# cherise215/advchain

Hardware: AMD Instinct MI355X
Metric: augmented images/sec (N adv steps, chain=noise+bias+morph+affine) (higher is better)
Workload: dtype f32

## Files before the change

### advchain_amd/_lib.py

```python
import ctypes
import os
from ctypes import c_char_p, c_double, c_float, c_int, c_int64, c_void_p

_HERE = os.path.dirname(os.path.abspath(__file__))
LIB_PATH = os.path.join(_HERE, "csrc", "libadvchain_hip.so")

_P, _I, _L, _F, _D = c_void_p, c_int, c_int64, c_float, c_double

PROTOTYPES = {
    "advchain_version": (_I, []),
    "advchain_last_error": (c_char_p, []),
    "advchain_set_deterministic": (None, [_I]),
    "advchain_get_deterministic": (_I, []),
    "advchain_grid_sample_fwd": (_I, [_P, _P, _P, _L, _L, _I, _P, _P, _I, _I, _I, _P]),
    "advchain_grid_sample_fwd_ride": (_I, [_P, _P, _P, _P, _P, _L, _L, _I, _P, _P, _I, _I, _I, _I, _P]),
    "advchain_scatter_workspace": (_L, [_L, _I, _P]),
    "advchain_grid_sample_bwd": (_I, [_P, _P, _P, _P, _P, _P, _L, _L, _I, _P, _P, _I, _I, _I, _I, _P]),
    "advchain_window_stage_workspace": (_L, [_L, _L, _I, _P]),
    "advchain_grid_sample_bwd_staged": (_I, [_P, _P, _P, _P, _P, _P, _L, _L, _I, _P, _P, _I, _I, _I, _I, _P, _P]),
    "advchain_last_bwd_route": (_I, []),
    "advchain_det_warp_workspace": (_L, [_L, _L, _I, _P]),
    "advchain_grid_sample_bwd_det": (_I, [_P, _P, _P, _P, _P, _P, _L, _L, _I, _P, _P, _I, _I, _I, _P]),
    "advchain_compose_self_fwd": (_I, [_P, _P, _P, _L, _I, _P, _I, _P, _P]),
    "advchain_compose_self_bwd": (_I, [_P, _P, _P, _P, _I, _I, _L, _I, _P, _P]),
    "advchain_affine_warp_fwd": (_I, [_P, _P, _P, _L, _L, _I, _P, _I, _I, _P]),
    "advchain_affine_warp_fwd_ride": (_I, [_P, _P, _P, _P, _P, _L, _L, _I, _P, _I, _I, _I, _P]),
    "advchain_affine_warp_bwd_workspace": (_L, [_L, _I, _P]),
    "advchain_affine_warp_bwd": (_I, [_P, _P, _P, _P, _P, _P, _L, _L, _I, _P, _I, _I, _P]),
    "advchain_affine_warp_bwd_det": (_I, [_P, _P, _P, _P, _P, _P, _P, _L, _L, _I, _P, _I, _I, _P]),
    "advchain_affine_theta_fwd": (_I, [_P, _P, _F, _P, _P, _L, _I, _P]),
    "advchain_affine_theta_bwd": (_I, [_P, _P, _F, _P, _P, _P, _L, _I, _P]),
    "advchain_tp_interp_fwd": (_I, [_P, _P, _P, _P, _P, _P, _P, _L, _L, _I, _I, _F, _P, _P, _P]),
    "advchain_tp_interp_fwd_smoothed_pair": (_I, [_P, _P, _P, _P, _P, _P, _P, _P, _L, _L, _I, _F, _P, _P, _F, _P]),
    "advchain_band_reduce_axis": (_I, [_P, _P, _P, _P, _P, _P, _P, _P, _I, _L, _L, _F, _P]),
    "advchain_band_reduce_rows_dense": (_I, [_P, _P, _P, _P, _P, _L, _L, _L, _L, _F, _P]),
    "advchain_bias_field_fwd": (_I, [_P, _P, _P, _P, _P, _P, _P, _P, _P, _L, _L, _F, _I, _F, _P]),
    "advchain_bias_field_bwd": (_I, [_P, _P, _P, _P, _P, _P, _P, _P, _P, _P, _L, _L, _F, _I, _F, _P]),
    "advchain_bias_rows_per_wg": (_I, [_P, _L]),
    "advchain_bias_field_fwd_rows": (_I, [_P, _P, _P, _P, _P, _P, _P, _P, _P, _L, _L, _F, _I, _F, _I, _P]),
    "advchain_bias_field_bwd_rows": (_I, [_P, _P, _P, _P, _P, _P, _P, _P, _P, _P, _L, _L, _F, _I, _F, _I, _P]),
    "advchain_bias_field_bwd_reduced": (_I, [_P, _P, _P, _P, _P, _P, _P, _P, _P, _P, _L, _L, _F, _I, _F, _P, _P, _L, _I, _P]),
    "advchain_gauss_axis": (_I, [_P, _P, _P, _L, _L, _I, _P, _I, _P, _I, _I, _F, _P]),
    "advchain_gauss_axis_generic": (_I, [_P, _P, _L, _I, _P, _I, _P, _I, _F, _P]),
    "advchain_max_displacement": (_I, [_P, _P, _L, _I, _P, _P]),
    "advchain_grid_sample_bicubic2d_fwd": (_I, [_P, _P, _P, _L, _L, _P, _P, _I, _P]),
    "advchain_grid_sample_bicubic2d_bwd": (_I, [_P, _P, _P, _P, _P, _L, _L, _P, _P, _I, _P]),
    "advchain_affine_grid2d_fwd": (_I, [_P, _P, _L, _P, _P]),
    "advchain_affine_grid2d_bwd_workspace": (_L, [_L, _P]),
    "advchain_affine_grid2d_bwd": (_I, [_P, _P, _P, _L, _P, _P]),
    "advchain_slot_rows_max": (_I, [_P, _P, _L, _L, _I, _P]),
    "advchain_demons_compose_pair_fwd": (_I, [_P, _P, _P, _P, _P, _P, _P, _P, _P, _P, _P, _P, _P, _L, _I, _I, _P, _P, _F, _F, _I, _P]),
    "advchain_demons_compose_pair_bwd": (_I, [_P, _P, _P, _P, _P, _P, _P, _P, _P, _P, _P, _P, _P, _P, _P, _P, _P, _L, _P, _P, _P, _L,
                                              _I, _I, _P, _F, _F, _P]),
    "advchain_bounds_check": (_I, [_P, _P, _P, _L, _P, _P]),
    "advchain_expo_chain_fused_levels": (_I, [_L, _I, _P, _I, _P]),
    "advchain_expo_chain_fwd": (_I, [_P, _P, _P, _L, _I, _P, _I, _P, _P, _P, _P]),
    "advchain_expo_chain_bwd": (_I, [_P, _P, _P, _P, _P, _P, _P, _L, _I, _P, _I, _P]),
    "advchain_gauss_xy": (_I, [_P, _P, _P, _L, _L, _I, _P, _P, _I, _I, _F, _P, _P, _L]),
    "advchain_gauss_xy_staged": (_I, [_P, _P, _P, _L, _L, _I, _P, _P, _I, _I, _F, _P, _P, _L]),
    "advchain_gauss_xy_lanes": (_I, [_P, _P, _P, _L, _L, _I, _P, _P, _I, _I, _F, _P, _P, _L, _I, _I]),
    "advchain_gauss_xy_plan": (_I, [_I, _P, _L, _P, _P, _P]),
    "advchain_gauss_small": (_I, [_P, _P, _L, _I, _P, _P, _I, _F, _P]),
    "advchain_gauss_small_pair": (_I, [_P, _P, _L, _I, _P, _P, _F, _I, _P]),
    "advchain_axpy": (_I, [_P, _P, _P, _F, _L, _P]),
    "advchain_sign_axpy": (_I, [_P, _P, _P, _F, _L, _P, _P, _P]),
    "advchain_nonzero_mask": (_I, [_P, _P, _L, _P]),
    "advchain_consistency_finish": (_I, [_P, _P, _P, _P, _I, _P]),
    "advchain_norm_workspace": (_L, [_L, _L]),
    "advchain_norm_axpy": (_I, [_P, _P, _P, _P, _F, _L, _L, _P]),
    "advchain_norm_axpy_gated": (_I, [_P, _P, _P, _P, _F, _L, _L, _P, _P, _P]),
    "advchain_update_multi": (_I, [_P, _I, _P, _P]),
    "advchain_consistency_fwd": (_I, [_P, _P, _P, _P, _P, _P, _P, _L, _L, _I, _P, _I, _I, _I, _I, _P]),
    "advchain_consistency_bwd": (_I, [_P, _P, _P, _P, _P, _P, _F, _F, _F, _F, _I, _L, _L, _I, _P, _I, _P]),
    "advchain_consistency_fused_fwd": (_I, [_P, _P, _P, _P, _P, _L, _L, _I, _P, _I, _I, _I, _I, _P]),
    "advchain_consistency_fused_bwd": (_I, [_P, _P, _P, _P, _P, _P, _F, _F, _F, _F, _I, _L, _L, _I, _P, _I, _P]),
    "advchain_consistency_wide_fwd": (_I, [_P, _P, _P, _P, _P, _P, _L, _L, _I, _P, _I, _I, _I, _I, _P]),
    "advchain_consistency_wide_bwd": (_I, [_P, _P, _P, _P, _P, _P, _P, _F, _F, _F, _F, _I, _L, _L, _I, _P, _I, _P]),
    "advchain_consistency_ref_bwd": (_I, [_P, _P, _P, _P, _P, _P, _P, _F, _F, _F, _F, _I, _L, _L, _I, _P, _I, _P]),
    "advchain_set_ref_grad_reg_max_k": (None, [_I]),
    "advchain_get_ref_grad_reg_max_k": (_I, []),
    "advchain_consistency_lp_fwd": (_I, [_P, _I, _P, _I, _P, _P, _P, _P, _L, _L, _I, _P, _I, _I, _I, _I, _P]),
    "advchain_consistency_lp_bwd": (_I, [_P, _I, _P, _I, _P, _P, _P, _P, _P, _F, _F, _F, _F, _I, _L, _L, _I, _P, _I, _P]),
    "advchain_consistency_lp_ref_bwd": (_I, [_P, _I, _P, _I, _P, _P, _P, _P, _P, _F, _F, _F, _F, _I, _L, _L, _I, _P, _I, _P]),
    "advchain_consistency_cw_fwd": (_I, [_P, _I, _P, _I, _P, _P, _P, _P, _L, _L, _I, _P, _I, _I, _I, _I, _P, _P]),
    "advchain_consistency_cw_bwd": (_I, [_P, _I, _P, _I, _P, _P, _P, _P, _P, _F, _F, _F, _F, _I, _L, _L, _I, _P, _I, _P, _P]),
    "advchain_consistency_cw_ref_bwd": (_I, [_P, _I, _P, _I, _P, _P, _P, _P, _P, _F, _F, _F, _F, _I, _L, _L, _I, _P, _I, _P, _P]),
    "advchain_consistency_fused_fwd_bf16": (_I, [_P, _P, _P, _P, _P, _L, _L, _I, _P, _P]),
    "advchain_consistency_fused_bwd_bf16": (_I, [_P, _P, _P, _P, _P, _P, _F, _F, _F, _L, _L, _I, _P, _P]),
    "advchain_seg_loss_workspace": (_L, [_L, _I, _P]),
    "advchain_ce2d_fwd": (_I, [_P, _I, _P, _P, _P, _P, _P, _P, _L, _L, _P, _F, _P]),
    "advchain_ce2d_bwd": (_I, [_P, _I, _P, _P, _P, _P, _P, _P, _P, _L, _L, _P, _F, _P]),
    "advchain_contour_fwd": (_I, [_P, _P, _P, _P, _P, _P, _P, _L, _L, _I, _P, _I, _I, _P]),
    "advchain_contour_bwd": (_I, [_P, _P, _P, _P, _L, _L, _I, _P, _I, _P]),
    "advchain_one_hot": (_I, [_P, _P, _L, _L, _L, _P]),
    "advchain_dice_workspace": (_L, [_L, _L, _I, _P]),
    "advchain_dice_fwd": (_I, [_P, _I, _P, _P, _P, _P, _P, _P, _P, _L, _L, _I, _P, _I, _F, _F, _F, _P]),
    "advchain_dice_bwd": (_I, [_P, _I, _P, _P, _P, _P, _P, _P, _P, _P, _L, _L, _I, _P, _F, _F, _P]),
    "advchain_edt": (_I, [_P, _I, _P, _I, _P, _L, _I, _P, _P]),
    "advchain_signed_maps_workspace": (_L, [_L, _L, _I, _P]),
    "advchain_signed_maps": (_I, [_P, _P, _P, _P, _L, _L, _I, _P, _P]),
    "advchain_surface_metrics_workspace": (_L, [_L, _L, _I, _P]),
    "advchain_surface_metrics": (_I, [_P, _P, _P, _D, _P, _P, _P, _P, _P, _P, _P, _P, _P, _L, _L, _I, _P, _P]),
    "advchain_boundary_workspace": (_L, [_L, _L, _I, _P]),
    "advchain_boundary_fwd": (_I, [_P, _I, _P, _P, _P, _P, _P, _P, _L, _L, _I, _P, _I, _P]),
    "advchain_boundary_bwd": (_I, [_P, _I, _P, _P, _P, _P, _P, _P, _L, _L, _I, _P, _I, _P]),
    "advchain_image_diff2d_fwd": (_I, [_P, _P, _P, _L, _L, _P, _P]),
    "advchain_image_diff2d_bwd": (_I, [_P, _P, _P, _L, _L, _P, _P]),
    "advchain_jacobian_det2d_fwd": (_I, [_P, _P, _L, _P, _P]),
    "advchain_jacobian_det2d_bwd": (_I, [_P, _P, _P, _L, _P, _P]),
    "advchain_expo_start": (_I, [_P, _P, _F, _L, _I, _P, _P]),
    "advchain_image_diff3d_fwd": (_I, [_P, _P, _P, _P, _L, _L, _P, _P]),
    "advchain_image_diff3d_bwd": (_I, [_P, _P, _P, _P, _L, _L, _P, _P]),
    "advchain_jacobian_det_fwd": (_I, [_P, _P, _L, _I, _P, _I, _P]),
    "advchain_jacobian_det_bwd": (_I, [_P, _P, _P, _P, _L, _I, _P, _I, _P]),
    "advchain_jacobian_det_workspace": (_L, [_L, _I, _P]),
    "advchain_jacobian_stats_workspace": (_L, [_L, _I, _P]),
    "advchain_jacobian_stats": (_I, [_P, _P, _P, _P, _P, _P, _L, _I, _P, _I, _P]),
    "advchain_sumsq_ordered": (_I, [_P, _L, _P, _P, _P]),
    "advchain_bicubic2d_det_workspace": (_L, [_L, _L, _P]),
    "advchain_grid_sample_bicubic2d_bwd_det": (_I, [_P, _P, _P, _P, _P, _P, _L, _L, _P, _P, _I, _P]),
    "advchain_tp_interp_sumsq_partials": (_L, [_P, _L]),
    "advchain_tp_interp_sumsq_ordered": (_I, [_P, _P, _P, _P, _P, _P, _L, _L, _P, _P, _P]),
    "advchain_consistency_fwd_partials": (_L, [_L, _L, _I, _P, _I, _I, _I]),
    "advchain_consistency_fwd_ord": (_I, [_P, _P, _P, _P, _P, _P, _P, _L, _P, _L, _L, _I, _P, _I, _I, _I, _I, _P]),
    "advchain_consistency_fused_fwd_partials": (_L, [_L, _L, _I, _P, _I, _I, _I, _I]),
    "advchain_consistency_fused_fwd_ord": (_I, [_P, _P, _P, _P, _P, _L, _P, _L, _L, _I, _P, _I, _I, _I, _I, _P]),
    "advchain_consistency_wide_fwd_partials": (_L, [_L, _L, _I, _P, _I, _I]),
    "advchain_consistency_wide_fwd_ord": (_I, [_P, _P, _P, _P, _P, _P, _L, _P, _L, _L, _I, _P, _I, _I, _I, _I, _P]),
    "advchain_consistency_lp_fwd_partials": (_L, [_L, _L, _I, _P, _I]),
    "advchain_consistency_lp_fwd_ord": (_I, [_P, _I, _P, _I, _P, _P, _P, _P, _L, _P, _L, _L, _I, _P, _I, _I, _I, _I, _P, _P]),
    "advchain_consistency_finish_ord": (_I, [_P, _L, _P, _P, _P, _P, _P]),
}

class UpdateDesc(ctypes.Structure):
    _fields_ = [("base", c_void_p), ("x", c_void_p), ("out", c_void_p), ("old", c_void_p), ("N", c_int64), ("M", c_int64),
                ("kind", ctypes.c_int32), ("step", c_float)]


_lib = None


class AdvchainHipError(RuntimeError):
    pass


class _Lib(object):

    def __init__(self, cdll):
        self._cdll = cdll
        self._raw = {}
        self.records = []

    def _bind(self, name, res, args):
        fn = getattr(self._cdll, name)
        fn.restype = res
        fn.argtypes = args
        self._raw[name] = fn
        setattr(self, name, fn)

    def timed(self, names=None, every=1):
        import contextlib
        import torch

        @contextlib.contextmanager
        def ctx():
            chosen = [n for n in self._raw if (names is None or n in names) and self._raw[n].restype is c_int
                      and len(self._raw[n].argtypes) > 0]
            for n in chosen:
                raw = self._raw[n]

                count = [0]

                def wrapped(*a, _raw=raw, _n=n, _count=count):
                    _count[0] += 1
                    if _count[0] % every:
                        return _raw(*a)
                    e0 = torch.cuda.Event(enable_timing=True)
                    e1 = torch.cuda.Event(enable_timing=True)
                    e0.record()
                    rc = _raw(*a)
                    e1.record()
                    self.records.append((_n, a, e0, e1))
                    return rc
                setattr(self, n, wrapped)
# ... 47 lines not shown
```

### advchain_amd/csrc/adjoint_gather.hip

```cpp
#include "sampler_common.h"

namespace advchain {

constexpr int kXPad = 4;

__global__ void k_gather_prepare(int32_t* ws, int chain) {
  ws[2] = chain ? ws[3] : 0;
  ws[0] = 0;
  ws[1] = 0;
  ws[3] = 0;
}

template <int E>
__device__ __forceinline__ float tent(float f) { return fmaxf(0.f, 1.f - fabsf(f - (float)E)); }

template <int H, int K = -H>
struct XSpread {
  template <int C>
  static __device__ __forceinline__ void run(float (&acc)[C][2 * H + 1], const float (&a)[C], float fx) {
    const float w = tent<K>(fx);
#pragma unroll
    for (int c = 0; c < C; ++c) acc[c][K + H] = fmaf(a[c], w, acc[c][K + H]);
    if constexpr (K < H) XSpread<H, K + 1>::template run<C>(acc, a, fx);
  }
// ... 394 lines not shown
#pragma unroll
    for (int cz = 0; cz < (DIM == 3 ? 2 : 1); ++cz)
#pragma unroll
      for (int cy = 0; cy < 2; ++cy)
#pragma unroll
        for (int cx = 0; cx < 2; ++cx) {
          if (!t.ok(cz, cy, cx)) continue;
          const int o = t.off(cz, cy, cx, d);
          const float wgt = t.w(cz, cy, cx);
          for (int c = 0; c < C; ++c) {
            const float v = wgt * gout[((int64_t)n * C + c) * V + s];
            const float old = atomicAdd(gin + ((int64_t)n * C + c) * V + o, v);
            const float nv = fabsf(old + v);
            if (absmax_out && nv > __builtin_nontemporal_load(absmax_out))
              atomicMax(reinterpret_cast<unsigned int*>(absmax_out), __float_as_uint(nv));
          }
        }
  }
}

template <int VEC>
__global__ void __launch_bounds__(kBlock) k_max_displacement(const float* __restrict__ phi, float* __restrict__ out, Dims d, int ndim) {
  const int V = (int)d.voxels();
  const int plane = blockIdx.y;
  const int a = plane % ndim;
  const int Sa = a == 0 ? d.s2 : (a == 1 ? d.s1 : d.s0);
  const float* p = phi + (int64_t)plane * V;
  float m = 0.f;
  for (int i = (blockIdx.x * kBlock + threadIdx.x) * VEC; i < V; i += gridDim.x * kBlock * VEC) {
    float v[VEC];
    load_vec<VEC>(p + i, v);
    const int x = i % d.s2, q = i / d.s2;
    const int y = q % d.s1, z = q / d.s1;
#pragma unroll
    for (int k = 0; k < VEC; ++k) {
      const int sa = a == 0 ? x + k : (a == 1 ? y : z);
      const float dv = fabsf(unnormalize(v[k], Sa) - (float)sa);
      m = fmaxf(m, dv < 1.0e9f ? dv : 1.0e9f);
    }
  }
#pragma unroll
  for (int o = 32; o > 0; o >>= 1) m = fmaxf(m, __shfl_xor(m, o, 64));
  __shared__ float smem[kBlock / 64];
  if ((threadIdx.x & 63) == 0) smem[threadIdx.x >> 6] = m;
  __syncthreads();
  if (threadIdx.x == 0) {
    for (int w = 1; w < kBlock / 64; ++w) m = fmaxf(m, smem[w]);
    if (m > __builtin_nontemporal_load(out)) atomicMax(reinterpret_cast<unsigned int*>(out), __float_as_uint(m));
  }
}

template <int NT, int VEC>
__global__ void __launch_bounds__(NT) k_slot_rows_max(float* __restrict__ slots, float* __restrict__ out, int cols, int reset) {
  float* p = slots + (int64_t)blockIdx.x * cols;
  float m = -3.4e38f;
  bool nan = false;
  if (VEC == 4) {
    for (int j = threadIdx.x * 4; j < cols; j += NT * 4) {
      const float4 v = *reinterpret_cast<const float4*>(p + j);
      nan = nan || !(v.x == v.x) || !(v.y == v.y) || !(v.z == v.z) || !(v.w == v.w);
      m = fmaxf(fmaxf(m, fmaxf(v.x, v.y)), fmaxf(v.z, v.w));
      if (reset) *reinterpret_cast<float4*>(p + j) = make_float4(0.f, 0.f, 0.f, 0.f);
    }
  } else {
    for (int j = threadIdx.x; j < cols; j += NT) {
      const float v = p[j];
      nan = nan || !(v == v);
      m = fmaxf(m, v);
      if (reset) p[j] = 0.f;
    }
  }
#pragma unroll
  for (int o = 32; o > 0; o >>= 1) {
    m = fmaxf(m, __shfl_xor(m, o, 64));
    const int other = __shfl_xor((int)nan, o, 64);
    nan = nan || other != 0;
  }
  __shared__ float sm[NT / 64];
  __shared__ int sn[NT / 64];
  if ((threadIdx.x & 63) == 0) { sm[threadIdx.x >> 6] = m; sn[threadIdx.x >> 6] = nan; }
  __syncthreads();
  if (threadIdx.x == 0) {
    for (int w = 1; w < NT / 64; ++w) { m = fmaxf(m, sm[w]); nan = nan || sn[w]; }
    out[blockIdx.x] = nan ? __int_as_float(0x7fc00000) : m;
  }
}

__global__ void __launch_bounds__(64) k_bounds_check(const float* __restrict__ v, const float* __restrict__ lo,
                                                     const float* __restrict__ hi, int n, int* __restrict__ flag) {
  bool bad = false;
  for (int i = threadIdx.x; i < n; i += 64) {
    const float x = v[i];
    bad = bad || !(x >= lo[i] && x < hi[i]);
  }
  if (__any(bad) && threadIdx.x == 0) atomicOr(flag, 1);
}

}

using namespace advchain;

template <int DIM, int C, int H, bool SELF, bool GG, int TZ, int TY, int NT>
static void launch_gather(const float* gout, const float* in, const float* grid, float* gin, float* ggrid, int64_t N,
                          Dims d, int padding, int clamp_grid, int32_t* ws, int chain, bool strict, hipStream_t st) {
  using G = GatherCfg<DIM, C, H, SELF, GG, TZ, TY, NT>;
  const int wide = d.s2 > 64;
  const int n2 = wide ? (d.s2 + (64 - 2 * kXPad) - 1) / (64 - 2 * kXPad) : 1;
  const int n1 = (d.s1 + TY - 1) / TY;
  const int n0 = DIM == 3 ? (d.s0 + TZ - 1) / TZ : 1;
  int* cnt = ws;
  float* amax_out = SELF ? reinterpret_cast<float*>(ws + 3) : nullptr;
  int2* list = reinterpret_cast<int2*>(ws + 4);
  const int64_t cap64 = N * d.voxels();
  const int cap = cap64 > 0x7fffffff ? 0x7fffffff : (int)cap64;
  const bool border = padding == PAD_BORDER;
  const uintptr_t al = reinterpret_cast<uintptr_t>(gout) | reinterpret_cast<uintptr_t>(grid) |
                       (GatherCfg<DIM, C, H, SELF, GG, TZ, TY, NT>::STAGE_IN ? reinterpret_cast<uintptr_t>(in) : 0);
  const bool unaligned = (d.s2 & 3) != 0 || (al & 15) != 0;
  const int flags = ((border || clamp_grid) ? kClip : 0) | (border ? kBorder : 0) | (clamp_grid ? kClampGrid : 0) |
                    (unaligned ? kUnaligned : 0);
  auto kern = k_adjoint_gather<DIM, C, H, SELF, GG, TZ, TY, NT>;
  static bool attr_set = false;
  if (G::LDS > 65536 && !attr_set) {
    (void)hipFuncSetAttribute(reinterpret_cast<const void*>(kern), hipFuncAttributeMaxDynamicSharedMemorySize, (int)G::LDS);
    attr_set = true;
  }
  if (strict) {
    hipLaunchKernelGGL(kern, dim3((unsigned)(n0 * n1 * n2), (unsigned)N), dim3(NT), G::LDS, st, gout, in, grid, gin, ggrid,
                       d, n1, n2, wide, flags, (float*)nullptr, (int*)nullptr, (int2*)nullptr, 0, SELF ? ws : (int32_t*)nullptr);
    return;
  }
  hipLaunchKernelGGL(k_gather_prepare, dim3(1), dim3(1), 0, st, ws, chain);
  hipLaunchKernelGGL(kern, dim3((unsigned)(n0 * n1 * n2), (unsigned)N), dim3(NT), G::LDS, st, gout, in, grid, gin, ggrid, d,
                     n1, n2, wide, flags, amax_out, cnt, list, cap, (int32_t*)nullptr);
  if (border) hipLaunchKernelGGL((k_gather_overflow<DIM, PAD_BORDER>), dim3(16), dim3(kBlock), 0, st, gout, grid, gin, C, d,
                                 clamp_grid, cnt, list, cap, amax_out);
  else hipLaunchKernelGGL((k_gather_overflow<DIM, PAD_ZEROS>), dim3(16), dim3(kBlock), 0, st, gout, grid, gin, C, d,
                          clamp_grid, cnt, list, cap, amax_out);
// ... 110 lines not shown
```

### advchain_amd/csrc/common.h

```cpp
#pragma once
#include <hip/hip_runtime.h>
#include <stdint.h>

namespace advchain {

__device__ __forceinline__ float sub_max(float m) { return m == -__builtin_inff() ? -3.402823466e38f : m; }

enum { INTERP_LINEAR = 0, INTERP_NEAREST = 1 };
enum { PAD_ZEROS = 0, PAD_BORDER = 1, PAD_REFLECTION = 2 };

constexpr int kBlock = 256;

struct Dims {
  int s0, s1, s2;
  __host__ __device__ int64_t voxels() const { return (int64_t)s0 * s1 * s2; }
};

__device__ __forceinline__ float mul_nc(float a, float b) {
#pragma clang fp contract(off)
  return a * b;
}

__device__ __forceinline__ float lin_coord(int i, int S) {
  if (S <= 1) return S == 1 ? -1.f : 0.f;
// ... 42 lines not shown
    else if (x >= (float)(S - 1)) { x = (float)(S - 1); mult = 0.f; }
  }
  return x;
}

template <int PAD>
__device__ __forceinline__ AxisTap make_tap(float coord, int S) {
  AxisTap t;
  float x = source_index<PAD>(coord, S, t.mult);
  if (!(x > -1.0e9f && x < 1.0e9f)) x = -16.f;
  const float f = floorf(x);
  t.i0 = (int)f;
  t.w1 = x - f;
  t.w0 = (f + 1.f) - x;
  t.v0 = (t.i0 >= 0) && (t.i0 < S);
  t.v1 = (t.i0 + 1 >= 0) && (t.i0 + 1 < S);
  return t;
}

template <int PAD>
__device__ __forceinline__ int nearest_index(float coord, int S, bool& valid) {
  float m;
  float x = source_index<PAD>(coord, S, m);
  if (!(x > -1.0e9f && x < 1.0e9f)) x = -16.f;
  const int i = (int)nearbyintf(x);
  valid = (i >= 0) && (i < S);
  return i;
}

__device__ __forceinline__ float wave_sum(float v) {
#pragma unroll
  for (int o = 32; o > 0; o >>= 1) v += __shfl_xor(v, o, 64);
  return v;
}

template <int NV>
__device__ __forceinline__ void block_sum(float (&v)[NV], float* smem) {
  const int lane = threadIdx.x & 63, wave = threadIdx.x >> 6;
#pragma unroll
  for (int k = 0; k < NV; ++k) v[k] = wave_sum(v[k]);
  if (lane == 0) {
#pragma unroll
    for (int k = 0; k < NV; ++k) smem[wave * NV + k] = v[k];
  }
  __syncthreads();
  if (threadIdx.x == 0) {
    const int nw = (blockDim.x + 63) >> 6;
#pragma unroll
    for (int k = 0; k < NV; ++k) {
      float s = 0.f;
      for (int w = 0; w < nw; ++w) s += smem[w * NV + k];
      v[k] = s;
    }
  }
}

__device__ __forceinline__ float lane_next_f(float v) {
  return __int_as_float(__builtin_amdgcn_update_dpp(0, __float_as_int(v), 0x130, 0xf, 0xf, false));
}
__device__ __forceinline__ float lane_prev_f(float v) {
  return __int_as_float(__builtin_amdgcn_update_dpp(0, __float_as_int(v), 0x138, 0xf, 0xf, false));
}

template <int CTRL, int ROW_MASK>
__device__ __forceinline__ float dpp_add(float v) {
  return v + __int_as_float(__builtin_amdgcn_update_dpp(0, __float_as_int(v), CTRL, ROW_MASK, 0xf, false));
}
__device__ __forceinline__ float wave_sum_lane63(float v) {
  v = dpp_add<0xB1, 0xf>(v);
  v = dpp_add<0x4E, 0xf>(v);
  v = dpp_add<0x141, 0xf>(v);
  v = dpp_add<0x140, 0xf>(v);
  v = dpp_add<0x142, 0xa>(v);
  return dpp_add<0x143, 0xc>(v);
}

constexpr int kSumSlots = 64;
__device__ __forceinline__ int sum_slot() { return (int)((blockIdx.x + blockIdx.y * 7u) % kSumSlots); }

#ifndef ADVCHAIN_FIX_RPI
#define ADVCHAIN_FIX_RPI 1
#endif
__device__ __forceinline__ int fix_round(float x) {
#if ADVCHAIN_FIX_RPI
  int r;
  asm("v_cvt_rpi_i32_f32 %0, %1" : "=v"(r) : "v"(x));
  return r;
#else
  return __float2int_rn(x);
#endif
}

struct FixScale {
  int shift;
  float mul;
  float inv;
};
__device__ __forceinline__ FixScale fix_scale(float gmax, int bits) {
  FixScale s;
  const bool ok = gmax <= 3.40282347e38f;
  const int e = ok ? __builtin_amdgcn_frexp_expf(gmax) : 0;
  const float gm = ok ? __builtin_amdgcn_frexp_mantf(gmax) : gmax;
  s.shift = bits - e;
  s.mul = (gmax > 0.f && ok) ? 1.f / gm : 0.f;
  s.inv = gm;
  return s;
// ... 89 lines not shown
```

### advchain_amd/csrc/demons_compose.cpp

```cpp
#include <stdint.h>
#include "advchain_hip.h"

#define ADVCHAIN_OK 0
#define ADVCHAIN_ERR_ARG (-1)
extern "C" void advchain_set_error_(const char* msg);
bool advchain_gauss_xy_takes(int ndim, const int64_t* dims, int64_t planes);

namespace {
inline int64_t prod(int ndim, const int64_t* d) {
  int64_t p = 1;
  for (int i = 0; i < ndim; ++i) p *= d[i];
  return p;
}
inline bool aligned16(const void* a, const void* b = nullptr, const void* c = nullptr, const void* d = nullptr) {
  return ((reinterpret_cast<uintptr_t>(a) | reinterpret_cast<uintptr_t>(b) | reinterpret_cast<uintptr_t>(c) |
           reinterpret_cast<uintptr_t>(d)) & 15) == 0;
}
}

extern "C" {

int advchain_demons_compose_pair_fwd(const float* vel, float* s1, float* phi0, float* fields, float* pos, float* q,
                                     float* disp, float* rows_max, const int32_t* itab, const float* ftab,
                                     const int64_t* S3, const int64_t* g3, const int64_t* B3, int64_t N, int ndim, int n,
                                     const int32_t* hints, const float* weights9_host, float scale, float inv, int fuse,
                                     void* stream) {
  if (!(vel && s1 && phi0 && pos && q && itab && ftab && S3 && g3 && B3 && weights9_host) || ndim != 2 || n < 1 || (n > 1 && !fields)) {
    advchain_set_error_("demons_compose_pair_fwd: null pointer / bad arguments (2D only)");
    return ADVCHAIN_ERR_ARG;
  }
  const int64_t* gd = g3 + 1;
  const int64_t* Sd = S3 + 1;
  if (prod(ndim, gd) > 4096 || !advchain_gauss_xy_takes(ndim, Sd, 2 * N * ndim) || !aligned16(pos, q)) return -2;
  int rc = advchain_tp_interp_fwd_smoothed_pair(vel, s1, phi0, itab, ftab, S3, g3, B3, N * ndim, ndim, 1, inv, disp, weights9_host,
                                                scale, stream);
  if (rc == -2) {
    rc = advchain_gauss_small_pair(vel, s1, N * ndim, ndim, gd, weights9_host, scale, 0, stream);
    if (rc != 0) return rc;
    rc = advchain_tp_interp_fwd(s1, phi0, itab, ftab, S3, g3, B3, 2 * N * ndim, ndim, ndim, 1, inv, nullptr, disp, stream);
  }
  if (rc != 0) return rc;
  auto late = [](int r, const char* what) {
    if (r == -2) { advchain_set_error_(what); return ADVCHAIN_ERR_ARG; }
    return r;
  };
  const int64_t slots = ADVCHAIN_DISP_SLOTS;
  rc = advchain_expo_chain_fwd(phi0, fields, pos, 2 * N, ndim, Sd, n, disp, hints, (disp && fuse) ? disp + (int64_t)(n + 1) * slots : nullptr, stream);
  if (rc != 0) return late(rc, "demons_compose_pair_fwd: the chain refused a shape the pre-check had accepted (launches already queued)");
  rc = advchain_gauss_xy(pos, q, nullptr, 2 * N * ndim, ndim, ndim, Sd, weights9_host, 2, 1, 1.0f, stream, nullptr, 2 * N * ndim);
  if (rc != 0) return late(rc, "demons_compose_pair_fwd: the final smoothing refused a shape the pre-check had accepted (launches already queued)");
  if (disp && rows_max) rc = advchain_slot_rows_max(disp, rows_max, n + 2, slots, 1, stream);
  return rc;
}

int advchain_demons_compose_pair_bwd(const float* gq_lo, const float* gq_hi, const float* pos, const float* phi0,
                                     const float* fields, float* gpos, float* g, float* scratch, int32_t* ws, float* t1,
                                     float* gs1, float* gvel, const int32_t* halos, const int32_t* itab, const float* ftab,
                                     const float* wd, const int32_t* wlo, int64_t WB, const int64_t* S3, const int64_t* g3,
                                     const int64_t* B3, int64_t N, int ndim, int n, const float* weights9_host, float scale,
                                     float inv, void* stream) {
  if (!(gq_lo && gq_hi && pos && phi0 && gpos && g && scratch && ws && t1 && gs1 && gvel && halos && itab && ftab && wd && wlo &&
        weights9_host) || ndim != 2 || n < 1) {
    advchain_set_error_("demons_compose_pair_bwd: null pointer / bad arguments (2D only)");
    return ADVCHAIN_ERR_ARG;
  }
  const int64_t* gd = g3 + 1;
  const int64_t* Sd = S3 + 1;
  const int64_t planes = 2 * N * ndim;
  if (prod(ndim, gd) > 4096 || !advchain_gauss_xy_takes(ndim, Sd, planes) || !aligned16(gq_lo, gq_hi, gpos, pos)) return -2;
  int rc = advchain_gauss_xy(gq_lo, gpos, pos, planes, ndim, ndim, Sd, weights9_host, 0, 2, 1.0f, stream, gq_hi, N * ndim);
  if (rc != 0) return rc;
  rc = advchain_expo_chain_bwd(gpos, phi0, fields, g, scratch, ws, halos, 2 * N, ndim, Sd, n, stream);
  if (rc == -2) {
    advchain_set_error_("demons_compose_pair_bwd: the chain refused a shape the pre-check had accepted (launches already queued)");
    return ADVCHAIN_ERR_ARG;
  }
  if (rc != 0) return rc;
  rc = advchain_band_reduce_rows_dense(g, gpos, t1, wd, wlo, planes * S3[1], S3[2], g3[2], WB, inv, stream);
  if (rc == -2) rc = advchain_band_reduce_axis(g, gpos, t1, itab, ftab, S3, g3, B3, 2, planes * S3[1], 1, inv, stream);
  if (rc != 0) return rc;
  rc = advchain_band_reduce_axis(t1, nullptr, gs1, itab, ftab, S3, g3, B3, 1, planes, g3[2], 1.0f, stream);
  if (rc != 0) return rc;
  return advchain_gauss_small_pair(gs1, gvel, N * ndim, ndim, gd, weights9_host, scale, 1, stream);
}

}
```

### advchain_amd/csrc/error.cpp

```cpp
#include <string.h>

#include <atomic>

static thread_local char g_last_error[512] = "";

extern "C" void advchain_set_error_(const char* msg) {
  strncpy(g_last_error, msg ? msg : "", sizeof(g_last_error) - 1);
  g_last_error[sizeof(g_last_error) - 1] = 0;
}

extern "C" const char* advchain_last_error(void) { return g_last_error; }

static std::atomic<int> g_deterministic{0};
extern "C" void advchain_set_deterministic(int on) { g_deterministic.store(on ? 1 : 0, std::memory_order_relaxed); }
extern "C" int advchain_get_deterministic(void) { return g_deterministic.load(std::memory_order_relaxed); }

static thread_local int g_last_bwd_route = 0;
extern "C" void advchain_set_route_(int route) { g_last_bwd_route = route; }
extern "C" int advchain_last_bwd_route(void) { return g_last_bwd_route; }

extern "C" int advchain_version(void) { return 200; }
```

### advchain_amd/csrc/fields.hip

```cpp
#include "sampler_common.h"

namespace advchain {

constexpr int kBandMax = 8;

struct BandAxis {
  const int* start;
  const float* w;
  const int* lo;
  const int* hi;
  int S, g, B;
};
struct BandTables { BandAxis a[3]; };

__device__ __forceinline__ void decode3(int v, const Dims& d, int& i0, int& i1, int& i2) {
  i2 = v % d.s2;
  const int r = v / d.s2;
  i1 = r % d.s1;
  i0 = r / d.s1;
}

__device__ __forceinline__ float tp_eval(const float* __restrict__ coef, const BandTables& T, int i0, int i1, int i2) {
  const BandAxis& A0 = T.a[0];
  const BandAxis& A1 = T.a[1];
  const BandAxis& A2 = T.a[2];
  const int s0 = A0.start[i0], s1 = A1.start[i1], s2 = A2.start[i2];
  const float* w0 = A0.w + i0 * A0.B;
  const float* w1 = A1.w + i1 * A1.B;
  const float* w2 = A2.w + i2 * A2.B;
  float acc = 0.f;
  for (int a = 0; a < A0.B; ++a) {
    float acc1 = 0.f;
    for (int b = 0; b < A1.B; ++b) {
      const float* row = coef + ((int64_t)(s0 + a) * A1.g + (s1 + b)) * A2.g + s2;
      float acc2 = 0.f;
      for (int c = 0; c < A2.B; ++c) acc2 += row[c] * w2[c];
      acc1 += acc2 * w1[b];
    }
    acc += acc1 * w0[a];
  }
  return acc;
}

constexpr int kTpChunk = 32;
constexpr int kTpMaxLds = 2048;

struct TpGeom { int XT, ROWS; };

__host__ __device__ inline TpGeom tp_geom(int S2) {
  TpGeom g;
  (void)S2;
  g.XT = 64;
// ... 858 lines not shown
      qb[b] = *reinterpret_cast<const float4*>(in + t + ((x0 >= 0 && x0 < d.s2) ? (b - 1) * 4 : 0));
    }
#pragma unroll
    for (int b = 0; b < 3; ++b) {
      const int x0 = idx[2] + (b - 1) * 4;
      const bool inr = x0 >= 0 && x0 < d.s2;
      win[b * 4 + 0] = inr ? pre(qb[b].x, idx[0], idx[1], x0) : 0.f;
      win[b * 4 + 1] = inr ? pre(qb[b].y, idx[0], idx[1], x0 + 1) : 0.f;
      win[b * 4 + 2] = inr ? pre(qb[b].z, idx[0], idx[1], x0 + 2) : 0.f;
      win[b * 4 + 3] = inr ? pre(qb[b].w, idx[0], idx[1], x0 + 3) : 0.f;
    }
#pragma unroll
    for (int o = 0; o < 4; ++o)
#pragma unroll
      for (int k = 0; k < 9; ++k) acc[o] += gw.w[k] * win[o + k];
  } else {
    const int stride = AXIS == 1 ? d.s2 : d.s1 * d.s2;
    const int ia = idx[AXIS];
    float4 q[9];
#pragma unroll
    for (int k = -4; k <= 4; ++k) {
      const int jc = min(max(ia + k, 0), S[AXIS] - 1);
      q[k + 4] = *reinterpret_cast<const float4*>(in + t + (int64_t)(jc - ia) * stride);
    }
#pragma unroll
    for (int k = -4; k <= 4; ++k) {
      const int j = ia + k;
      const bool inr = j >= 0 && j < S[AXIS];
      const int j0 = AXIS == 0 ? j : idx[0], j1 = AXIS == 1 ? j : idx[1];
      const float w = gw.w[k + 4];
      acc[0] += inr ? w * pre(q[k + 4].x, j0, j1, idx[2]) : 0.f;
      acc[1] += inr ? w * pre(q[k + 4].y, j0, j1, idx[2] + 1) : 0.f;
      acc[2] += inr ? w * pre(q[k + 4].z, j0, j1, idx[2] + 2) : 0.f;
      acc[3] += inr ? w * pre(q[k + 4].w, j0, j1, idx[2] + 3) : 0.f;
    }
  }
  if (POST == 1) {
#pragma unroll
    for (int o = 0; o < 4; ++o) acc[o] += lin_coord(caxis == 2 ? idx[2] + o : idx[caxis], S[caxis]);
  }
  if (POST == 2) {
    const float4 a = *reinterpret_cast<const float4*>(aux + t);
    const float av[4] = {a.x, a.y, a.z, a.w};
#pragma unroll
    for (int o = 0; o < 4; ++o) {
      float slope;
      border_identity(av[o], S[caxis], slope);
      acc[o] *= slope;
    }
  }
  *reinterpret_cast<float4*>(out + t) = make_float4(acc[0], acc[1], acc[2], acc[3]);
}

template <int PRE, int POST>
__global__ void __launch_bounds__(kBlock)
k_gauss_xy(const float* __restrict__ in, float* __restrict__ out, const float* __restrict__ aux, Dims d, int C, GaussW gw,
           float scale, int TY, const float* __restrict__ in_hi, int planes_lo) {
  extern __shared__ float gx_lds[];
  const int W = d.s2, Q = W >> 2, PA = W + 8;
  const int R = TY + 8;
  float* A = gx_lds;
  float* B = gx_lds + R * PA;
  const int plane = blockIdx.z, iz = blockIdx.y;
  const int y0 = blockIdx.x * TY;
  const int caxis = 2 - plane % C;
  const int Sc = caxis == 2 ? d.s2 : (caxis == 1 ? d.s1 : d.s0);
  const int64_t base = ((int64_t)plane * d.s0 + iz) * d.s1 * (int64_t)W;
  const float* src = (in_hi && plane >= planes_lo) ? in_hi + (((int64_t)(plane - planes_lo) * d.s0 + iz) * d.s1 * (int64_t)W) : in + base;
  for (int e = threadIdx.x; e < R * 2; e += kBlock)
    *reinterpret_cast<float4*>(A + (e >> 1) * PA + ((e & 1) ? W + 4 : 0)) = make_float4(0.f, 0.f, 0.f, 0.f);
  for (int e = threadIdx.x; e < R * Q; e += kBlock) {
    const int r = e / Q, q = e - r * Q;
    const int gy = y0 - 4 + r;
    const bool inr = gy >= 0 && gy < d.s1;
    const float4 v = *reinterpret_cast<const float4*>(src + (int64_t)min(max(gy, 0), d.s1 - 1) * W + 4 * q);
    float t[4] = {v.x, v.y, v.z, v.w};
#pragma unroll
    for (int o = 0; o < 4; ++o) {
      if (PRE == 1) t[o] *= scale;
      if (PRE == 2) {
        float sl;
        t[o] = border_identity(t[o], Sc, sl) - lin_coord(caxis == 2 ? 4 * q + o : (caxis == 1 ? gy : iz), Sc);
      }
      if (!inr) t[o] = 0.f;
    }
    *reinterpret_cast<float4*>(A + r * PA + 4 + 4 * q) = make_float4(t[0], t[1], t[2], t[3]);
  }
  __syncthreads();
  for (int e = threadIdx.x; e < R * Q; e += kBlock) {
    const int r = e / Q, q = e - r * Q;
    const float* a = A + r * PA + 4 * q;
    const float4 a0 = *reinterpret_cast<const float4*>(a), a1 = *reinterpret_cast<const float4*>(a + 4),
                 a2 = *reinterpret_cast<const float4*>(a + 8);
    const float win[12] = {a0.x, a0.y, a0.z, a0.w, a1.x, a1.y, a1.z, a1.w, a2.x, a2.y, a2.z, a2.w};
    float acc[4] = {0.f, 0.f, 0.f, 0.f};
#pragma unroll
    for (int o = 0; o < 4; ++o)
#pragma unroll
      for (int k = 0; k < 9; ++k) acc[o] += gw.w[k] * win[o + k];
    *reinterpret_cast<float4*>(B + r * W + 4 * q) = make_float4(acc[0], acc[1], acc[2], acc[3]);
  }
  __syncthreads();
  for (int e = threadIdx.x; e < TY * Q; e += kBlock) {
    const int ry = e / Q, q = e - ry * Q;
    const int gy = y0 + ry;
    if (gy >= d.s1) continue;
    float acc[4] = {0.f, 0.f, 0.f, 0.f};
#pragma unroll
    for (int k = 0; k < 9; ++k) {
      const float4 b = *reinterpret_cast<const float4*>(B + (ry + k) * W + 4 * q);
      acc[0] += gw.w[k] * b.x; acc[1] += gw.w[k] * b.y; acc[2] += gw.w[k] * b.z; acc[3] += gw.w[k] * b.w;
    }
    const int64_t off = base + (int64_t)gy * W + 4 * q;
    if (POST == 1) {
#pragma unroll
      for (int o = 0; o < 4; ++o) acc[o] += lin_coord(caxis == 2 ? 4 * q + o : (caxis == 1 ? gy : iz), Sc);
    }
    if (POST == 2) {
      const float4 a4 = *reinterpret_cast<const float4*>(aux + off);
      const float av[4] = {a4.x, a4.y, a4.z, a4.w};
#pragma unroll
      for (int o = 0; o < 4; ++o) {
        float slope;
        border_identity(av[o], Sc, slope);
        acc[o] *= slope;
      }
    }
    *reinterpret_cast<float4*>(out + off) = make_float4(acc[0], acc[1], acc[2], acc[3]);
  }
}

template <int PRE, int POST, int NT, int U>
__global__ void __launch_bounds__(NT)
k_gauss_xy_lanes(const float* __restrict__ in, float* __restrict__ out, const float* __restrict__ aux, Dims d, int C, GaussW gw,
                 float scale, int TY, const float* __restrict__ in_hi, int planes_lo) {
  extern __shared__ float gx_lds[];
  const int W = d.s2, Q = W >> 2;
  const int R = TY + 8, NI = R * Q;
  float* B = gx_lds;
  const int plane = blockIdx.z, iz = blockIdx.y;
  const int y0 = blockIdx.x * TY;
  const int caxis = 2 - plane % C;
  const int Sc = caxis == 2 ? d.s2 : (caxis == 1 ? d.s1 : d.s0);
  const int64_t base = ((int64_t)plane * d.s0 + iz) * d.s1 * (int64_t)W;
  const float* src = (in_hi && plane >= planes_lo) ? in_hi + (((int64_t)(plane - planes_lo) * d.s0 + iz) * d.s1 * (int64_t)W) : in + base;
  float4 v[U];
#pragma unroll
  for (int u = 0; u < U; ++u) {
    if (u * NT >= NI) break;
    const int e = min((int)threadIdx.x + u * NT, NI - 1);
    const int r = e / Q, q = e - r * Q;
    const int gy = y0 - 4 + r;
    v[u] = *reinterpret_cast<const float4*>(src + (int64_t)min(max(gy, 0), d.s1 - 1) * W + 4 * q);
  }
#pragma unroll
  for (int u = 0; u < U; ++u) {
    if (u * NT >= NI) break;
    const int e0 = (int)threadIdx.x + u * NT;
    const int e = min(e0, NI - 1);
    const int r = e / Q, q = e - r * Q;
    const int gy = y0 - 4 + r;
    const bool inr = gy >= 0 && gy < d.s1;
    float t[4] = {v[u].x, v[u].y, v[u].z, v[u].w};
#pragma unroll
    for (int o = 0; o < 4; ++o) {
      if (PRE == 1) t[o] *= scale;
      if (PRE == 2) {
        float sl;
        t[o] = border_identity(t[o], Sc, sl) - lin_coord(caxis == 2 ? 4 * q + o : (caxis == 1 ? gy : iz), Sc);
      }
      if (!inr) t[o] = 0.f;
    }
    float win[12];
    const bool first = q == 0, last = q == Q - 1;
#pragma unroll
    for (int o = 0; o < 4; ++o) {
      const float pv = lane_prev_f(t[o]), nx = lane_next_f(t[o]);
      win[o] = first ? 0.f : pv;
      win[4 + o] = t[o];
      win[8 + o] = last ? 0.f : nx;
    }
    float acc[4] = {0.f, 0.f, 0.f, 0.f};
#pragma unroll
    for (int o = 0; o < 4; ++o)
#pragma unroll
      for (int k = 0; k < 9; ++k) acc[o] += gw.w[k] * win[o + k];
    if (e0 < NI) *reinterpret_cast<float4*>(B + r * W + 4 * q) = make_float4(acc[0], acc[1], acc[2], acc[3]);
  }
  __syncthreads();
// ... 112 lines not shown
template <int NT>
__global__ void __launch_bounds__(NT)
k_gauss_small(const float* __restrict__ in, float* __restrict__ out, Dims d, int ndim, GaussW gw, float scale, int mirror,
              int P) {
  __shared__ float buf[2][kGaussSmallMax];
  const int V = (int)d.voxels();
  const int S[3] = {d.s0, d.s1, d.s2};
  const int stride[3] = {d.s1 * d.s2, d.s2, 1};
  const int b = blockIdx.x;
  float first[(kGaussSmallMax + NT - 1) / NT];
  const int rounds = mirror == 2 ? 2 : 1;
  for (int round = 0; round < rounds; ++round) {
    const float* src = in + (int64_t)(mirror == 1 ? b % P : b + round * P) * V;
    const float sc = (mirror == 1 && b >= P) ? -scale : scale;
    if (round) __syncthreads();
    for (int i = threadIdx.x; i < V; i += NT) buf[0][i] = src[i] * sc;
    __syncthreads();
    int cur = 0;
    for (int pass = 0; pass < ndim; ++pass) {
      const int axis = 2 - pass;
      const int Sa = S[axis], st = stride[axis];
      for (int i = threadIdx.x; i < V; i += NT) {
        const int ia = (i / st) % Sa;
        float acc = 0.f;
#pragma unroll
        for (int k = -4; k <= 4; ++k) {
          const int j = ia + k;
          if (j >= 0 && j < Sa) acc += gw.w[k + 4] * buf[cur][i + k * st];
        }
        buf[cur ^ 1][i] = acc;
      }
      __syncthreads();
      cur ^= 1;
    }
    float* dst = out + (int64_t)b * V;
    if (mirror != 2) {
      for (int i = threadIdx.x; i < V; i += NT) dst[i] = buf[cur][i];
    } else if (round == 0) {
#pragma unroll
      for (int q = 0; q < (kGaussSmallMax + NT - 1) / NT; ++q) {
        const int i = threadIdx.x + q * NT;
        first[q] = i < V ? buf[cur][i] : 0.f;
      }
    } else {
#pragma unroll
      for (int q = 0; q < (kGaussSmallMax + NT - 1) / NT; ++q) {
        const int i = threadIdx.x + q * NT;
        if (i < V) dst[i] = first[q] - buf[cur][i];
      }
    }
  }
}

__global__ void __launch_bounds__(kBlock)
k_axpy(const float* __restrict__ x, const float* __restrict__ y, float* __restrict__ out, float a, int64_t n4,
       int64_t n) {
  const int64_t i = (int64_t)blockIdx.x * kBlock + threadIdx.x;
  if (i < n4) {
    const float4 p = reinterpret_cast<const float4*>(y)[i];
    float4 q = x ? reinterpret_cast<const float4*>(x)[i] : make_float4(0.f, 0.f, 0.f, 0.f);
    q.x += a * p.x; q.y += a * p.y; q.z += a * p.z; q.w += a * p.w;
    reinterpret_cast<float4*>(out)[i] = q;
  }
  const int64_t j = n4 * 4 + i;
  if (j < n) out[j] = (x ? x[j] : 0.f) + a * y[j];
}

__global__ void __launch_bounds__(kBlock)
k_sign_axpy(const float* __restrict__ base, const float* __restrict__ x, float* __restrict__ out, float a, int64_t n,
            const float* __restrict__ gate, const float* __restrict__ old) {
  const int64_t i = (int64_t)blockIdx.x * kBlock + threadIdx.x;
  if (i >= n) return;
  if (gate && !(fabsf(gate[0]) <= 3.0e38f)) { out[i] = old[i]; return; }
  const float v = x[i];
  const float sg = v > 0.f ? 1.f : (v < 0.f ? -1.f : v);
  out[i] = (base ? base[i] : 0.f) + a * sg;
}

__global__ void __launch_bounds__(kBlock)
k_nonzero_mask(const float* __restrict__ x, float* __restrict__ out, int64_t n) {
  const int64_t i = (int64_t)blockIdx.x * kBlock + threadIdx.x;
  if (i < n) out[i] = x[i] != 0.f ? 1.f : 0.f;
}

__global__ void __launch_bounds__(kBlock)
k_sumsq_partial(const float* __restrict__ x, float* __restrict__ partial, int64_t M, int chunk) {
  __shared__ float smem[4];
  const int n = blockIdx.y, b = blockIdx.x;
  const float* xn = x + (int64_t)n * M;
  const int64_t lo = (int64_t)b * chunk, hi = min(lo + chunk, M);
  float s[1] = {0.f};
  for (int64_t i = lo + threadIdx.x; i < hi; i += kBlock) { const float q = xn[i]; s[0] += q * q; }
  block_sum<1>(s, smem);
  if (threadIdx.x == 0) partial[(int64_t)n * gridDim.x + b] = s[0];
}

__global__ void __launch_bounds__(kBlock)
k_norm_axpy(const float* __restrict__ base, const float* __restrict__ x, const float* __restrict__ partial,
            int nb, float step, float* __restrict__ out, int64_t M, int chunk, const float* __restrict__ gate,
            const float* __restrict__ old) {
  __shared__ float smem[4];
  __shared__ float inv_s;
  const int n = blockIdx.y, b = blockIdx.x;
  float s[1] = {0.f};
  for (int i = threadIdx.x; i < nb; i += kBlock) s[0] += partial[(int64_t)n * nb + i];
  block_sum<1>(s, smem);
// ... 525 lines not shown
  }
#define GA(PRE, POST)                                                                                                     \
  do {                                                                                                                    \
    if (!v4) hipLaunchKernelGGL((k_gauss_axis<PRE, POST>), grid, blk, 0, st, in, out, aux, total, d, (int)C, axis, gw, scale); \
    else if (axis == 2) hipLaunchKernelGGL((k_gauss_axis_v4<PRE, POST, 2>), grid, blk, 0, st, in, out, aux, total / 4, d, (int)C, gw, scale, riw); \
    else if (axis == 1) hipLaunchKernelGGL((k_gauss_axis_v4<PRE, POST, 1>), grid, blk, 0, st, in, out, aux, total / 4, d, (int)C, gw, scale, 0); \
    else hipLaunchKernelGGL((k_gauss_axis_v4<PRE, POST, 0>), grid, blk, 0, st, in, out, aux, total / 4, d, (int)C, gw, scale, 0); \
  } while (0)
  switch (pre * 3 + post) {
    case 0: GA(0, 0); break;
    case 1: GA(0, 1); break;
    case 2: GA(0, 2); break;
    case 3: GA(1, 0); break;
    case 4: GA(1, 1); break;
    case 5: GA(1, 2); break;
    case 6: GA(2, 0); break;
    case 7: GA(2, 1); break;
    default: GA(2, 2); break;
  }
#undef GA
  ADVCHAIN_LAUNCH_CHECK();
  return ADVCHAIN_OK;
}

}

bool advchain_gauss_xy_takes(int ndim, const int64_t* dims, int64_t planes) {
  if (!dims_ok(ndim, dims)) return false;
  const Dims d = make_dims(ndim, dims);
  if ((d.s2 & 3) != 0 || d.s2 < 8 || d.s2 > 512 || d.s1 < 8 || planes > 65535 || d.s0 > 65535) return false;
  int TY = 32;
  while (TY > 8 && (size_t)(TY + 8) * (2 * d.s2 + 8) * 4 > 53248) TY >>= 1;
  if (TY > d.s1) TY = (d.s1 + 7) / 8 * 8;
  return (size_t)(TY + 8) * (2 * d.s2 + 8) * sizeof(float) <= 65536;
}

static bool gauss_xy_lane_shape(const Dims& d) {
  const int Q = d.s2 >> 2;
  return (d.s2 & 3) == 0 && Q >= 2 && Q <= 64 && (Q & (Q - 1)) == 0 && d.s1 >= 8;
}
static bool gauss_xy_lane_tile_ok(int ty, int nt) {
  return (ty == 16 && (nt == 256 || nt == 512)) || (ty == 32 && (nt == 256 || nt == 512)) || (ty == 64 && nt == 1024);
}
static bool gauss_xy_lane_rule(const Dims& d, int64_t planes, int& ty, int& nt) {
  (void)planes;
  if (!gauss_xy_lane_shape(d) || d.s2 != 256) return false;
  ty = 32; nt = 512;
  return true;
}
static inline int gauss_xy_clamp_ty(int TY, const Dims& d) { return TY > d.s1 ? (d.s1 + 7) / 8 * 8 : TY; }

enum { kGxyAuto = 0, kGxyStaged = 1, kGxyLanes = 2 };

static int gauss_xy_launch(const float* in, float* out, const float* aux, int64_t planes, int64_t C, int ndim, const int64_t* dims,
                           const float* weights9, int pre, int post, float scale, void* stream, const float* in_hi, int64_t planes_lo,
                           int want, int ty, int nt) {
  ADVCHAIN_CHECK_ARG(in && out && in != out && weights9, "gauss_xy: null/aliased pointer");
  ADVCHAIN_CHECK_ARG(dims_ok(ndim, dims), "gauss_xy: bad dims");
  ADVCHAIN_CHECK_ARG(C >= 1 && C <= 3 && pre >= 0 && pre <= 2 && post >= 0 && post <= 2 && (post != 2 || aux), "gauss_xy: bad C/pre/post");
  ADVCHAIN_CHECK_ARG(post == 0 || ndim == 2, "gauss_xy: post belongs to the last axis");
  const Dims d = make_dims(ndim, dims);
  if ((d.s2 & 3) != 0 || d.s2 < 8 || d.s2 > 512 || d.s1 < 8 || planes > 65535 || d.s0 > 65535 ||
      ((reinterpret_cast<uintptr_t>(in) | reinterpret_cast<uintptr_t>(out) | reinterpret_cast<uintptr_t>(aux) |
        reinterpret_cast<uintptr_t>(in_hi)) & 15) != 0)
    return ADVCHAIN_ERR_UNSUPPORTED;
  ADVCHAIN_CHECK_ARG(!in_hi || (planes_lo > 0 && planes_lo < planes), "gauss_xy: bad split of the input planes");
  if (want == kGxyLanes) {
    ADVCHAIN_CHECK_ARG(gauss_xy_lane_tile_ok(ty, nt), "gauss_xy_lanes: (ty, nt) must be (16,256), (16,512), (32,256), (32,512) or (64,1024)");
    if (!gauss_xy_lane_shape(d)) return ADVCHAIN_ERR_UNSUPPORTED;
  }
  if (planes == 0 || d.voxels() == 0) return ADVCHAIN_OK;
  GaussW gw;
  for (int k = 0; k < 9; ++k) gw.w[k] = weights9[k];
  hipStream_t st = (hipStream_t)stream;
  if (want == kGxyLanes || (want == kGxyAuto && gauss_xy_lane_rule(d, planes, ty, nt))) {
    const int TY = gauss_xy_clamp_ty(ty, d);
    const size_t lds = (size_t)(TY + 8) * d.s2 * sizeof(float);
    dim3 grid((unsigned)((d.s1 + TY - 1) / TY), (unsigned)d.s0, (unsigned)planes);
#define GXL(PRE, POST, NT_, U_) do { \
    auto kern = k_gauss_xy_lanes<PRE, POST, NT_, U_>; \
    if (lds > 65536) (void)hipFuncSetAttribute(reinterpret_cast<const void*>(kern), hipFuncAttributeMaxDynamicSharedMemorySize, (int)lds); \
    hipLaunchKernelGGL(kern, grid, dim3(NT_), lds, st, in, out, aux, d, (int)C, gw, scale, TY, in_hi, (int)planes_lo); } while (0)
#define GXL_TILE(PRE, POST) do { \
    if (ty == 16 && nt == 256) GXL(PRE, POST, 256, 6); \
    else if (ty == 16) GXL(PRE, POST, 512, 3); \
    else if (ty == 32 && nt == 256) GXL(PRE, POST, 256, 10); \
    else if (ty == 32) GXL(PRE, POST, 512, 5); \
    else GXL(PRE, POST, 1024, 5); } while (0)
    switch (pre * 3 + post) {
      case 0: GXL_TILE(0, 0); break;
      case 1: GXL_TILE(0, 1); break;
      case 2: GXL_TILE(0, 2); break;
      case 3: GXL_TILE(1, 0); break;
      case 4: GXL_TILE(1, 1); break;
      case 5: GXL_TILE(1, 2); break;
      case 6: GXL_TILE(2, 0); break;
      case 7: GXL_TILE(2, 1); break;
      default: GXL_TILE(2, 2); break;
    }
#undef GXL_TILE
#undef GXL
    ADVCHAIN_LAUNCH_CHECK();
    return ADVCHAIN_OK;
  }
  int TY = 32;
  while (TY > 8 && (size_t)(TY + 8) * (2 * d.s2 + 8) * 4 > 53248) TY >>= 1;
  if (TY > d.s1) TY = (d.s1 + 7) / 8 * 8;
  const size_t lds = (size_t)(TY + 8) * (2 * d.s2 + 8) * sizeof(float);
  if (lds > 65536) return ADVCHAIN_ERR_UNSUPPORTED;
  dim3 grid((unsigned)((d.s1 + TY - 1) / TY), (unsigned)d.s0, (unsigned)planes);
#define GXY(PRE, POST) hipLaunchKernelGGL((k_gauss_xy<PRE, POST>), grid, dim3(kBlock), lds, st, in, out, aux, d, (int)C, gw, scale, TY, in_hi, (int)planes_lo)
  switch (pre * 3 + post) {
    case 0: GXY(0, 0); break;
    case 1: GXY(0, 1); break;
    case 2: GXY(0, 2); break;
    case 3: GXY(1, 0); break;
    case 4: GXY(1, 1); break;
    case 5: GXY(1, 2); break;
    case 6: GXY(2, 0); break;
    case 7: GXY(2, 1); break;
    default: GXY(2, 2); break;
  }
#undef GXY
  ADVCHAIN_LAUNCH_CHECK();
  return ADVCHAIN_OK;
}

extern "C" {

int advchain_gauss_xy(const float* in, float* out, const float* aux, int64_t planes, int64_t C, int ndim, const int64_t* dims,
                      const float* weights9, int pre, int post, float scale, void* stream, const float* in_hi, int64_t planes_lo) {
  return gauss_xy_launch(in, out, aux, planes, C, ndim, dims, weights9, pre, post, scale, stream, in_hi, planes_lo, kGxyAuto, 0, 0);
}

int advchain_gauss_xy_staged(const float* in, float* out, const float* aux, int64_t planes, int64_t C, int ndim,
                             const int64_t* dims, const float* weights9, int pre, int post, float scale, void* stream,
                             const float* in_hi, int64_t planes_lo) {
  return gauss_xy_launch(in, out, aux, planes, C, ndim, dims, weights9, pre, post, scale, stream, in_hi, planes_lo, kGxyStaged, 0, 0);
}

int advchain_gauss_xy_lanes(const float* in, float* out, const float* aux, int64_t planes, int64_t C, int ndim,
                            const int64_t* dims, const float* weights9, int pre, int post, float scale, void* stream,
                            const float* in_hi, int64_t planes_lo, int ty, int nt) {
  return gauss_xy_launch(in, out, aux, planes, C, ndim, dims, weights9, pre, post, scale, stream, in_hi, planes_lo, kGxyLanes, ty, nt);
}

int advchain_gauss_xy_plan(int ndim, const int64_t* dims, int64_t planes, int* form, int* ty, int* nt) {
  if (!form || !ty || !nt || !dims_ok(ndim, dims) || planes < 0) return -1;
  *form = 0; *ty = 0; *nt = 0;
  if (!advchain_gauss_xy_takes(ndim, dims, planes)) return 0;
  const Dims d = make_dims(ndim, dims);
  int t = 0, n = 0;
  if (gauss_xy_lane_rule(d, planes, t, n)) {
    *form = 2; *ty = gauss_xy_clamp_ty(t, d); *nt = n;
    return 0;
  }
  int TY = 32;
  while (TY > 8 && (size_t)(TY + 8) * (2 * d.s2 + 8) * 4 > 53248) TY >>= 1;
  *form = 1; *ty = gauss_xy_clamp_ty(TY, d); *nt = kBlock;
  return 0;
}

static int gauss_small_launch(const float* in, float* out, int64_t planes, int ndim, const int64_t* dims,
                              const float* weights9, int pre, float scale, int mirror, void* stream) {
  ADVCHAIN_CHECK_ARG(in && out && in != out && weights9, "gauss_small: null/aliased pointer");
  ADVCHAIN_CHECK_ARG(dims_ok(ndim, dims), "gauss_small: bad dims");
  ADVCHAIN_CHECK_ARG(pre == 0 || pre == 1, "gauss_small: pre must be 0 or 1");
  const Dims d = make_dims(ndim, dims);
  ADVCHAIN_CHECK_ARG(d.voxels() <= kGaussSmallMax, "gauss_small: plane larger than 4096 voxels");
  ADVCHAIN_CHECK_ARG(planes >= 0 && planes < (1ll << 30), "gauss_small: bad plane count");
  if (planes == 0) return ADVCHAIN_OK;
  GaussW gw;
  for (int k = 0; k < 9; ++k) gw.w[k] = weights9[k];
  const unsigned blocks = (unsigned)(mirror == 1 ? 2 * planes : planes);
  if (d.voxels() > 1024)
    hipLaunchKernelGGL(k_gauss_small<1024>, dim3(blocks), dim3(1024), 0, (hipStream_t)stream, in, out, d, ndim, gw,
                       pre == 1 ? scale : 1.f, mirror, (int)planes);
  else
    hipLaunchKernelGGL(k_gauss_small<kBlock>, dim3(blocks), dim3(kBlock), 0, (hipStream_t)stream, in, out, d, ndim, gw,
                       pre == 1 ? scale : 1.f, mirror, (int)planes);
  ADVCHAIN_LAUNCH_CHECK();
  return ADVCHAIN_OK;
}

int advchain_gauss_small(const float* in, float* out, int64_t planes, int ndim, const int64_t* dims,
                         const float* weights9, int pre, float scale, void* stream) {
  return gauss_small_launch(in, out, planes, ndim, dims, weights9, pre, scale, 0, stream);
}

int advchain_gauss_small_pair(const float* in, float* out, int64_t planes, int ndim, const int64_t* dims,
                              const float* weights9, float scale, int adjoint, void* stream) {
  return gauss_small_launch(in, out, planes, ndim, dims, weights9, 1, scale, adjoint ? 2 : 1, stream);
}

int advchain_sign_axpy(const float* base, const float* x, float* out, float a, int64_t n, const float* gate, const float* old,
                       void* stream) {
  ADVCHAIN_CHECK_ARG(x && out && n >= 0 && (!gate || old), "sign_axpy: null pointer");
  if (n == 0) return ADVCHAIN_OK;
  hipLaunchKernelGGL(k_sign_axpy, dim3(advchain_blocks(n, kBlock)), dim3(kBlock), 0, (hipStream_t)stream, base, x, out, a, n, gate, old);
  ADVCHAIN_LAUNCH_CHECK();
  return ADVCHAIN_OK;
}

int advchain_nonzero_mask(const float* x, float* out, int64_t n, void* stream) {
  ADVCHAIN_CHECK_ARG(x && out && n >= 0, "nonzero_mask: null pointer");
  if (n == 0) return ADVCHAIN_OK;
  hipLaunchKernelGGL(k_nonzero_mask, dim3(advchain_blocks(n, kBlock)), dim3(kBlock), 0, (hipStream_t)stream, x, out, n);
  ADVCHAIN_LAUNCH_CHECK();
  return ADVCHAIN_OK;
}

int advchain_axpy(const float* x, const float* y, float* out, float a, int64_t n, void* stream) {
  ADVCHAIN_CHECK_ARG(y && out && n >= 0, "axpy: null pointer");
  if (n == 0) return ADVCHAIN_OK;
  const bool al = ((reinterpret_cast<uintptr_t>(y) | reinterpret_cast<uintptr_t>(out) | reinterpret_cast<uintptr_t>(x)) & 15) == 0;
  const int64_t n4 = al ? n / 4 : 0;
  const int64_t threads = n4 > (n - 4 * n4) ? n4 : (n - 4 * n4);
  hipLaunchKernelGGL(k_axpy, dim3(advchain_blocks(threads, kBlock)), dim3(kBlock), 0, (hipStream_t)stream, x, y, out, a, n4, n);
  ADVCHAIN_LAUNCH_CHECK();
  return ADVCHAIN_OK;
}

int64_t advchain_norm_workspace(int64_t N, int64_t M) {
  const int64_t chunk = 4096;
  return N * ((M + chunk - 1) / chunk);
}

int advchain_norm_axpy_gated(const float* base, const float* x, float* out, float* workspace, float step, int64_t N,
                             int64_t M, const float* gate, const float* old, void* stream) {
  ADVCHAIN_CHECK_ARG(x && out && workspace && (!gate || old), "norm_axpy: null pointer");
  ADVCHAIN_CHECK_ARG(N >= 0 && N < 65536 && M >= 0, "norm_axpy: bad N/M");
  if (N == 0 || M == 0) return ADVCHAIN_OK;
  const int chunk = 4096;
  const int nb = (int)((M + chunk - 1) / chunk);
  dim3 grid(nb, (unsigned)N), blk(kBlock);
  if (M <= 16384) {
    hipLaunchKernelGGL(k_norm_axpy_row, dim3((unsigned)N), blk, 0, (hipStream_t)stream, base, x, step, out, M, gate, old);
    ADVCHAIN_LAUNCH_CHECK();
    return ADVCHAIN_OK;
  }
  hipLaunchKernelGGL(k_sumsq_partial, grid, blk, 0, (hipStream_t)stream, x, workspace, M, chunk);
  hipLaunchKernelGGL(k_norm_axpy, grid, blk, 0, (hipStream_t)stream, base, x, workspace, nb, step, out, M, chunk, gate, old);
  ADVCHAIN_LAUNCH_CHECK();
  return ADVCHAIN_OK;
}

int advchain_norm_axpy(const float* base, const float* x, float* out, float* workspace, float step, int64_t N,
// ... 27 lines not shown
```

### advchain_amd/csrc/loss.hip

```cpp
#include <algorithm>
#include "loss_common.h"

namespace advchain {

constexpr int kMaxK = 16;

template <class... ORD>
__global__ void __launch_bounds__(kBlock)
k_softmax_diff(const float* __restrict__ pred, const float* __restrict__ ref, const float* __restrict__ mask,
               float* __restrict__ P, float* __restrict__ D, float* __restrict__ sums, int K, int V, int mask_ch,
               int ref_is_prob, int want_kl, ORD... ord) {
  __shared__ float smem[8];
  const int n = blockIdx.y;
  const int v = blockIdx.x * kBlock + threadIdx.x;
  float acc[2] = {0.f, 0.f};
  if (v < V) {
    const float* pn = pred + (int64_t)n * K * V + v;
    const float* rn = ref + (int64_t)n * K * V + v;
    float mp = -INFINITY, mr = -INFINITY;
    for (int k = 0; k < K; ++k) {
      mp = fmaxf(mp, pn[(int64_t)k * V]);
      mr = fmaxf(mr, rn[(int64_t)k * V]);
    }
    float sp = 0.f, sr = 0.f;
    for (int k = 0; k < K; ++k) {
      sp += ADVCHAIN_SM_EXP(pn[(int64_t)k * V] - mp);
      sr += ADVCHAIN_SM_EXP(rn[(int64_t)k * V] - mr);
    }
    const float lsp = logf(sp), lsr = logf(sr);
    const float isp = 1.f / sp, isr = 1.f / sr;
    for (int k = 0; k < K; ++k) {
      const float zp = pn[(int64_t)k * V] - mp, zr = rn[(int64_t)k * V] - mr;
      const float p = mul_nc(ADVCHAIN_SM_EXP(zp), isp);
      const float t = ref_is_prob ? rn[(int64_t)k * V] : mul_nc(ADVCHAIN_SM_EXP(zr), isr);
      const float m = mask ? mask[((int64_t)n * mask_ch + (mask_ch > 1 ? k : 0)) * V + v] : 1.f;
      const int64_t o = ((int64_t)n * K + k) * V + v;
      P[o] = p;
      D[o] = p - t;
      const float e = p * m - t * m;
      acc[0] += e * e;
      if (want_kl) acc[1] += kl_term(t, zr - lsr, zp - lsp, m, ref_is_prob);
    }
  }
  block_sum<2>(acc, smem);
  if (threadIdx.x == 0) {
    sums_put(sums, 0, acc[0], ord...);
    if (want_kl) sums_put(sums, 3, acc[1], ord...);
  }
}

template <int K, class... ORD>
__global__ void __launch_bounds__(kBlock)
k_softmax_diff_v4(const float* __restrict__ pred, const float* __restrict__ ref, const float* __restrict__ mask,
// ... 765 lines not shown
        }
      }
    }
  };
  if (EDGES) { row(y0 - 1, 0); }
  row(y0, 1);
  for (int i1 = y0; i1 < y1; ++i1) {
    if (EDGES) {
      row(i1 + 1, 2);
      const int v = (i0 * d.s1 + i1) * d.s2 + x;
      float m[4] = {1.f, 1.f, 1.f, 1.f};
      if (mask) {
        const float4 mm = *reinterpret_cast<const float4*>(mask + (int64_t)n * V + v);
        m[0] = mm.x; m[1] = mm.y; m[2] = mm.z; m[3] = mm.w;
      }
#pragma unroll
      for (int k = 1; k < K; ++k) {
        float ra[4], rb[4];
#pragma unroll
        for (int q = 0; q < 4; ++q) {
          float ga, gb;
          if (DIM == 2) {
            ga = zd[k - 1][0].v[q] + 2.f * zd[k - 1][1].v[q] + zd[k - 1][2].v[q];
            gb = zs[k - 1][0].v[q] - zs[k - 1][2].v[q];
          } else {
            ga = zs[k - 1][0].v[q] - zs[k - 1][2].v[q];
            gb = zd[k - 1][0].v[q] + 2.f * zd[k - 1][1].v[q] + zd[k - 1][2].v[q];
          }
          const float ea = ga * m[q], eb = gb * m[q];
          if (ok) { acc[1] += ea * ea; acc[2] += eb * eb; }
          ra[q] = 2.f * m[q] * m[q] * ga;
          rb[q] = 2.f * m[q] * m[q] * gb;
        }
        if (R && ok) {
          st4(R + ((int64_t)n * 2 * (K - 1) + 2 * (k - 1)) * V + v, ra[0], ra[1], ra[2], ra[3]);
          st4(R + ((int64_t)n * 2 * (K - 1) + 2 * (k - 1) + 1) * V + v, rb[0], rb[1], rb[2], rb[3]);
        }
        zs[k - 1][0] = zs[k - 1][1]; zs[k - 1][1] = zs[k - 1][2];
        zd[k - 1][0] = zd[k - 1][1]; zd[k - 1][1] = zd[k - 1][2];
      }
    } else if (i1 + 1 < y1) {
      row(i1 + 1, 1);
    }
  }
  block_sum<4>(acc, smem);
  if (threadIdx.x == 0) {
    sums_put(sums, 0, acc[0], ord...);
    if (EDGES) {
      sums_put(sums, 1, acc[1], ord...);
      sums_put(sums, 2, acc[2], ord...);
    }
    if (KL) sums_put(sums, 3, acc[3], ord...);
  }
}

template <int DIM, int K, bool KL, typename ST = float>
__global__ void __launch_bounds__(kBlock)
k_loss_fused_bwd4(const ST* __restrict__ pred, const ST* __restrict__ ref, const ST* __restrict__ R,
                  const float* __restrict__ mask, const float* __restrict__ gscale, ST* __restrict__ gpred,
                  float c_mse, float c_a, float c_b, Dims d, int mlen, float c_kl, int ref_is_prob) {
  const int n = blockIdx.y;
  const int V = (int)d.voxels();
  int i0, y0, x;
  bool first, last, ok;
  strip_decode4(d, mlen, i0, y0, x, first, last, ok);
  const float gs = gscale ? gscale[0] : 1.f;
  Quad za[K - 1][3], zb[K - 1][3];
  auto fold = [&](int k, int j1, Quad& a, Quad& b) {
    const ST* Ra = R + ((int64_t)n * 2 * (K - 1) + 2 * (k - 1)) * V;
    Quad as, ad, bs, bd;
    fold_row4<DIM>(Ra, i0, j1, x, first, last, d, as, ad);
    fold_row4<DIM>(Ra + V, i0, j1, x, first, last, d, bs, bd);
#pragma unroll
    for (int q = 0; q < 4; ++q) {
      a.v[q] = DIM == 3 ? as.v[q] : -ad.v[q];
      b.v[q] = DIM == 3 ? -bd.v[q] : bs.v[q];
    }
  };
  if (R) {
#pragma unroll
    for (int k = 1; k < K; ++k) {
      fold(k, y0 - 1, za[k - 1][0], zb[k - 1][0]);
      fold(k, y0, za[k - 1][1], zb[k - 1][1]);
    }
  }
  const int y1 = min(y0 + mlen, d.s1);
  for (int i1 = y0; i1 < y1; ++i1) {
    const int v = (i0 * d.s1 + i1) * d.s2 + x;
    float gp[K][4], pk[K][4], tk[K][4], mt[KL ? K : 1][4], lq[1][4], lt[1][4];
    float dot[4] = {0.f, 0.f, 0.f, 0.f}, klS[4] = {0.f, 0.f, 0.f, 0.f};
    float m[4] = {1.f, 1.f, 1.f, 1.f};
    if (mask) {
      const float4 mm = *reinterpret_cast<const float4*>(mask + (int64_t)n * V + v);
      m[0] = mm.x; m[1] = mm.y; m[2] = mm.z; m[3] = mm.w;
    }
    softmax_pair4<K, false, ST>(pred, ref, (int64_t)n * K * V + v, V, ref_is_prob, pk, tk, lq, lt);
#pragma unroll
    for (int k = 0; k < K; ++k) {
      if (k >= 1 && R) fold(k, i1 + 1, za[k - 1][2], zb[k - 1][2]);
#pragma unroll
      for (int q = 0; q < 4; ++q) {
        const float dv = pk[k][q] - tk[k][q];
        float g = c_mse * 2.f * m[q] * m[q] * dv;
        if (k >= 1 && R) {
          float sa, sb;
          if (DIM == 2) {
// ... 458 lines not shown
  ADVCHAIN_CHECK_ARG(pred && ref && P && D && sums, "consistency_fwd: null pointer");
  ADVCHAIN_CHECK_ARG(dims_ok(ndim, dims), "consistency_fwd: bad dims");
  ADVCHAIN_CHECK_ARG(N >= 0 && N < 65536 && K >= 1 && K <= kMaxK, "consistency_fwd: bad N/K (K <= 16)");
  ADVCHAIN_CHECK_ARG(!mask || mask_channels == 1 || mask_channels == K, "consistency_fwd: mask must have 1 or K channels");
  if (oc)
    for (int r = 0; r < 4; ++r) oc->counts[r] = 0;
  if (N == 0) return ADVCHAIN_OK;
  const Dims d = make_dims(ndim, dims);
  ADVCHAIN_CHECK_ARG(d.voxels() < (1ll << 31), "consistency_fwd: volume too large");
  const int V = (int)d.voxels();
  dim3 g(advchain_blocks(V, kBlock), (unsigned)N), b(kBlock);
  hipStream_t st = (hipStream_t)stream;
  const bool al16 = ((reinterpret_cast<uintptr_t>(pred) | reinterpret_cast<uintptr_t>(ref) | reinterpret_cast<uintptr_t>(mask) |
                      reinterpret_cast<uintptr_t>(P) | reinterpret_cast<uintptr_t>(D)) & 15) == 0;
  const bool v4 = V % 4 == 0 && al16 && K >= 2 && K <= 5;
  const dim3 g4(advchain_blocks(V / 4, kBlock), (unsigned)N);
  const bool edges = want_edges && K > 1;
  const bool rows = (d.s2 % 64) == 0;
  EdgeMarch em;
  const bool march = edges && mask_channels <= 1 && edge_march_plan(K, N, d, D, mask, R, rows, em);
  if (oc) {
    const dim3 gs = v4 ? g4 : g, ge = march ? em.grid : g;
    ADVCHAIN_CHECK_ARG(oc->fits(gs) && (!edges || oc->fits(ge)),
                       "consistency_fwd_ord: the partial buffer is smaller than a launch (advchain_consistency_fwd_partials)");
    oc->set(0, gs);
    if (want_kl) oc->set(3, gs);
    if (edges) { oc->set(1, ge); oc->set(2, ge); }
  }
  if (v4) {
    switch (K) {
      case 2: hipLaunchKernelGGL((k_softmax_diff_v4<2, ORD...>), g4, b, 0, st, pred, ref, mask, P, D, sums, V, mask_channels, ref_is_prob, want_kl, ord...); break;
      case 3: hipLaunchKernelGGL((k_softmax_diff_v4<3, ORD...>), g4, b, 0, st, pred, ref, mask, P, D, sums, V, mask_channels, ref_is_prob, want_kl, ord...); break;
      case 4: hipLaunchKernelGGL((k_softmax_diff_v4<4, ORD...>), g4, b, 0, st, pred, ref, mask, P, D, sums, V, mask_channels, ref_is_prob, want_kl, ord...); break;
      default: hipLaunchKernelGGL((k_softmax_diff_v4<5, ORD...>), g4, b, 0, st, pred, ref, mask, P, D, sums, V, mask_channels, ref_is_prob, want_kl, ord...); break;
    }
  } else {
    hipLaunchKernelGGL((k_softmax_diff<ORD...>), g, b, 0, st, pred, ref, mask, P, D, sums, (int)K, V, mask_channels, ref_is_prob, want_kl, ord...);
  }
  if (edges) {
    if (ndim == 3) {
      if (march) launch_edge_march<3>(em, K, d, st, D, mask, R, sums, mask_channels, ord...);
      else if (rows) hipLaunchKernelGGL((k_edge_fwd_rows<3, ORD...>), g, b, 0, st, D, mask, R, sums, (int)K, d, mask_channels, ord...);
      else hipLaunchKernelGGL((k_edge_fwd<3, ORD...>), g, b, 0, st, D, mask, R, sums, (int)K, d, mask_channels, ord...);
    } else {
      if (march) launch_edge_march<2>(em, K, d, st, D, mask, R, sums, mask_channels, ord...);
      else if (rows) hipLaunchKernelGGL((k_edge_fwd_rows<2, ORD...>), g, b, 0, st, D, mask, R, sums, (int)K, d, mask_channels, ord...);
      else hipLaunchKernelGGL((k_edge_fwd<2, ORD...>), g, b, 0, st, D, mask, R, sums, (int)K, d, mask_channels, ord...);
    }
  }
  ADVCHAIN_LAUNCH_CHECK();
  return ADVCHAIN_OK;
}

template <class... ORD>
static int consistency_fused_fwd(const OrdCounts* oc, const float* pred, const float* ref, const float* mask, float* R, float* sums,
                                 int64_t N, int64_t K, int ndim, const int64_t* dims, int mask_channels, int ref_is_prob,
                                 int want_edges, int want_kl, void* stream, ORD... ord) {
  ADVCHAIN_CHECK_ARG(pred && ref && sums, "consistency_fused_fwd: null pointer");
  ADVCHAIN_CHECK_ARG(dims_ok(ndim, dims), "consistency_fused_fwd: bad dims");
  ADVCHAIN_CHECK_ARG(N >= 0 && N < 65536 && K >= 1 && K <= kMaxK, "consistency_fused_fwd: bad N/K (K <= 16)");
  const Dims d = make_dims(ndim, dims);
  const bool edges = want_edges && K > 1;
  const bool zmarch = ndim == 3 && z3_takes(d, edges);
  if ((ndim == 3 && !zmarch) || K < 2 || K > 4 || (mask && mask_channels != 1)) return ADVCHAIN_ERR_UNSUPPORTED;
  if (d.voxels() >= (1ll << 31) || !march4_ok(d, pred, ref, mask, R)) return ADVCHAIN_ERR_UNSUPPORTED;
  if (oc)
    for (int r = 0; r < 4; ++r) oc->counts[r] = 0;
  if (N == 0) return ADVCHAIN_OK;
  const int zc = zmarch ? z3_chunk(d, N) : 0;
  const int mlen = zmarch ? 0 : march4_len(d, N);
  const dim3 gf = zmarch ? z3_grid(d, N, zc) : march4_grid(d, N, mlen);
  if (oc) {
    ADVCHAIN_CHECK_ARG(oc->fits(gf), "consistency_fused_fwd_ord: the partial buffer is smaller than the launch (advchain_consistency_fused_fwd_partials)");
    oc->set(0, gf);
    if (edges) { oc->set(1, gf); oc->set(2, gf); }
    if (want_kl) oc->set(3, gf);
  }
  if (zmarch) {
    const dim3 gz = gf, bz(kZ3Waves * 64);
    const size_t lds = z3_lds(d, K);
    hipStream_t stz = (hipStream_t)stream;
#define FWD3DZ(K_) do { \
      if (want_kl) hipLaunchKernelGGL((k_loss_fused_fwd3d_z<K_, true, ORD...>), gz, bz, lds, stz, pred, ref, mask, R, sums, d, zc, ref_is_prob, ord...); \
      else hipLaunchKernelGGL((k_loss_fused_fwd3d_z<K_, false, ORD...>), gz, bz, lds, stz, pred, ref, mask, R, sums, d, zc, ref_is_prob, ord...); } while (0)
    switch (K) { case 2: FWD3DZ(2); break; case 3: FWD3DZ(3); break; default: FWD3DZ(4); break; }
#undef FWD3DZ
    ADVCHAIN_LAUNCH_CHECK();
    return ADVCHAIN_OK;
  }
  if (edges && !R) R = nullptr;
  const dim3 g4 = gf, b4(kBlock);
  hipStream_t st = (hipStream_t)stream;
#define FUSED_FWD(DIM_, K_) do { \
    if (want_kl) { if (edges) hipLaunchKernelGGL((k_loss_fused_fwd4<DIM_, K_, true, true, float, ORD...>), g4, b4, 0, st, pred, ref, mask, R, sums, d, mlen, ref_is_prob, ord...); \
                   else hipLaunchKernelGGL((k_loss_fused_fwd4<DIM_, K_, true, false, float, ORD...>), g4, b4, 0, st, pred, ref, mask, R, sums, d, mlen, ref_is_prob, ord...); } \
    else { if (edges) hipLaunchKernelGGL((k_loss_fused_fwd4<DIM_, K_, false, true, float, ORD...>), g4, b4, 0, st, pred, ref, mask, R, sums, d, mlen, ref_is_prob, ord...); \
           else hipLaunchKernelGGL((k_loss_fused_fwd4<DIM_, K_, false, false, float, ORD...>), g4, b4, 0, st, pred, ref, mask, R, sums, d, mlen, ref_is_prob, ord...); } } while (0)
  switch (K) { case 2: FUSED_FWD(2, 2); break; case 3: FUSED_FWD(2, 3); break; default: FUSED_FWD(2, 4); break; }
#undef FUSED_FWD
  ADVCHAIN_LAUNCH_CHECK();
  return ADVCHAIN_OK;
}

__global__ void __launch_bounds__(kBlock)
k_consistency_finish_ord(const float* __restrict__ partials, int stride, int n0, int n1, int n2, int n3, float c0, float c1, float c2,
                         float c3, float* __restrict__ sums, float* __restrict__ value) {
  __shared__ float row[4];
  const int r = threadIdx.x >> 6, j = threadIdx.x & 63;
  const int cnt = r == 0 ? n0 : (r == 1 ? n1 : (r == 2 ? n2 : n3));
  const float* p = partials + (int64_t)r * stride;
  float v = 0.f;
  for (int i = j; i < cnt; i += 64) v += p[i];
  v = wave_sum(v);
  if (j == 0) { row[r] = v; sums[r] = v; }
  __syncthreads();
  if (threadIdx.x == 0) value[0] = ((c0 * row[0] + c1 * row[1]) + c2 * row[2]) + c3 * row[3];
}

extern "C" {

int advchain_consistency_fwd(const float* pred, const float* ref, const float* mask, float* P, float* D, float* R,
                             float* sums, int64_t N, int64_t K, int ndim, const int64_t* dims, int mask_channels,
                             int ref_is_prob, int want_edges, int want_kl, void* stream) {
  return consistency_fwd<>(nullptr, pred, ref, mask, P, D, R, sums, N, K, ndim, dims, mask_channels, ref_is_prob, want_edges,
                           want_kl, stream);
}

int64_t advchain_consistency_fwd_partials(int64_t N, int64_t K, int ndim, const int64_t* dims, int mask_channels, int want_edges,
                                          int aligned16) {
  if (!dims_ok(ndim, dims) || N < 0 || N >= 65536 || K < 1 || K > kMaxK) return -1;
  const Dims d = make_dims(ndim, dims);
  if (d.voxels() >= (1ll << 31)) return -1;
  const int64_t V = d.voxels();
  const int64_t all = (int64_t)advchain_blocks(V, kBlock) * N;
  int64_t w = (V % 4 == 0 && aligned16 && K >= 2 && K <= 5) ? (int64_t)advchain_blocks(V / 4, kBlock) * N : all;
  if (want_edges && K > 1) {
    EdgeMarch em;
    const float* a = reinterpret_cast<const float*>(aligned16 ? (uintptr_t)0 : (uintptr_t)4);
    if (N > 0 && mask_channels <= 1 && edge_march_plan(K, N, d, a, a, nullptr, (d.s2 % 64) == 0, em))
      w = std::max(w, (int64_t)em.grid.x * em.grid.y);
    else
      w = std::max(w, all);
  }
  return w;
}

int advchain_consistency_fwd_ord(const float* pred, const float* ref, const float* mask, float* P, float* D, float* R,
                                 float* partials, int64_t stride, int32_t* counts, int64_t N, int64_t K, int ndim,
                                 const int64_t* dims, int mask_channels, int ref_is_prob, int want_edges, int want_kl, void* stream) {
  ADVCHAIN_CHECK_ARG(counts && stride >= 1 && stride < (1ll << 31), "consistency_fwd_ord: bad partial buffer (stride / counts)");
  const OrdCounts oc{stride, counts};
  return consistency_fwd<SumsOrdered>(&oc, pred, ref, mask, P, D, R, partials, N, K, ndim, dims, mask_channels, ref_is_prob,
                                      want_edges, want_kl, stream, SumsOrdered{(int)stride});
}

int advchain_consistency_finish(float* slots, const float* coef4_host, float* sums, float* value, int reset, void* stream) {
  ADVCHAIN_CHECK_ARG(slots && coef4_host && sums && value, "consistency_finish: null pointer");
  static_assert(kSumSlots == 64 && kBlock == 256, "one wave per row of slots");
  hipLaunchKernelGGL(k_consistency_finish, dim3(1), dim3(kBlock), 0, (hipStream_t)stream, slots, coef4_host[0], coef4_host[1],
                     coef4_host[2], coef4_host[3], sums, value, reset);
  ADVCHAIN_LAUNCH_CHECK();
  return ADVCHAIN_OK;
}

int advchain_consistency_bwd(const float* P, const float* D, const float* R, const float* mask,
                             const float* grad_scale, float* grad_pred, float c_mse, float c_a, float c_b, float c_kl,
                             int kl_is_gt, int64_t N, int64_t K, int ndim, const int64_t* dims, int mask_channels,
                             void* stream) {
  ADVCHAIN_CHECK_ARG(P && D && grad_pred, "consistency_bwd: null pointer");
  ADVCHAIN_CHECK_ARG(dims_ok(ndim, dims), "consistency_bwd: bad dims");
  ADVCHAIN_CHECK_ARG(N >= 0 && N < 65536 && K >= 1 && K <= kMaxK, "consistency_bwd: bad N/K (K <= 16)");
  ADVCHAIN_CHECK_ARG(!mask || mask_channels == 1 || mask_channels == K, "consistency_bwd: mask must have 1 or K channels");
  if (N == 0) return ADVCHAIN_OK;
  const Dims d = make_dims(ndim, dims);
  ADVCHAIN_CHECK_ARG(d.voxels() < (1ll << 31), "consistency_bwd: volume too large");
  dim3 g(advchain_blocks(d.voxels(), kBlock), (unsigned)N), b(kBlock);
  hipStream_t st = (hipStream_t)stream;
  const bool rows = (d.s2 % 64) == 0;
  if (ndim == 3) {
    if (launch_bwd_march<3>(K, N, d, st, P, D, R, mask, grad_scale, grad_pred, c_mse, c_a, c_b, mask_channels, rows, c_kl, kl_is_gt)) {}
    else if (rows) hipLaunchKernelGGL(k_consistency_bwd_rows<3>, g, b, 0, st, P, D, R, mask, grad_scale, grad_pred, c_mse, c_a, c_b, (int)K, d, mask_channels, c_kl, kl_is_gt);
    else hipLaunchKernelGGL(k_consistency_bwd<3>, g, b, 0, st, P, D, R, mask, grad_scale, grad_pred, c_mse, c_a, c_b, (int)K, d, mask_channels, c_kl, kl_is_gt);
  } else {
    if (launch_bwd_march<2>(K, N, d, st, P, D, R, mask, grad_scale, grad_pred, c_mse, c_a, c_b, mask_channels, rows, c_kl, kl_is_gt)) {}
    else if (rows) hipLaunchKernelGGL(k_consistency_bwd_rows<2>, g, b, 0, st, P, D, R, mask, grad_scale, grad_pred, c_mse, c_a, c_b, (int)K, d, mask_channels, c_kl, kl_is_gt);
    else hipLaunchKernelGGL(k_consistency_bwd<2>, g, b, 0, st, P, D, R, mask, grad_scale, grad_pred, c_mse, c_a, c_b, (int)K, d, mask_channels, c_kl, kl_is_gt);
  }
  ADVCHAIN_LAUNCH_CHECK();
  return ADVCHAIN_OK;
}

int advchain_consistency_fused_fwd(const float* pred, const float* ref, const float* mask, float* R, float* sums, int64_t N,
                                   int64_t K, int ndim, const int64_t* dims, int mask_channels, int ref_is_prob, int want_edges,
                                   int want_kl, void* stream) {
  return consistency_fused_fwd<>(nullptr, pred, ref, mask, R, sums, N, K, ndim, dims, mask_channels, ref_is_prob, want_edges,
                                 want_kl, stream);
}

int64_t advchain_consistency_fused_fwd_partials(int64_t N, int64_t K, int ndim, const int64_t* dims, int has_mask, int mask_channels,
                                                int want_edges, int aligned16) {
  if (!dims_ok(ndim, dims) || N < 0 || N >= 65536 || K < 1 || K > kMaxK) return -1;
  const Dims d = make_dims(ndim, dims);
  const bool edges = want_edges && K > 1;
  const bool zmarch = ndim == 3 && z3_takes(d, edges);
  if ((ndim == 3 && !zmarch) || K < 2 || K > 4 || (has_mask && mask_channels != 1)) return ADVCHAIN_ERR_UNSUPPORTED;
  const void* a = reinterpret_cast<const void*>(aligned16 ? (uintptr_t)0 : (uintptr_t)4);
  if (d.voxels() >= (1ll << 31) || !march4_ok(d, a, a, a, a)) return ADVCHAIN_ERR_UNSUPPORTED;
  if (N == 0) return 0;
  const dim3 g = zmarch ? z3_grid(d, N, z3_chunk(d, N)) : march4_grid(d, N, march4_len(d, N));
  return (int64_t)g.x * g.y;
}

int advchain_consistency_fused_fwd_ord(const float* pred, const float* ref, const float* mask, float* R, float* partials,
                                       int64_t stride, int32_t* counts, int64_t N, int64_t K, int ndim, const int64_t* dims,
                                       int mask_channels, int ref_is_prob, int want_edges, int want_kl, void* stream) {
  ADVCHAIN_CHECK_ARG(counts && stride >= 1 && stride < (1ll << 31), "consistency_fused_fwd_ord: bad partial buffer (stride / counts)");
  const OrdCounts oc{stride, counts};
  return consistency_fused_fwd<SumsOrdered>(&oc, pred, ref, mask, R, partials, N, K, ndim, dims, mask_channels, ref_is_prob,
                                            want_edges, want_kl, stream, SumsOrdered{(int)stride});
}

int advchain_consistency_finish_ord(const float* partials, int64_t stride, const int32_t* counts4_host, const float* coef4_host,
                                    float* sums, float* value, void* stream) {
  ADVCHAIN_CHECK_ARG(partials && counts4_host && coef4_host && sums && value, "consistency_finish_ord: null pointer");
  ADVCHAIN_CHECK_ARG(stride >= 1 && stride < (1ll << 31), "consistency_finish_ord: bad stride");
  for (int r = 0; r < 4; ++r)
    ADVCHAIN_CHECK_ARG(counts4_host[r] >= 0 && counts4_host[r] <= stride, "consistency_finish_ord: a count exceeds the stride");
  hipLaunchKernelGGL(k_consistency_finish_ord, dim3(1), dim3(kBlock), 0, (hipStream_t)stream, partials, (int)stride, counts4_host[0],
                     counts4_host[1], counts4_host[2], counts4_host[3], coef4_host[0], coef4_host[1], coef4_host[2], coef4_host[3],
                     sums, value);
  ADVCHAIN_LAUNCH_CHECK();
  return ADVCHAIN_OK;
}

int advchain_consistency_fused_bwd(const float* pred, const float* ref, const float* R, const float* mask,
                                   const float* grad_scale, float* grad_pred, float c_mse, float c_a, float c_b, float c_kl,
                                   int ref_is_prob, int64_t N, int64_t K, int ndim, const int64_t* dims, int mask_channels,
                                   void* stream) {
  ADVCHAIN_CHECK_ARG(pred && ref && grad_pred, "consistency_fused_bwd: null pointer");
  ADVCHAIN_CHECK_ARG(dims_ok(ndim, dims), "consistency_fused_bwd: bad dims");
  ADVCHAIN_CHECK_ARG(N >= 0 && N < 65536 && K >= 1 && K <= kMaxK, "consistency_fused_bwd: bad N/K (K <= 16)");
  if (K < 2 || K > 4 || (mask && mask_channels != 1)) return ADVCHAIN_ERR_UNSUPPORTED;
  const Dims d = make_dims(ndim, dims);
  if (d.voxels() >= (1ll << 31) || !march4_ok(d, pred, ref, R, mask) || (reinterpret_cast<uintptr_t>(grad_pred) & 15) != 0)
    return ADVCHAIN_ERR_UNSUPPORTED;
  if (N == 0) return ADVCHAIN_OK;
  const bool kl = c_kl != 0.f;
  if (ndim == 3 && R && z3_takes(d, true)) {
    const int zc = z3_chunk(d, N);
    const dim3 gz = z3_grid(d, N, zc), bz(kZ3Waves * 64);
    const size_t lds = z3_lds(d, K);
    hipStream_t stz = (hipStream_t)stream;
#define BWD3DZ(K_) do { \
      if (kl) hipLaunchKernelGGL((k_loss_fused_bwd3d_z<K_, true>), gz, bz, lds, stz, pred, ref, R, mask, grad_scale, grad_pred, c_mse, c_a, c_b, d, zc, c_kl, ref_is_prob); \
      else hipLaunchKernelGGL((k_loss_fused_bwd3d_z<K_, false>), gz, bz, lds, stz, pred, ref, R, mask, grad_scale, grad_pred, c_mse, c_a, c_b, d, zc, c_kl, ref_is_prob); } while (0)
    switch (K) { case 2: BWD3DZ(2); break; case 3: BWD3DZ(3); break; default: BWD3DZ(4); break; }
#undef BWD3DZ
    ADVCHAIN_LAUNCH_CHECK();
    return ADVCHAIN_OK;
  }
  if (ndim == 3) return ADVCHAIN_ERR_UNSUPPORTED;
  const int mlen = march4_len(d, N);
  const dim3 g4 = march4_grid(d, N, mlen), b4(kBlock);
  hipStream_t st = (hipStream_t)stream;
#define FUSED_BWD(DIM_, K_) do { \
    if (kl) hipLaunchKernelGGL((k_loss_fused_bwd4<DIM_, K_, true>), g4, b4, 0, st, pred, ref, R, mask, grad_scale, grad_pred, c_mse, c_a, c_b, d, mlen, c_kl, ref_is_prob); \
    else hipLaunchKernelGGL((k_loss_fused_bwd4<DIM_, K_, false>), g4, b4, 0, st, pred, ref, R, mask, grad_scale, grad_pred, c_mse, c_a, c_b, d, mlen, c_kl, ref_is_prob); } while (0)
  switch (K) { case 2: FUSED_BWD(2, 2); break; case 3: FUSED_BWD(2, 3); break; default: FUSED_BWD(2, 4); break; }
#undef FUSED_BWD
  ADVCHAIN_LAUNCH_CHECK();
  return ADVCHAIN_OK;
}

int advchain_consistency_fused_fwd_bf16(const void* pred, const void* ref, const float* mask, void* R, float* sums, int64_t N,
                                        int64_t K, int ndim, const int64_t* dims, void* stream) {
  ADVCHAIN_CHECK_ARG(pred && ref && sums, "consistency_fused_fwd_bf16: null pointer");
  ADVCHAIN_CHECK_ARG(dims_ok(ndim, dims), "consistency_fused_fwd_bf16: bad dims");
  ADVCHAIN_CHECK_ARG(N >= 0 && N < 65536, "consistency_fused_fwd_bf16: bad N");
  const Dims d = make_dims(ndim, dims);
  const uintptr_t al = reinterpret_cast<uintptr_t>(pred) | reinterpret_cast<uintptr_t>(ref) | reinterpret_cast<uintptr_t>(R);
  if (ndim != 2 || K != 4 || d.s2 % 4 != 0 || d.s2 > 256 || (al & 7) != 0 || (reinterpret_cast<uintptr_t>(mask) & 15) != 0 ||
      d.voxels() >= (1ll << 31))
    return ADVCHAIN_ERR_UNSUPPORTED;
  if (N == 0) return ADVCHAIN_OK;
  const int mlen = march4_len(d, N);
// ... 29 lines not shown
```

### advchain_amd/csrc/loss_common.h

```cpp
#pragma once
#include "common.h"

#ifndef ADVCHAIN_SOFTMAX_FAST_EXP
#define ADVCHAIN_SOFTMAX_FAST_EXP 1
#endif
#if ADVCHAIN_SOFTMAX_FAST_EXP
#define ADVCHAIN_SM_EXP(x) __expf(x)
#else
#define ADVCHAIN_SM_EXP(x) expf(x)
#endif

namespace advchain {

__device__ __forceinline__ float hsm(int i) { return i == 1 ? 2.f : 1.f; }
__device__ __forceinline__ float hdf(int i) { return i == 0 ? 1.f : (i == 1 ? 0.f : -1.f); }

template <int DIM>
__device__ __forceinline__ void stencil_w(int a0, int a1, int a2, float& wa, float& wb) {
  if (DIM == 2) {
    wa = hsm(a1) * hdf(a2);
    wb = hdf(a1) * hsm(a2);
  } else {
    wa = hsm(a0) * hdf(a1) * hsm(a2);
    wb = hsm(a0) * hsm(a1) * hdf(a2);
  }
}

__device__ __forceinline__ float kl_prob(float t, int is_gt) { return is_gt ? (t == 0.f ? 1e-8f : 1.f) : t; }
__device__ __forceinline__ float kl_term(float t, float log_t, float log_q, float m, int is_gt) {
  const float p = kl_prob(t, is_gt);
  const float lp = is_gt ? logf(p) : log_t;
  return m * (p * lp) - m * (p * log_q);
}

struct SumsOrdered { int stride; };
__device__ __forceinline__ void sums_put(float* __restrict__ sums, int row, float v) {
  atomic_add_f32(sums + row * kSumSlots + sum_slot(), v);
}
__device__ __forceinline__ void sums_put(float* __restrict__ sums, int row, float v, const SumsOrdered& o) {
  sums[(int64_t)row * o.stride + ((int64_t)blockIdx.z * gridDim.y + blockIdx.y) * gridDim.x + blockIdx.x] = v;
}
__device__ __forceinline__ void sums_put(float* __restrict__ sums, int row, float v, const float*) { sums_put(sums, row, v); }
__device__ __forceinline__ void sums_put(float* __restrict__ sums, int row, float v, const float*, const SumsOrdered& o) {
  sums_put(sums, row, v, o);
}
struct OrdCounts {
  int64_t stride;
  int32_t* counts;
  bool fits(dim3 g) const { return (int64_t)g.x * g.y * g.z <= stride; }
  void set(int row, dim3 g) const { counts[row] = (int32_t)((int64_t)g.x * g.y * g.z); }
};


__device__ __forceinline__ void online_step(float x, float& mx, float& s) {
  const float d = x - sub_max(mx);
  const float e = ADVCHAIN_SM_EXP(-fabsf(d));
  if (d > 0.f) { s = s * e + 1.f; mx = x; }
  else s += e;
}

template <int DIM>
struct WTile {
  static constexpr int TX = DIM == 2 ? 64 : 32, TY = 8, TZ = DIM == 2 ? 1 : 4;
  static constexpr int HX = TX + 2, HY = TY + 2, HZ = DIM == 2 ? 1 : TZ + 2;
  static constexpr int NH = HX * HY * HZ, NO = TX * TY * TZ;
  static constexpr int SLOTS = (NH + kBlock - 1) / kBlock, OUTS = NO / kBlock;
  int x0, y0, z0;
  __device__ __forceinline__ WTile(const Dims& d) {
    const int tx = (d.s2 + TX - 1) / TX, ty = (d.s1 + TY - 1) / TY;
    const int b = blockIdx.x;
    x0 = (b % tx) * TX;
    y0 = ((b / tx) % ty) * TY;
    z0 = (b / (tx * ty)) * TZ;
  }
  __device__ __forceinline__ int halo_voxel(int e, const Dims& d) const {
    const int hx = e % HX, hy = (e / HX) % HY, hz = e / (HX * HY);
    const int gx = x0 + hx - 1, gy = y0 + hy - 1, gz = DIM == 3 ? z0 + hz - 1 : 0;
    const bool in = e < NH && gx >= 0 && gx < d.s2 && gy >= 0 && gy < d.s1 && gz >= 0 && gz < d.s0;
    return in ? (gz * d.s1 + gy) * d.s2 + gx : -1;
  }
  __device__ __forceinline__ int out_voxel(int o, const Dims& d, int& corner) const {
    const int ox = o % TX, oy = (o / TX) % TY, oz = o / (TX * TY);
    corner = (oz * HY + oy) * HX + ox;
    const int gx = x0 + ox, gy = y0 + oy, gz = z0 + oz;
    return (gx < d.s2 && gy < d.s1 && gz < d.s0) ? (gz * d.s1 + gy) * d.s2 + gx : -1;
  }
  static int64_t count(const Dims& d) {
    return (int64_t)((d.s2 + TX - 1) / TX) * ((d.s1 + TY - 1) / TY) * ((d.s0 + TZ - 1) / TZ);
  }
};

template <int DIM>
__device__ __forceinline__ void tile_stencil(const float* __restrict__ bufa, const float* __restrict__ bufb, int corner,
                                             float& ga, float& gb) {
  using T = WTile<DIM>;
  float sa = 0.f, sb = 0.f;
#pragma unroll
  for (int a0 = (DIM == 3 ? 0 : 1); a0 < (DIM == 3 ? 3 : 2); ++a0)
#pragma unroll
    for (int a1 = 0; a1 < 3; ++a1)
#pragma unroll
      for (int a2 = 0; a2 < 3; ++a2) {
        float wa, wb;
        stencil_w<DIM>(a0, a1, a2, wa, wb);
// ... 47 lines not shown
```

### advchain_amd/ops.py

```python
import collections
import ctypes
import functools

import numpy as np
import torch

from . import _lib
from .bands import gaussian_weights_1d

_INTERP = {"bilinear": 0, "trilinear": 0, "linear": 0, "nearest": 1, "bicubic": 2}
_PAD = {"zeros": 0, "border": 1, "reflection": 2}
_GAUSS9 = _lib.float_array(gaussian_weights_1d(1.0))
_GAUSS9_CACHE = {}


GENERIC_MAX_TAPS = 129


def gauss9(sigma, taps=None):
    sigma = float(sigma)
    if taps is None:
        taps = 2 * int(4 * sigma + 0.5) + 1
    taps = int(taps)
    if sigma == 1.0 and taps == 9:
# ... 97 lines not shown

def _hint_bits(disp):
    if disp is None or not disp == disp or disp < 0:
        return 0
    return min(int(disp) + 1, 255) << 8


def _fine_bits(disp):
    if disp is None or not disp == disp or disp < 0:
        return 0
    return max(1, min(int(disp * 1024.0) + 1, (1 << 22) - 1))


def raw_grid_sample_fwd(inp, grid, interp, padding, clamp_grid, disp_hint=None):
    N, C = inp.shape[:2]
    nd = inp.dim() - 2
    odims = grid.shape[2:]
    out = torch.empty((N, C) + tuple(odims), device=inp.device, dtype=torch.float32)
    _lib.check(_lib.load().advchain_grid_sample_fwd(_ptr(inp), _ptr(grid), _ptr(out), N, C, nd,
                                                    _lib.dims_array(inp.shape[2:]), _lib.dims_array(odims),
                                                    interp, padding, int(clamp_grid) | _hint_bits(disp_hint), _stream()),
               "grid_sample_fwd")
    return out


def raw_grid_sample_fwd_ride(inp, grid, ride, interp, padding, clamp_grid, nonzero, disp_hint=None):
    N, C = inp.shape[:2]
    nd = inp.dim() - 2
    odims = tuple(grid.shape[2:])
    out = torch.empty((N, C) + odims, device=inp.device, dtype=torch.float32)
    rout = torch.empty((N, 1) + odims, device=inp.device, dtype=torch.float32)
    _lib.check(_lib.load().advchain_grid_sample_fwd_ride(_ptr(inp), _ptr(grid), _ptr(out), _ptr(ride), _ptr(rout), N, C, nd,
                                                         _lib.dims_array(inp.shape[2:]), _lib.dims_array(odims), interp, padding,
                                                         int(clamp_grid) | _hint_bits(disp_hint), int(bool(nonzero)), _stream()),
               "grid_sample_fwd_ride")
    return out, rout


DISP_SLOTS = 4096
ADAPTIVE_HALO = True
PAIR_FIELDS = True
TILED_SCATTER = True
FUSED_LOSS = True
WIDE_LOSS_MIN_K = 17
REF_GRAD_REG_MAX_K = 4
FUSE_2D = True
COMPOSITE = True
RIDE_MASK = True
RIDE_INTERPS = ("bilinear", "trilinear", "linear", "nearest")
WINDOW_STAGED = True
WINDOW_STAGED_CHANNELS = (1, 2, 4)
BIAS_REDUCED = True
GAUSS_XY_LANES = True

BWD_ROUTES = ("none", "general", "rows", "gather", "march", "window_float", "window_int64", "window_staged", "tiled")


def last_bwd_route():
    return BWD_ROUTES[_lib.load().advchain_last_bwd_route()]


def set_deterministic(on):
    _lib.load().advchain_set_deterministic(1 if on else 0)


def is_deterministic():
    return bool(_lib.load().advchain_get_deterministic())


def _scatter_workspace(N, dims, device):
    n = _lib.load().advchain_scatter_workspace(N, len(dims), _lib.dims_array(dims))
    return torch.empty(n, device=device, dtype=torch.int32)


def _det_warp_workspace(N, C, dims, device):
    n = _lib.load().advchain_det_warp_workspace(N, C, len(dims), _lib.dims_array(dims))
    return torch.empty(max(1, n), device=device, dtype=torch.int32)


def _general_warp_kernel(C, interp, in_dims, out_dims):
    return C > 4 or interp != 0 or tuple(in_dims) != tuple(out_dims)


def raw_grid_sample_bwd(gout, inp, grid, interp, padding, clamp_grid, need_gin, need_ggrid, halo=0):
    N, C = inp.shape[:2]
    nd = inp.dim() - 2
    if need_gin and is_deterministic() and _general_warp_kernel(C, interp, inp.shape[2:], grid.shape[2:]):
        ws = _det_warp_workspace(N, C, inp.shape[2:], inp.device)
        gin = torch.empty_like(inp)
        ggrid = torch.empty_like(grid) if need_ggrid else None
        _lib.check(_lib.load().advchain_grid_sample_bwd_det(_ptr(gout), _ptr(inp), _ptr(grid), _ptr(gin), _ptr(ggrid), _ptr(ws),
                                                            N, C, nd, _lib.dims_array(inp.shape[2:]),
                                                            _lib.dims_array(grid.shape[2:]), interp, padding, int(clamp_grid),
                                                            _stream()), "grid_sample_bwd_det")
        return gin, ggrid
    tiled = TILED_SCATTER and need_gin
    ws = _scatter_workspace(N, inp.shape[2:], inp.device) if tiled else None
    gin = (torch.empty_like(inp) if tiled else torch.zeros_like(inp)) if need_gin else None
    ggrid = torch.empty_like(grid) if need_ggrid else None
    if (tiled and WINDOW_STAGED and nd == 2 and C in WINDOW_STAGED_CHANNELS and is_deterministic()
            and not _general_warp_kernel(C, interp, inp.shape[2:], grid.shape[2:])):
        lib = _lib.load()
        n = lib.advchain_window_stage_workspace(N, C, nd, _lib.dims_array(inp.shape[2:]))
        stage = torch.empty(max(4, n), device=inp.device, dtype=torch.int32)
        _lib.check(lib.advchain_grid_sample_bwd_staged(_ptr(gout), _ptr(inp), _ptr(grid), _ptr(gin), _ptr(ggrid), _ptr(ws),
                                                       N, C, nd, _lib.dims_array(inp.shape[2:]),
# ... 35 lines not shown
                                                     _lib.dims_array(phi.shape[2:]), _stream()), "max_displacement")
    return out


def raw_slot_rows_max(slots, reset=False, out=None):
    if out is None:
        out = torch.empty(slots.shape[0], device=slots.device, dtype=torch.float32)
    _lib.check(_lib.load().advchain_slot_rows_max(_ptr(slots), _ptr(out), slots.shape[0], slots.shape[1], int(bool(reset)),
                                                  _stream()), "slot_rows_max")
    return out


_PERSISTENT = {}


def _persistent_zeros(tag, shape, device):
    stream = _raw_stream(_raw_device()) if (_raw_stream and _raw_device) else torch.cuda.current_stream().cuda_stream
    key = (tag, tuple(shape), str(device), stream)
    plan = _PLAN
    if plan is not None and plan.is_frozen:
        key = key[:3]
        buf = plan.persistent.get(key)
        if buf is None:
            buf = plan.persistent[key] = torch.zeros(shape, device=device, dtype=torch.float32)
        return buf
    if plan is not None and plan.recording:
        plan.wanted_zeros.add(key[:3])
    buf = _PERSISTENT.get(key)
    if buf is None:
        if len(_PERSISTENT) > 64:
            _PERSISTENT.clear()
        buf = _PERSISTENT[key] = torch.zeros(shape, device=device, dtype=torch.float32)
    return buf


def _forget_persistent(buf):
    stores = [_PERSISTENT] + ([_PLAN.persistent] if _PLAN is not None else [])
    for store in stores:
        for k in [k for k, v in store.items() if v is buf]:
            del store[k]


def raw_gauss_small_pair(x, scale, adjoint=False, weights=None):
    if x[0, 0].numel() > 4096 or not x.is_contiguous() or (weights is not None and len(weights) != 9):
        return None
    nd = x.dim() - 2
    n_in = x.shape[0]
    n_out = n_in // 2 if adjoint else 2 * n_in
    out = torch.empty((n_out,) + tuple(x.shape[1:]), device=x.device, dtype=torch.float32)
    planes = (n_out if adjoint else n_in) * x.shape[1]
    _lib.check(_lib.load().advchain_gauss_small_pair(_ptr(x), _ptr(out), planes, nd, _lib.dims_array(x.shape[2:]),
                                                     weights or _GAUSS9, float(scale), int(bool(adjoint)), _stream()),
               "gauss_small_pair")
    return out


def raw_gauss_small_pair_into(x, out, scale, weights=None):
    _lib.check(_lib.load().advchain_gauss_small_pair(_ptr(x), _ptr(out), x.shape[0] * x.shape[1], x.dim() - 2,
                                                     _lib.dims_array(x.shape[2:]), weights or _GAUSS9, float(scale), 0, _stream()),
               "gauss_small_pair")


@_on_tensor_device
def sign_axpy(base, x, a, gate=None, old=None):
    x = _dev(x.detach(), "x")
    base = None if base is None else _dev(base.detach(), "base")
    gate, old = _gate_args(gate, old, x)
    out = torch.empty_like(x)
    _lib.check(_lib.load().advchain_sign_axpy(_ptr(base), _ptr(x), _ptr(out), float(a), x.numel(), _ptr(gate), _ptr(old),
                                              _stream()), "sign_axpy")
    return out


@_on_tensor_device
def nonzero_mask(x):
    x = _dev(x.detach(), "x")
    out = torch.empty_like(x)
    _lib.check(_lib.load().advchain_nonzero_mask(_ptr(x), _ptr(out), x.numel(), _stream()), "nonzero_mask")
    return out


_ONES = {}


def cached_ones(shape, device):
    key = (tuple(shape), str(device))
    plan = _PLAN
    store = plan.persistent if (plan is not None and plan.is_frozen) else _ONES
    t = store.get(("ones",) + key) if store is not _ONES else _ONES.get(key)
    if t is None:
        if store is _ONES:
            if len(_ONES) > 16:
                _ONES.clear()
            t = _ONES[key] = torch.ones(shape, device=device, dtype=torch.float32)
        else:
            t = _ONES.get(key)
            if t is None:
                t = torch.ones(shape, device=device, dtype=torch.float32)
            store[("ones",) + key] = t
    return t


_CLASS_W = {}


def class_weights_device(values, device):
# ... 44 lines not shown
    else:
        shape = tuple(x.shape)
    nd = x.dim() - 2
    planes = shape[0] * shape[1]
    dims = _lib.dims_array(x.shape[2:])
    axes = [2, 1, 0][:nd]
    lib = _lib.load()
    if len(w9) != 9:
        if post != 0 or pre not in (0, 1):
            raise NotImplementedError("the fused prologue / epilogue of the Gaussian exists for the 9-tap window only")
        cur = torch.cat([x, x_hi], 0) if x_hi is not None else x
        cur = cur if cur.is_contiguous() else cur.contiguous()
        for i, ax in enumerate(axes):
            out = torch.empty_like(cur)
            _lib.check(lib.advchain_gauss_axis_generic(_ptr(cur), _ptr(out), planes, nd, dims, ax, w9, len(w9),
                                                       float(scale) if (pre == 1 and i == 0) else 1.0, _stream()),
                       "gauss_axis_generic")
            cur = out
        return cur
    if x_hi is not None and (x[0, 0].numel() <= 4096 or not (x.is_contiguous() and x_hi.is_contiguous())):
        x, x_hi = torch.cat([x, x_hi], 0), None
    if post == 0 and pre in (0, 1) and x[0, 0].numel() <= 4096:
        out = torch.empty_like(x)
        _lib.check(lib.advchain_gauss_small(_ptr(x), _ptr(out), planes, nd, dims, w9, pre, float(scale), _stream()),
                   "gauss_small")
        return out
    cur = x
    out = torch.empty(shape, device=x.device, dtype=torch.float32)
    gauss_xy = lib.advchain_gauss_xy if GAUSS_XY_LANES else lib.advchain_gauss_xy_staged
    rc = gauss_xy(_ptr(x),_ptr(out), _ptr(aux) if (post == 2 and nd == 2) else None, planes, C, nd, dims, w9,
                               pre, post if nd == 2 else 0, float(scale) if pre == 1 else 1.0, _stream(), _ptr(x_hi),
                               x.shape[0] * x.shape[1])
    if rc == 0:
        if nd == 2:
            return out
        out2 = torch.empty_like(out)
        _lib.check(lib.advchain_gauss_axis(_ptr(out), _ptr(out2), _ptr(aux) if post == 2 else None, planes, C, nd, dims, 0,
                                           w9, 0, post, 1.0, _stream()), "gauss_axis")
        return out2
    if rc != -2:
        _lib.check(rc, "gauss_xy")
    if x_hi is not None:
        x = cur = torch.cat([x, x_hi], 0)
    for i, ax in enumerate(axes):
        out = torch.empty_like(x)
        p = pre if i == 0 else 0
        q = post if i == len(axes) - 1 else 0
        _lib.check(lib.advchain_gauss_axis(_ptr(cur), _ptr(out), _ptr(aux) if q == 2 else None, planes, C, nd, dims, ax,
                                           w9, p, q, float(scale) if p == 1 else 1.0, _stream()), "gauss_axis")
        cur = out
    return cur


def raw_tp_interp(coef, tables, C, add_identity=False, scale=1.0, want_out=True, sumsq=None, disp_out=None, out=None):
    planes = coef.shape[0] * coef.shape[1]
    if want_out and out is None:
        out = torch.empty((coef.shape[0], coef.shape[1]) + tuple(tables.full_dims), device=coef.device,
                          dtype=torch.float32)
    _lib.check(_lib.load().advchain_tp_interp_fwd(_ptr(coef), _ptr(out), _ptr(tables.itab), _ptr(tables.ftab),
                                                  _lib.dims_array(tables.S), _lib.dims_array(tables.g),
                                                  _lib.dims_array(tables.B), planes, C, tables.ndim,
                                                  int(add_identity), float(scale), _ptr(sumsq), _ptr(disp_out),
                                                  _stream()),
               "tp_interp_fwd")
    return out


def field_sumsq(coef, tables, C):
    coef = _dev(coef, "coefficients")
    if is_deterministic():
        lib = _lib.load()
        planes = coef.shape[0] * coef.shape[1]
        S = _lib.dims_array(tables.S)
        partials = torch.empty(max(1, lib.advchain_tp_interp_sumsq_partials(S, planes)), device=coef.device, dtype=torch.float32)
        out = torch.empty(1, device=coef.device, dtype=torch.float32)
        _lib.check(lib.advchain_tp_interp_sumsq_ordered(_ptr(coef), _ptr(tables.itab), _ptr(tables.ftab), S,
                                                        _lib.dims_array(tables.g), _lib.dims_array(tables.B), planes, C,
                                                        _ptr(partials), _ptr(out), _stream()), "tp_interp_sumsq_ordered")
        return out
    slots = torch.zeros(64, device=coef.device, dtype=torch.float32)
    raw_tp_interp(coef, tables, C, want_out=False, sumsq=slots)
    return slots.sum().reshape(1)


def raw_tp_adjoint(gfull, tables, gfull2=None, scale=1.0):
    return _tp_adjoint_passes(gfull, tables, gfull2, scale, (2, 1, 0))


def raw_tp_adjoint_from_t1(t1, tables):
    return _tp_adjoint_passes(t1, tables, None, 1.0, (1, 0))


def _tp_adjoint_passes(gfull, tables, gfull2, scale, axes):
    lib = _lib.load()
    N, C = gfull.shape[:2]
    S, g, B = list(tables.S), list(tables.g), list(tables.B)
    Sa, ga, Ba = _lib.dims_array(S), _lib.dims_array(g), _lib.dims_array(B)
    cur, cur2 = gfull, gfull2
    shape = list(S)
    for ax in (2, 1, 0):
        if ax not in axes:
            shape[ax] = g[ax]
    first = 2 in axes
    for ax in axes:
        if S[ax] == 1 and g[ax] == 1:
            continue
        outer = N * C
        for a in range(ax):
            outer *= shape[a]
        inner = 1
        for a in range(ax + 1, 3):
            inner *= shape[a]
        shape[ax] = g[ax]
        out = torch.empty((N, C) + tuple(shape[3 - tables.ndim:]), device=gfull.device, dtype=torch.float32)
        rc = -2
        if ax == 2 and inner == 1 and getattr(tables, "dense_inner", None) is not None:
            wd, lo, WB = tables.dense_inner
            rc = lib.advchain_band_reduce_rows_dense(_ptr(cur), _ptr(cur2), _ptr(out), _ptr(wd), _ptr(lo), outer, S[2], g[2], WB,
                                                     float(scale) if first else 1.0, _stream())
            if rc != -2:
                _lib.check(rc, "band_reduce_rows_dense")
        if rc == -2:
            _lib.check(lib.advchain_band_reduce_axis(_ptr(cur), _ptr(cur2), _ptr(out), _ptr(tables.itab), _ptr(tables.ftab),
                                                     Sa, ga, Ba, ax, outer, inner, float(scale) if first else 1.0,
                                                     _stream()), "band_reduce_axis")
        cur, cur2, first = out, None, False
    if first and 2 in axes:
        cur = (gfull - gfull2 if gfull2 is not None else gfull) * scale
    return cur


def raw_axpy(x, y, a):
    out = torch.empty_like(y)
    _lib.check(_lib.load().advchain_axpy(_ptr(x), _ptr(y), _ptr(out), float(a), y.numel(), _stream()), "axpy")
    return out


def _gate_args(gate, old, like):
    if gate is None:
        return None, None
    gate = _dev(gate.detach().reshape(1), "gate")
    old = _dev(old.detach(), "old")
    if old.shape != like.shape:
        raise RuntimeError("gated update: `old` must have the shape of the result")
    return gate, old


@_on_tensor_device
def normalized_axpy(base, x, step=1.0, gate=None, old=None):
    x = _dev(x.detach(), "x")
    base = None if base is None else _dev(base.detach(), "base")
    gate, old = _gate_args(gate, old, x)
    N = x.shape[0]
    M = x.numel() // max(N, 1)
# ... 638 lines not shown
        while True:
            out = _DemonsField._enqueue_chain(ctx, vel, s1, tables, d, n, scale, w9, pos_only, composite, plan, frozen, pair)
            if norm_rb is None:
                break
            norm, want = float(norm_rb.values()[0]), int(n_base)
            while norm / (2.0 ** want) > 0.5:
                want += 1
            norm_rb = None
            _NSTEPS_HINT[nkey] = want
            NSTEPS_STATS["chains"] += 1
            if plan is not None:
                if want != n:
                    del plan.pending[mark:]
                plan.pending.insert(mark, ("nsteps", dict(n=want, n_base=int(n_base))))
            if want == n:
                break
            NSTEPS_STATS["respeculated"] += 1
            n = want
        return out

    @staticmethod
    def _enqueue_chain(ctx, vel, s1, tables, d, n, scale, w9, pos_only, composite, plan, frozen, pair):
        N = s1.shape[0]
        inv = 1.0 / (2.0 ** n)
        disp = _persistent_zeros("disp", (n + 2, DISP_SLOTS), vel.device) if ADAPTIVE_HALO else None
        row = (lambda m: None) if disp is None else (lambda m: disp[m])
        key = (str(s1.device), tuple(s1.shape), n, HINT_SLOT)
        site = None
        if frozen:
            if disp is None:
                raise PlanMismatch("launch plan: a frozen chain needs the measured displacements (ops.ADAPTIVE_HALO is off)")
            site = plan.take("chain", n=n, d=d)
            hints = site["bounds"].values()
        else:
            pend = _PENDING_BOUNDS.pop(key, None)
            if pend is not None and pend.event.query():
                _note_chain_bounds(key, pend.values(), n)
            hints = _CHAIN_HINTS.get(key)
        full = (N, d) + tuple(tables.full_dims)
        phi0 = torch.empty(full, device=vel.device, dtype=torch.float32) if composite else \
            raw_tp_interp(s1, tables, d, add_identity=True, scale=inv, disp_out=row(0))
        fields = torch.empty((n - 1,) + tuple(phi0.shape), device=phi0.device, dtype=torch.float32)
        pos = torch.empty_like(phi0)
        harr = None if hints is None else (ctypes.c_int32 * n)(*[(_hint_bits(hints[m]) >> 8) | (_fine_bits(hints[m]) << 8)
                                                                 for m in range(n)])
        if COUNT_FUSED and harr is not None and disp is not None and FUSE_2D:
            FUSE_STATS["fused_levels"] += _lib.load().advchain_expo_chain_fused_levels(phi0.shape[0], d, _lib.dims_array(phi0.shape[2:]), n, harr)
        try:
            rows_max = rc = None
            if composite:
                q = torch.empty_like(phi0)
                rows_max = None if disp is None else (plan.slot(site) if site is not None else
                                                      torch.empty(disp.shape[0], device=vel.device, dtype=torch.float32))
                rc = _lib.load().advchain_demons_compose_pair_fwd(
                    _ptr(vel), _ptr(s1), _ptr(phi0), _ptr(fields), _ptr(pos), _ptr(q), _ptr(disp), _ptr(rows_max), _ptr(tables.itab),
                    _ptr(tables.ftab), _lib.dims_array(tables.S), _lib.dims_array(tables.g), _lib.dims_array(tables.B),
                    vel.shape[0], d, n, harr, w9, float(scale), float(inv), int(bool(FUSE_2D)), _stream())
                if rc == -2:
                    composite = ctx.composite = False
                    raw_gauss_small_pair_into(vel, s1, scale, w9)
                    raw_tp_interp(s1, tables, d, add_identity=True, scale=inv, disp_out=row(0), out=phi0)
                else:
                    _lib.check(rc, "demons_compose_pair_fwd")
            if not composite:
                _lib.check(_lib.load().advchain_expo_chain_fwd(_ptr(phi0), _ptr(fields), _ptr(pos), phi0.shape[0], d,
                                                               _lib.dims_array(phi0.shape[2:]), n, _ptr(disp), harr,
                                                               None if (disp is None or not FUSE_2D) else _ptr(disp[n + 1]), _stream()),
                           "expo_chain_fwd")
                q = pos if pos_only else raw_gauss(pos, d, pre=2, post=1, weights=w9)
                rows_max = None if disp is None else raw_slot_rows_max(disp, reset=True, out=None if site is None else plan.slot(site))
        except BaseException:
            if disp is not None:
                _forget_persistent(disp)
            raise
        ctx.save_for_backward(pos, phi0, fields)
        ctx.frozen = site is not None
        if site is not None:
            plan.check(rows_max, site)
            ctx.disp = site["bounds"]
        else:
            ctx.disp = None if rows_max is None else _Readback(rows_max)
            if ctx.disp is not None:
                _PENDING_BOUNDS[key] = ctx.disp
                if plan is not None:
                    plan.note("chain", rb=ctx.disp, n=n, d=d)
        global _LAST_FIELD_BOUND
        _LAST_FIELD_BOUND = None if ctx.disp is None else (ctx.disp, n)
        ctx.cfg = (scale, tables, inv, d)
        ctx.nsteps = n
        ctx.hint_key = key
        if pair:
            return q[:N // 2], q[N // 2:]
        return q

    @staticmethod
    def backward(ctx, *grads):
        pos, phi0, fields = ctx.saved_tensors
        scale, tables, inv, d = ctx.cfg
        smooth_iter, w9, pos_only = ctx.opts
        gq = tuple(_dev(g, "grad") for g in grads) if ctx.pair else _dev(grads[0], "grad")
        composite = (ctx.composite and TILED_SCATTER and ctx.pair and gq[0].is_contiguous() and gq[1].is_contiguous()
                     and gq[0].shape == gq[1].shape)
        if composite:
            gpos = torch.empty_like(pos)
        elif pos_only:
            gpos = torch.cat(gq, 0) if ctx.pair else gq.contiguous()
        else:
            gpos = raw_gauss(gq, d, post=2, aux=pos, weights=w9)
        g = gpos
        ws = _scatter_workspace(gpos.shape[0], gpos.shape[2:], gpos.device) if TILED_SCATTER else None
        n = ctx.nsteps
        if ctx.disp is not None:
            dm = ctx.disp.values()
            if not ctx.frozen:
                _PENDING_BOUNDS.pop(ctx.hint_key, None)
                _note_chain_bounds(ctx.hint_key, dm, n)
            halos = [squaring_halo(dm[m], d) for m in range(n - 1, -1, -1)]
        else:
            big = 2 if d == 3 else 16
            halos = [big, big, max(1, big // 2)] + [1 if d == 3 else 2] * n
        halos = halos[:n]
        if composite:
            N2 = gpos.shape[0]
            S, gg = list(tables.S), list(tables.g)
            g, scratch = torch.empty_like(gpos), torch.empty_like(gpos)
            t1 = torch.empty((N2, d, S[1], gg[2]), device=gpos.device, dtype=torch.float32)
            gs1 = torch.empty((N2, d, gg[1], gg[2]), device=gpos.device, dtype=torch.float32)
            gvel = torch.empty((N2 // 2, d, gg[1], gg[2]), device=gpos.device, dtype=torch.float32)
            wd, wlo, WB = tables.dense_inner
            rc = _lib.load().advchain_demons_compose_pair_bwd(
                _ptr(gq[0]), _ptr(gq[1]), _ptr(pos), _ptr(phi0), _ptr(fields), _ptr(gpos), _ptr(g), _ptr(scratch), _ptr(ws), _ptr(t1),
                _ptr(gs1), _ptr(gvel), (ctypes.c_int32 * n)(*[int(h) for h in halos]), _ptr(tables.itab), _ptr(tables.ftab), _ptr(wd),
                _ptr(wlo), int(WB), _lib.dims_array(S), _lib.dims_array(gg), _lib.dims_array(tables.B), N2 // 2, d, n, w9, float(scale),
                float(inv), _stream())
            if rc != -2:
                _lib.check(rc, "demons_compose_pair_bwd")
                return gvel, None, None, None, None, None, None
            gpos = raw_gauss(gq, d, post=2, aux=pos, weights=w9)
            g = gpos
        if ws is None:
            phis = [phi0] + list(fields.unbind(0))
            for i, phi in enumerate(reversed(phis)):
                g = raw_compose_self_bwd(g, phi, None, chain=False, halo=halos[i])
        else:
            g, scratch = torch.empty_like(gpos), torch.empty_like(gpos)
            _lib.check(_lib.load().advchain_expo_chain_bwd(_ptr(gpos), _ptr(phi0), _ptr(fields), _ptr(g), _ptr(scratch), _ptr(ws),
                                                           (ctypes.c_int32 * n)(*[int(h) for h in halos]), gpos.shape[0], d,
                                                           _lib.dims_array(gpos.shape[2:]), n, _stream()), "expo_chain_bwd")
        gs1 = raw_tp_adjoint(g, tables, gfull2=gpos, scale=inv)
        for _ in range(smooth_iter - 1):
            gs1 = raw_gauss(gs1, d, weights=w9)
        gvel = raw_gauss_small_pair(gs1, scale, adjoint=True, weights=w9) if ctx.pair else None
        if gvel is None:
            gvel = raw_gauss(gs1, d, pre=1, scale=scale, weights=w9)
            if ctx.pair:
                h = gvel.shape[0] // 2
                gvel = gvel[:h] - gvel[h:]
        return gvel, None, None, None, None, None, None


_LAST_FIELD_BOUND = None
HINT_SLOT = 0
FUSE_STATS = {"chains": 0, "refused": 0, "fused_levels": 0}
COUNT_FUSED = False


class _HintCache(dict):
    CAP = 256

    def __setitem__(self, key, value):
        if len(self) >= self.CAP and key not in self:
            self.clear()
        dict.__setitem__(self, key, value)


_NSTEPS_HINT = _HintCache()
NSTEPS_STATS = {"chains": 0, "respeculated": 0}
_PENDING_BOUNDS = _HintCache()


def _note_chain_bounds(key, dm, n):
    FUSE_STATS["chains"] += 1
    if len(dm) > n + 1 and dm[n + 1] > 0:
        FUSE_STATS["refused"] += 1
    _CHAIN_HINTS[key] = list(dm)


_CHAIN_HINTS = _HintCache()
_WARP_HINTS = _HintCache()


def _ride_key(rb, q):
    return None if isinstance(rb, _FrozenBounds) else (str(q.device),) + tuple(q.shape[2:])


@_on_tensor_device
def demons_field(vel, scale, tables, nsteps_rule, reduce_sumsq=None, opts=None):
    global _LAST_FIELD_BOUND
    _LAST_FIELD_BOUND = None
    q = _DemonsField.apply(vel, float(scale), tables, bool(nsteps_rule), reduce_sumsq, False, opts)
    if opts is not None and opts[3]:
        _LAST_FIELD_BOUND = None
# ... 55 lines not shown
    return qp, qm


def _aligned16(*tensors):
    return int(all(t is None or t.data_ptr() % 16 == 0 for t in tensors))


@functools.lru_cache(maxsize=256)
def _ordered_stride(family, N, K, shape, *flags):
    fn = getattr(_lib.load(), "advchain_consistency_%s_partials" % family)
    return int(fn(N, K, len(shape), _lib.dims_array(shape), *flags))


def _ordered_partials(n, what, device):
    if n < 0:
        raise ValueError("bad loss shape for %s" % what)
    stride = max(1, int(n))
    return torch.empty(4 * stride, device=device, dtype=torch.float32), stride, (ctypes.c_int32 * 4)()


class _Consistency(torch.autograd.Function):

    @staticmethod
    def forward(ctx, pred, ref, mask, coef, ref_is_prob, want_edges, class_w=None):
        pred, ref = _dev_logits(pred, "pred"), _dev_logits(ref, "reference")
        if class_w is not None and len(class_w) != pred.shape[1]:
            raise ValueError("class_w must have %d entries (one per class), got %d" % (pred.shape[1], len(class_w)))
        typed = class_w is not None or pred.dtype != torch.float32 or ref.dtype != torch.float32
        if typed and isinstance(mask, torch.Tensor) and mask.dtype in (torch.bfloat16, torch.float16, torch.float64):
            mask = mask.float()
        mask = None if mask is None else _dev(mask, "mask")
        N, K = pred.shape[:2]
        if typed or K >= WIDE_LOSS_MIN_K:
            return _Consistency._forward_lp(ctx, pred, ref, mask, coef, ref_is_prob, want_edges, class_w)
        nd = pred.dim() - 2
        dims = _lib.dims_array(pred.shape[2:])
        mch = 1 if mask is None else mask.shape[1]
        need_pred, need_ref = ctx.needs_input_grad[0], ctx.needs_input_grad[1]
        need_grad = need_pred or need_ref
        want_kl = coef[3] != 0.0
        R = None
        if need_grad and want_edges and K > 1:
            R = torch.empty((N, 2 * (K - 1)) + tuple(pred.shape[2:]), device=pred.device, dtype=torch.float32)
        sums = torch.empty(4, device=pred.device, dtype=torch.float32)
        value = torch.empty((), device=pred.device, dtype=torch.float32)
        lib = _lib.load()
        if is_deterministic():
            args = (N, K, nd, dims, mch, int(ref_is_prob), int(want_edges), int(want_kl), _stream())
            shape = tuple(pred.shape[2:])
            fused = False
            P = D = None
            nf = _ordered_stride("fused_fwd", N, K, shape, int(mask is not None), mch, int(want_edges),
                                 _aligned16(pred, ref, mask, R)) if FUSED_LOSS else -2
            if nf != -2:
                part, stride, counts = _ordered_partials(nf, "consistency_fused_fwd_ord", pred.device)
                rc = lib.advchain_consistency_fused_fwd_ord(_ptr(pred), _ptr(ref), _ptr(mask), _ptr(R), _ptr(part), stride,
                                                            counts, *args)
                fused = rc != -2
                if fused:
                    _lib.check(rc, "consistency_fused_fwd_ord")
            if not fused:
                P = torch.empty_like(pred)
                D = torch.empty_like(pred)
                part, stride, counts = _ordered_partials(_ordered_stride(
                    "fwd", N, K, shape, mch, int(want_edges), _aligned16(pred, ref, mask, P, D, R)), "consistency_fwd_ord",
                    pred.device)
                _lib.check(lib.advchain_consistency_fwd_ord(_ptr(pred), _ptr(ref), _ptr(mask), _ptr(P), _ptr(D), _ptr(R),
                                                            _ptr(part), stride, counts, *args), "consistency_fwd_ord")
            _lib.check(lib.advchain_consistency_finish_ord(_ptr(part), stride, counts, _lib.float_array(coef), _ptr(sums),
                                                           _ptr(value), _stream()), "consistency_finish_ord")
            return _Consistency._save_fp32(ctx, value, sums, pred, ref, mask, R, P, D, fused, coef, mch, ref_is_prob,
                                           want_edges)
        slots = _persistent_zeros("loss", (4, 64), pred.device)
        try:
            rc = lib.advchain_consistency_fused_fwd(_ptr(pred), _ptr(ref), _ptr(mask), _ptr(R), _ptr(slots), N, K, nd, dims, mch,
                                                    int(ref_is_prob), int(want_edges), int(want_kl), _stream()) if FUSED_LOSS else -2
            fused = rc != -2
            if fused:
                _lib.check(rc, "consistency_fused_fwd")
                P = D = None
            else:
                P = torch.empty_like(pred)
                D = torch.empty_like(pred)
                _lib.check(lib.advchain_consistency_fwd(_ptr(pred), _ptr(ref), _ptr(mask), _ptr(P), _ptr(D), _ptr(R),
                                                        _ptr(slots), N, K, nd, dims, mch, int(ref_is_prob),
                                                        int(want_edges), int(want_kl), _stream()), "consistency_fwd")
            _lib.check(lib.advchain_consistency_finish(_ptr(slots), _lib.float_array(coef), _ptr(sums), _ptr(value), 1,
                                                       _stream()), "consistency_finish")
        except BaseException:
            _forget_persistent(slots)
            raise
        return _Consistency._save_fp32(ctx, value, sums, pred, ref, mask, R, P, D, fused, coef, mch, ref_is_prob, want_edges)

    @staticmethod
    def _save_fp32(ctx, value, sums, pred, ref, mask, R, P, D, fused, coef, mch, ref_is_prob, want_edges):
        K = pred.shape[1]
        need_pred, need_ref = ctx.needs_input_grad[0], ctx.needs_input_grad[1]
        need_grad = need_pred or need_ref
        if need_grad:
            if fused:
                ctx.save_for_backward(pred, ref, R, mask)
            elif need_ref:
                ctx.save_for_backward(P if need_pred else None, D if need_pred else None, R, mask, pred, ref)
            else:
                ctx.save_for_backward(P, D, R, mask)
        ctx.ref_grad = need_ref and not (ref_is_prob and coef[0] == 0.0 and not (want_edges and K > 1))
        ctx.fused = fused
        ctx.cfg = (coef, mch, int(ref_is_prob))
        ctx.mark_non_differentiable(sums)
        ctx.set_materialize_grads(False)
        return value, sums

    @staticmethod
# ... 787 lines not shown
```

### include/advchain_hip.h

```cpp
#ifndef ADVCHAIN_HIP_H_
#define ADVCHAIN_HIP_H_

#include <stdint.h>

#ifdef __cplusplus
extern "C" {
#endif

#define ADVCHAIN_INTERP_LINEAR 0
#define ADVCHAIN_INTERP_NEAREST 1
#define ADVCHAIN_INTERP_BICUBIC 2
#define ADVCHAIN_PAD_ZEROS 0
#define ADVCHAIN_PAD_BORDER 1
#define ADVCHAIN_PAD_REFLECTION 2

int advchain_version(void);
const char* advchain_last_error(void);

void advchain_set_deterministic(int on);
int advchain_get_deterministic(void);

int advchain_grid_sample_fwd(const float* in, const float* grid, float* out, int64_t N, int64_t C, int ndim,
                             const int64_t* in_dims, const int64_t* out_dims, int interp, int padding,
                             int clamp_grid, void* stream);
int advchain_grid_sample_fwd_ride(const float* in, const float* grid, float* out, const float* ride_in, float* ride_out,
                                  int64_t N, int64_t C, int ndim, const int64_t* in_dims, const int64_t* out_dims,
                                  int interp, int padding, int clamp_grid, int flags, void* stream);
int64_t advchain_scatter_workspace(int64_t N, int ndim, const int64_t* dims);
int advchain_grid_sample_bwd(const float* grad_out, const float* in, const float* grid, float* grad_in,
                             float* grad_grid, int32_t* workspace, int64_t N, int64_t C, int ndim,
                             const int64_t* in_dims, const int64_t* out_dims, int interp, int padding, int clamp_grid,
                             int halo, void* stream);
int64_t advchain_window_stage_workspace(int64_t N, int64_t C, int ndim, const int64_t* in_dims);
int advchain_grid_sample_bwd_staged(const float* grad_out, const float* in, const float* grid, float* grad_in,
                                    float* grad_grid, int32_t* workspace, int64_t N, int64_t C, int ndim,
                                    const int64_t* in_dims, const int64_t* out_dims, int interp, int padding, int clamp_grid,
                                    int halo, void* stream, int32_t* stage_ws);
#define ADVCHAIN_ROUTE_NONE 0
#define ADVCHAIN_ROUTE_GENERAL 1
#define ADVCHAIN_ROUTE_ROWS 2
#define ADVCHAIN_ROUTE_GATHER 3
#define ADVCHAIN_ROUTE_MARCH 4
#define ADVCHAIN_ROUTE_WINDOW_FLOAT 5
#define ADVCHAIN_ROUTE_WINDOW_INT64 6
#define ADVCHAIN_ROUTE_WINDOW_STAGED 7
#define ADVCHAIN_ROUTE_TILED 8
int advchain_last_bwd_route(void);
int64_t advchain_det_warp_workspace(int64_t N, int64_t C, int ndim, const int64_t* in_dims);
int advchain_grid_sample_bwd_det(const float* grad_out, const float* in, const float* grid, float* grad_in,
                                 float* grad_grid, int32_t* det_ws, int64_t N, int64_t C, int ndim,
                                 const int64_t* in_dims, const int64_t* out_dims, int interp, int padding, int clamp_grid,
                                 void* stream);

#define ADVCHAIN_DISP_SLOTS 4096
int advchain_compose_self_fwd(const float* phi, float* out, const float* phi0, int64_t N, int ndim,
                              const int64_t* dims, int final_mode, float* disp_out, void* stream);
int advchain_compose_self_bwd(const float* grad_out, const float* phi, float* grad_phi, int32_t* workspace, int chain,
                              int halo, int64_t N, int ndim, const int64_t* dims, void* stream);
int advchain_expo_chain_fused_levels(int64_t N, int ndim, const int64_t* dims, int n, const int32_t* hints);
int advchain_expo_chain_fwd(const float* phi0, float* fields, float* pos, int64_t N, int ndim, const int64_t* dims, int n,
                            float* disp_rows, const int32_t* hints, float* fuse_flag, void* stream);
int advchain_expo_chain_bwd(const float* grad_pos, const float* phi0, const float* fields, float* grad_phi0, float* scratch,
                            int32_t* workspace, const int32_t* halos, int64_t N, int ndim, const int64_t* dims, int n,
                            void* stream);
int advchain_demons_compose_pair_fwd(const float* vel, float* s1, float* phi0, float* fields, float* pos, float* q,
                                     float* disp, float* rows_max, const int32_t* itab, const float* ftab,
                                     const int64_t* S3, const int64_t* g3, const int64_t* B3, int64_t N, int ndim, int n,
                                     const int32_t* hints, const float* weights9_host, float scale, float inv, int fuse,
                                     void* stream);
int advchain_demons_compose_pair_bwd(const float* gq_lo, const float* gq_hi, const float* pos, const float* phi0,
                                     const float* fields, float* gpos, float* g, float* scratch, int32_t* ws, float* t1,
                                     float* gs1, float* gvel, const int32_t* halos, const int32_t* itab, const float* ftab,
                                     const float* wd, const int32_t* wlo, int64_t WB, const int64_t* S3, const int64_t* g3,
// ... 38 lines not shown
int advchain_tp_interp_fwd(const float* coef, float* out, const int32_t* itab, const float* ftab, const int64_t* S,
                           const int64_t* g, const int64_t* B, int64_t planes, int64_t C, int ndim, int add_identity,
                           float scale, float* sumsq, float* disp_out, void* stream);
int64_t advchain_tp_interp_sumsq_partials(const int64_t* S, int64_t planes);
int advchain_tp_interp_sumsq_ordered(const float* coef, const int32_t* itab, const float* ftab, const int64_t* S, const int64_t* g,
                                     const int64_t* B, int64_t planes, int64_t C, float* partials, float* out, void* stream);
int advchain_tp_interp_fwd_smoothed_pair(const float* vel, float* s1, float* out, const int32_t* itab, const float* ftab,
                                         const int64_t* S, const int64_t* g, const int64_t* B, int64_t P, int64_t C,
                                         int add_identity, float scale, float* disp_out, const float* weights9, float gscale,
                                         void* stream);
int advchain_band_reduce_axis(const float* in, const float* in2, float* out, const int32_t* itab, const float* ftab,
                              const int64_t* S, const int64_t* g, const int64_t* B, int axis, int64_t outer,
                              int64_t inner, float scale, void* stream);
int advchain_band_reduce_rows_dense(const float* in, const float* in2, float* out, const float* wd, const int32_t* lo,
                                    int64_t rows, int64_t S, int64_t g, int64_t WB, float scale, void* stream);

int advchain_bias_field_fwd(const float* cp, const float* data, float* out, float* field, const int32_t* itab,
                            const float* ftab, const int64_t* S, const int64_t* g, const int64_t* B, int64_t N,
                            int64_t C, float eps, int use_log, float cp_scale, void* stream);
int advchain_bias_field_bwd(const float* cp, const float* data, const float* grad_out, float* grad_L, float* grad_data,
                            const int32_t* itab, const float* ftab, const int64_t* S, const int64_t* g,
                            const int64_t* B, int64_t N, int64_t C, float eps, int use_log, float cp_scale,
                            void* stream);
int advchain_bias_rows_per_wg(const int64_t* S, int64_t N);
int advchain_bias_field_fwd_rows(const float* cp, const float* data, float* out, float* field, const int32_t* itab,
                                 const float* ftab, const int64_t* S, const int64_t* g, const int64_t* B, int64_t N,
                                 int64_t C, float eps, int use_log, float cp_scale, int rows_per_wg, void* stream);
int advchain_bias_field_bwd_rows(const float* cp, const float* data, const float* grad_out, float* grad_L, float* grad_data,
                                 const int32_t* itab, const float* ftab, const int64_t* S, const int64_t* g,
                                 const int64_t* B, int64_t N, int64_t C, float eps, int use_log, float cp_scale,
                                 int rows_per_wg, void* stream);
int advchain_bias_field_bwd_reduced(const float* cp, const float* data, const float* grad_out, float* t1, float* grad_data,
                                    const int32_t* itab, const float* ftab, const int64_t* S, const int64_t* g,
                                    const int64_t* B, int64_t N, int64_t C, float eps, int use_log, float cp_scale,
                                    const float* wd, const int32_t* lo, int64_t WB, int rows_per_wg, void* stream);

int advchain_gauss_axis(const float* in, float* out, const float* aux, int64_t planes, int64_t C, int ndim,
                        const int64_t* dims, int axis, const float* weights9_host, int pre, int post, float scale,
                        void* stream);

int advchain_gauss_axis_generic(const float* in, float* out, int64_t planes, int ndim, const int64_t* dims, int axis,
                                const float* weights_host, int ntaps, float scale, void* stream);

int advchain_gauss_xy(const float* in, float* out, const float* aux, int64_t planes, int64_t C, int ndim, const int64_t* dims,
                      const float* weights9, int pre, int post, float scale, void* stream, const float* in_hi,
                      int64_t planes_lo);
int advchain_gauss_xy_staged(const float* in, float* out, const float* aux, int64_t planes, int64_t C, int ndim,
                             const int64_t* dims, const float* weights9, int pre, int post, float scale, void* stream,
                             const float* in_hi, int64_t planes_lo);
int advchain_gauss_xy_lanes(const float* in, float* out, const float* aux, int64_t planes, int64_t C, int ndim,
                            const int64_t* dims, const float* weights9, int pre, int post, float scale, void* stream,
                            const float* in_hi, int64_t planes_lo, int ty, int nt);
int advchain_gauss_xy_plan(int ndim, const int64_t* dims, int64_t planes, int* form, int* ty, int* nt);
int advchain_gauss_small(const float* in, float* out, int64_t planes, int ndim, const int64_t* dims,
                         const float* weights9_host, int pre, float scale, void* stream);

int advchain_gauss_small_pair(const float* in, float* out, int64_t planes, int ndim, const int64_t* dims,
                              const float* weights9_host, float scale, int adjoint, void* stream);

int advchain_axpy(const float* x, const float* y, float* out, float a, int64_t n, void* stream);
int advchain_sign_axpy(const float* base, const float* x, float* out, float a, int64_t n, const float* gate, const float* old,
                       void* stream);
int advchain_nonzero_mask(const float* x, float* out, int64_t n, void* stream);
int64_t advchain_norm_workspace(int64_t N, int64_t M);
int advchain_norm_axpy(const float* base, const float* x, float* out, float* workspace, float step, int64_t N,
                       int64_t M, void* stream);
int advchain_norm_axpy_gated(const float* base, const float* x, float* out, float* workspace, float step, int64_t N,
                             int64_t M, const float* gate, const float* old, void* stream);
typedef struct advchain_update_desc {
  const float* base;
  const float* x;
  float* out;
  const float* old;
  int64_t N;
  int64_t M;
  int32_t kind;
  float step;
} advchain_update_desc;
int advchain_update_multi(const advchain_update_desc* descs, int n, const float* gate, void* stream);

int advchain_consistency_fwd(const float* pred, const float* ref, const float* mask, float* P, float* D, float* R,
                             float* sums, int64_t N, int64_t K, int ndim, const int64_t* dims, int mask_channels,
                             int ref_is_prob, int want_edges, int want_kl, void* stream);
int advchain_consistency_finish(float* slots, const float* coef4_host, float* sums, float* value, int reset, void* stream);
int advchain_consistency_bwd(const float* P, const float* D, const float* R, const float* mask,
                             const float* grad_scale, float* grad_pred, float c_mse, float c_a, float c_b, float c_kl,
                             int kl_is_gt, int64_t N, int64_t K, int ndim, const int64_t* dims, int mask_channels,
                             void* stream);
int advchain_consistency_fused_fwd(const float* pred, const float* ref, const float* mask, float* R, float* sums, int64_t N,
                                   int64_t K, int ndim, const int64_t* dims, int mask_channels, int ref_is_prob, int want_edges,
                                   int want_kl, void* stream);
int advchain_consistency_fused_bwd(const float* pred, const float* ref, const float* R, const float* mask,
                                   const float* grad_scale, float* grad_pred, float c_mse, float c_a, float c_b, float c_kl,
                                   int ref_is_prob, int64_t N, int64_t K, int ndim, const int64_t* dims, int mask_channels,
                                   void* stream);

int advchain_consistency_wide_fwd(const float* pred, const float* ref, const float* mask, float* stats, float* R, float* sums,
                                  int64_t N, int64_t K, int ndim, const int64_t* dims, int mask_channels, int ref_is_prob,
                                  int want_edges, int want_kl, void* stream);
int advchain_consistency_wide_bwd(const float* pred, const float* ref, const float* stats, const float* R, const float* mask,
                                  const float* grad_scale, float* grad_pred, float c_mse, float c_a, float c_b, float c_kl,
                                  int ref_is_prob, int64_t N, int64_t K, int ndim, const int64_t* dims, int mask_channels,
                                  void* stream);

int advchain_consistency_ref_bwd(const float* pred, const float* ref, const float* stats ,
                                 const float* R , const float* mask, const float* grad_scale,
                                 float* grad_ref, float c_mse, float c_a, float c_b, float c_kl, int ref_is_prob,
                                 int64_t N, int64_t K, int ndim, const int64_t* dims, int mask_channels, void* stream);
void advchain_set_ref_grad_reg_max_k(int k);
int advchain_get_ref_grad_reg_max_k(void);

int advchain_consistency_lp_fwd(const void* pred, int pred_bf16, const void* ref, int ref_bf16, const float* mask, float* stats,
                                float* R , float* sums, int64_t N, int64_t K, int ndim, const int64_t* dims,
                                int mask_channels, int ref_is_prob, int want_edges, int want_kl, void* stream);
int advchain_consistency_lp_bwd(const void* pred, int pred_bf16, const void* ref, int ref_bf16, const float* stats,
                                const float* R , const float* mask, const float* grad_scale, void* grad_pred,
                                float c_mse, float c_a, float c_b, float c_kl, int ref_is_prob, int64_t N, int64_t K, int ndim,
                                const int64_t* dims, int mask_channels, void* stream);
int advchain_consistency_lp_ref_bwd(const void* pred, int pred_bf16, const void* ref, int ref_bf16, const float* stats,
                                    const float* R , const float* mask, const float* grad_scale, void* grad_ref,
                                    float c_mse, float c_a, float c_b, float c_kl, int ref_is_prob, int64_t N, int64_t K,
                                    int ndim, const int64_t* dims, int mask_channels, void* stream);

int advchain_consistency_cw_fwd(const void* pred, int pred_bf16, const void* ref, int ref_bf16, const float* mask, float* stats,
                                float* R , float* sums, int64_t N, int64_t K, int ndim, const int64_t* dims,
                                int mask_channels, int ref_is_prob, int want_edges, int want_kl, const float* class_w,
                                void* stream);
int advchain_consistency_cw_bwd(const void* pred, int pred_bf16, const void* ref, int ref_bf16, const float* stats,
                                const float* R , const float* mask, const float* grad_scale, void* grad_pred,
                                float c_mse, float c_a, float c_b, float c_kl, int ref_is_prob, int64_t N, int64_t K, int ndim,
                                const int64_t* dims, int mask_channels, const float* class_w, void* stream);
int advchain_consistency_cw_ref_bwd(const void* pred, int pred_bf16, const void* ref, int ref_bf16, const float* stats,
                                    const float* R , const float* mask, const float* grad_scale, void* grad_ref,
                                    float c_mse, float c_a, float c_b, float c_kl, int ref_is_prob, int64_t N, int64_t K,
                                    int ndim, const int64_t* dims, int mask_channels, const float* class_w, void* stream);

int64_t advchain_consistency_fwd_partials(int64_t N, int64_t K, int ndim, const int64_t* dims, int mask_channels, int want_edges,
                                          int aligned16);
int advchain_consistency_fwd_ord(const float* pred, const float* ref, const float* mask, float* P, float* D, float* R,
                                 float* partials, int64_t stride, int32_t* counts, int64_t N, int64_t K, int ndim,
                                 const int64_t* dims, int mask_channels, int ref_is_prob, int want_edges, int want_kl, void* stream);
int64_t advchain_consistency_fused_fwd_partials(int64_t N, int64_t K, int ndim, const int64_t* dims, int has_mask, int mask_channels,
                                                int want_edges, int aligned16);
int advchain_consistency_fused_fwd_ord(const float* pred, const float* ref, const float* mask, float* R, float* partials,
                                       int64_t stride, int32_t* counts, int64_t N, int64_t K, int ndim, const int64_t* dims,
                                       int mask_channels, int ref_is_prob, int want_edges, int want_kl, void* stream);
int64_t advchain_consistency_wide_fwd_partials(int64_t N, int64_t K, int ndim, const int64_t* dims, int want_edges, int aligned16);
int advchain_consistency_wide_fwd_ord(const float* pred, const float* ref, const float* mask, float* stats, float* R,
                                      float* partials, int64_t stride, int32_t* counts, int64_t N, int64_t K, int ndim,
                                      const int64_t* dims, int mask_channels, int ref_is_prob, int want_edges, int want_kl,
                                      void* stream);
int64_t advchain_consistency_lp_fwd_partials(int64_t N, int64_t K, int ndim, const int64_t* dims, int want_edges);
int advchain_consistency_lp_fwd_ord(const void* pred, int pred_bf16, const void* ref, int ref_bf16, const float* mask, float* stats,
                                    float* R, float* partials, int64_t stride, int32_t* counts, int64_t N, int64_t K, int ndim,
                                    const int64_t* dims, int mask_channels, int ref_is_prob, int want_edges, int want_kl,
                                    const float* class_w , void* stream);
int advchain_consistency_finish_ord(const float* partials, int64_t stride, const int32_t* counts4_host, const float* coef4_host,
                                    float* sums, float* value, void* stream);

int advchain_consistency_fused_fwd_bf16(const void* pred, const void* ref, const float* mask, void* R, float* sums, int64_t N,
                                        int64_t K, int ndim, const int64_t* dims, void* stream);
int advchain_consistency_fused_bwd_bf16(const void* pred, const void* ref, const void* R, const float* mask,
                                        const float* grad_scale, void* grad_pred, float c_mse, float c_a, float c_b, int64_t N,
                                        int64_t K, int ndim, const int64_t* dims, void* stream);

int64_t advchain_seg_loss_workspace(int64_t N, int ndim, const int64_t* dims);
int advchain_ce2d_fwd(const void* logits, int logits_bf16, const int64_t* labels, const float* soft, const float* weight,
                      float* lse, float* workspace, float* value, int64_t N, int64_t K, const int64_t* dims, float denom,
                      void* stream);
int advchain_ce2d_bwd(const void* logits, int logits_bf16, const int64_t* labels, const float* soft, const float* weight,
                      const float* lse, const float* grad_scale, void* grad_logits, float* grad_soft, int64_t N, int64_t K,
                      const int64_t* dims, float denom, void* stream);
int advchain_contour_fwd(const float* input, const int64_t* labels, const float* soft, const float* mask, float* R,
                         float* workspace, float* value, int64_t N, int64_t K, int ndim, const int64_t* dims, int first_class,
                         int mask_channels, void* stream);
int advchain_contour_bwd(const float* R, const float* grad_scale, float* grad_input, float* grad_soft, int64_t N, int64_t K,
                         int ndim, const int64_t* dims, int first_class, void* stream);
int advchain_one_hot(const int64_t* labels, float* out, int64_t N, int64_t depth, int64_t V, void* stream);

#define ADVCHAIN_DICE_IGNORE_BACKGROUND 1
#define ADVCHAIN_DICE_BATCH 2
int64_t advchain_dice_workspace(int64_t N, int64_t K, int ndim, const int64_t* dims);
int advchain_dice_fwd(const void* logits, int logits_bf16, const int64_t* labels, const float* soft, const float* weight,
                      float* lse, float* coef, float* workspace, float* value, int64_t N, int64_t K, int ndim,
                      const int64_t* dims, int flags, float smooth, float dice_w, float ce_w, void* stream);
int advchain_dice_bwd(const void* logits, int logits_bf16, const int64_t* labels, const float* soft, const float* weight,
                      const float* lse, const float* coef, const float* grad_scale, void* grad_logits, float* grad_soft,
                      int64_t N, int64_t K, int ndim, const int64_t* dims, float dice_w, float ce_w, void* stream);

int advchain_edt(const void* mask, int mask_kind, const float* sampling, int squared, float* out, int64_t B, int ndim,
                 const int64_t* dims, void* stream);
int64_t advchain_signed_maps_workspace(int64_t N, int64_t K, int ndim, const int64_t* dims);
int advchain_signed_maps(const int64_t* labels, const float* sampling, float* out, float* workspace, int64_t N, int64_t K,
                         int ndim, const int64_t* dims, void* stream);

int64_t advchain_surface_metrics_workspace(int64_t N, int64_t K, int ndim, const int64_t* dims);
int advchain_surface_metrics(const int64_t* pred, const int64_t* target, const float* sampling, double q, float* hausdorff,
                             float* hausdorff_pct, float* assd, float* directed, int64_t* surface_voxels, double* max_squared,
                             int64_t* overlap, float* dice, void* workspace, int64_t N, int64_t K, int ndim,
                             const int64_t* dims, void* stream);

#define ADVCHAIN_BOUNDARY_IGNORE_BACKGROUND 1
int64_t advchain_boundary_workspace(int64_t N, int64_t K, int ndim, const int64_t* dims);
int advchain_boundary_fwd(const void* logits, int logits_bf16, const int64_t* labels, const float* maps, const float* weight,
                          float* saved, float* workspace, float* value, int64_t N, int64_t K, int ndim, const int64_t* dims,
                          int flags, void* stream);
int advchain_boundary_bwd(const void* logits, int logits_bf16, const int64_t* labels, const float* maps, const float* weight,
                          const float* saved, const float* grad_scale, void* grad_logits, int64_t N, int64_t K, int ndim,
                          const int64_t* dims, int flags, void* stream);

int advchain_image_diff2d_fwd(const float* in, float* dx, float* dy, int64_t N, int64_t C, const int64_t* dims, void* stream);
// ... 28 lines not shown
```

Baseline: 4444.

## Fold slot-max, backward tail and loss finish into existing kernel launches

Moves the per-row slot max reduction into a prologue of the Gaussian smoothing kernel, and fuses the last band-reduce axis with the paired small Gaussian in the backward pass into one kernel. It also arms the consistency-loss finish step so it can run inside the ordered forward kernel. All three are guarded by a launch-fold mask that defaults to on. The goal is fewer kernel launches per adversarial step, at the cost of more LDS use and added code complexity in the fused kernels.

```diff
diff --git a/advchain_amd/_lib.py b/advchain_amd/_lib.py
--- a/advchain_amd/_lib.py
+++ b/advchain_amd/_lib.py
@@ -60,8 +60,14 @@
     "advchain_gauss_xy_staged": (_I, [_P, _P, _P, _L, _L, _I, _P, _P, _I, _I, _F, _P, _P, _L]),
     "advchain_gauss_xy_lanes": (_I, [_P, _P, _P, _L, _L, _I, _P, _P, _I, _I, _F, _P, _P, _L, _I, _I]),
     "advchain_gauss_xy_plan": (_I, [_I, _P, _L, _P, _P, _P]),
+    "advchain_gauss_xy_slots_plan": (_I, [_I, _P, _L, _L, _L, _I]),
+    "advchain_gauss_xy_slots": (_I, [_P, _P, _L, _L, _I, _P, _P, _P, _P, _L, _L, _I, _I, _P]),
+    "advchain_set_launch_folds": (None, [_I]),
+    "advchain_get_launch_folds": (_I, []),
     "advchain_gauss_small": (_I, [_P, _P, _L, _I, _P, _P, _I, _F, _P]),
     "advchain_gauss_small_pair": (_I, [_P, _P, _L, _I, _P, _P, _F, _I, _P]),
+    "advchain_band_reduce_gauss_pair_takes": (_I, [_P, _P]),
+    "advchain_band_reduce_gauss_pair": (_I, [_P, _P, _P, _P, _P, _P, _P, _L, _P, _F, _P]),
     "advchain_axpy": (_I, [_P, _P, _P, _F, _L, _P]),
     "advchain_sign_axpy": (_I, [_P, _P, _P, _F, _L, _P, _P, _P]),
     "advchain_nonzero_mask": (_I, [_P, _P, _L, _P]),
@@ -130,6 +136,8 @@
     "advchain_consistency_lp_fwd_partials": (_L, [_L, _L, _I, _P, _I]),
     "advchain_consistency_lp_fwd_ord": (_I, [_P, _I, _P, _I, _P, _P, _P, _P, _L, _P, _L, _L, _I, _P, _I, _I, _I, _I, _P, _P]),
     "advchain_consistency_finish_ord": (_I, [_P, _L, _P, _P, _P, _P, _P]),
+    "advchain_consistency_finish_ord_arm": (_I, [_P, _P, _P, _P, _P]),
+    "advchain_consistency_fused_fwd_ord_finish_takes": (_I, [_L, _L, _I, _P, _I, _I, _I, _I]),
 }
 
 class UpdateDesc(ctypes.Structure):
diff --git a/advchain_amd/csrc/adjoint_gather.hip b/advchain_amd/csrc/adjoint_gather.hip
--- a/advchain_amd/csrc/adjoint_gather.hip
+++ b/advchain_amd/csrc/adjoint_gather.hip
@@ -470,38 +470,9 @@
 
 template <int NT, int VEC>
 __global__ void __launch_bounds__(NT) k_slot_rows_max(float* __restrict__ slots, float* __restrict__ out, int cols, int reset) {
-  float* p = slots + (int64_t)blockIdx.x * cols;
-  float m = -3.4e38f;
-  bool nan = false;
-  if (VEC == 4) {
-    for (int j = threadIdx.x * 4; j < cols; j += NT * 4) {
-      const float4 v = *reinterpret_cast<const float4*>(p + j);
-      nan = nan || !(v.x == v.x) || !(v.y == v.y) || !(v.z == v.z) || !(v.w == v.w);
-      m = fmaxf(fmaxf(m, fmaxf(v.x, v.y)), fmaxf(v.z, v.w));
-      if (reset) *reinterpret_cast<float4*>(p + j) = make_float4(0.f, 0.f, 0.f, 0.f);
-    }
-  } else {
-    for (int j = threadIdx.x; j < cols; j += NT) {
-      const float v = p[j];
-      nan = nan || !(v == v);
-      m = fmaxf(m, v);
-      if (reset) p[j] = 0.f;
-    }
-  }
-#pragma unroll
-  for (int o = 32; o > 0; o >>= 1) {
-    m = fmaxf(m, __shfl_xor(m, o, 64));
-    const int other = __shfl_xor((int)nan, o, 64);
-    nan = nan || other != 0;
-  }
   __shared__ float sm[NT / 64];
   __shared__ int sn[NT / 64];
-  if ((threadIdx.x & 63) == 0) { sm[threadIdx.x >> 6] = m; sn[threadIdx.x >> 6] = nan; }
-  __syncthreads();
-  if (threadIdx.x == 0) {
-    for (int w = 1; w < NT / 64; ++w) { m = fmaxf(m, sm[w]); nan = nan || sn[w]; }
-    out[blockIdx.x] = nan ? __int_as_float(0x7fc00000) : m;
-  }
+  slot_row_max<NT, VEC>(slots + (int64_t)blockIdx.x * cols, out + blockIdx.x, cols, reset, sm, sn);
 }
 
 __global__ void __launch_bounds__(64) k_bounds_check(const float* __restrict__ v, const float* __restrict__ lo,
diff --git a/advchain_amd/csrc/common.h b/advchain_amd/csrc/common.h
--- a/advchain_amd/csrc/common.h
+++ b/advchain_amd/csrc/common.h
@@ -118,6 +118,40 @@
       for (int w = 0; w < nw; ++w) s += smem[w * NV + k];
       v[k] = s;
     }
+  }
+}
+
+template <int NT, int VEC>
+__device__ __forceinline__ void slot_row_max(float* __restrict__ p, float* __restrict__ out, int cols, int reset, float* sm,
+                                             int* sn) {
+  float m = -3.4e38f;
+  bool nan = false;
+  if (VEC == 4) {
+    for (int j = threadIdx.x * 4; j < cols; j += NT * 4) {
+      const float4 v = *reinterpret_cast<const float4*>(p + j);
+      nan = nan || !(v.x == v.x) || !(v.y == v.y) || !(v.z == v.z) || !(v.w == v.w);
+      m = fmaxf(fmaxf(m, fmaxf(v.x, v.y)), fmaxf(v.z, v.w));
+      if (reset) *reinterpret_cast<float4*>(p + j) = make_float4(0.f, 0.f, 0.f, 0.f);
+    }
+  } else {
+    for (int j = threadIdx.x; j < cols; j += NT) {
+      const float v = p[j];
+      nan = nan || !(v == v);
+      m = fmaxf(m, v);
+      if (reset) p[j] = 0.f;
+    }
+  }
+#pragma unroll
+  for (int o = 32; o > 0; o >>= 1) {
+    m = fmaxf(m, __shfl_xor(m, o, 64));
+    const int other = __shfl_xor((int)nan, o, 64);
+    nan = nan || other != 0;
+  }
+  if ((threadIdx.x & 63) == 0) { sm[threadIdx.x >> 6] = m; sn[threadIdx.x >> 6] = nan; }
+  __syncthreads();
+  if (threadIdx.x == 0) {
+    for (int w = 1; w < NT / 64; ++w) { m = fmaxf(m, sm[w]); nan = nan || sn[w]; }
+    *out = nan ? __int_as_float(0x7fc00000) : m;
   }
 }
 
diff --git a/advchain_amd/csrc/demons_compose.cpp b/advchain_amd/csrc/demons_compose.cpp
--- a/advchain_amd/csrc/demons_compose.cpp
+++ b/advchain_amd/csrc/demons_compose.cpp
@@ -47,6 +47,11 @@
   const int64_t slots = ADVCHAIN_DISP_SLOTS;
   rc = advchain_expo_chain_fwd(phi0, fields, pos, 2 * N, ndim, Sd, n, disp, hints, (disp && fuse) ? disp + (int64_t)(n + 1) * slots : nullptr, stream);
   if (rc != 0) return late(rc, "demons_compose_pair_fwd: the chain refused a shape the pre-check had accepted (launches already queued)");
+  if (disp && rows_max && (advchain_get_launch_folds() & ADVCHAIN_FOLD_SLOT_MAX)) {
+    rc = advchain_gauss_xy_slots(pos, q, 2 * N * ndim, ndim, ndim, Sd, weights9_host, disp, rows_max, n + 2, slots, 1, 0, stream);
+    if (rc != 0) return late(rc, "demons_compose_pair_fwd: the final smoothing refused a shape the pre-check had accepted (launches already queued)");
+    return rc;
+  }
   rc = advchain_gauss_xy(pos, q, nullptr, 2 * N * ndim, ndim, ndim, Sd, weights9_host, 2, 1, 1.0f, stream, nullptr, 2 * N * ndim);
   if (rc != 0) return late(rc, "demons_compose_pair_fwd: the final smoothing refused a shape the pre-check had accepted (launches already queued)");
   if (disp && rows_max) rc = advchain_slot_rows_max(disp, rows_max, n + 2, slots, 1, stream);
@@ -79,6 +84,10 @@
   rc = advchain_band_reduce_rows_dense(g, gpos, t1, wd, wlo, planes * S3[1], S3[2], g3[2], WB, inv, stream);
   if (rc == -2) rc = advchain_band_reduce_axis(g, gpos, t1, itab, ftab, S3, g3, B3, 2, planes * S3[1], 1, inv, stream);
   if (rc != 0) return rc;
+  if (advchain_get_launch_folds() & ADVCHAIN_FOLD_BWD_TAIL) {
+    rc = advchain_band_reduce_gauss_pair(t1, gvel, itab, ftab, S3, g3, B3, N * ndim, weights9_host, scale, stream);
+    if (rc != -2) return rc;
+  }
   rc = advchain_band_reduce_axis(t1, nullptr, gs1, itab, ftab, S3, g3, B3, 1, planes, g3[2], 1.0f, stream);
   if (rc != 0) return rc;
   return advchain_gauss_small_pair(gs1, gvel, N * ndim, ndim, gd, weights9_host, scale, 1, stream);
diff --git a/advchain_amd/csrc/error.cpp b/advchain_amd/csrc/error.cpp
--- a/advchain_amd/csrc/error.cpp
+++ b/advchain_amd/csrc/error.cpp
@@ -15,6 +15,10 @@
 extern "C" void advchain_set_deterministic(int on) { g_deterministic.store(on ? 1 : 0, std::memory_order_relaxed); }
 extern "C" int advchain_get_deterministic(void) { return g_deterministic.load(std::memory_order_relaxed); }
 
+static std::atomic<int> g_launch_folds{0x7fffffff};
+extern "C" void advchain_set_launch_folds(int mask) { g_launch_folds.store(mask, std::memory_order_relaxed); }
+extern "C" int advchain_get_launch_folds(void) { return g_launch_folds.load(std::memory_order_relaxed); }
+
 static thread_local int g_last_bwd_route = 0;
 extern "C" void advchain_set_route_(int route) { g_last_bwd_route = route; }
 extern "C" int advchain_last_bwd_route(void) { return g_last_bwd_route; }
diff --git a/advchain_amd/csrc/fields.hip b/advchain_amd/csrc/fields.hip
--- a/advchain_amd/csrc/fields.hip
+++ b/advchain_amd/csrc/fields.hip
@@ -1,3 +1,5 @@
+#include <tuple>
+#include <type_traits>
 #include "sampler_common.h"
 
 namespace advchain {
@@ -962,11 +964,28 @@
   *reinterpret_cast<float4*>(out + t) = make_float4(acc[0], acc[1], acc[2], acc[3]);
 }
 
-template <int PRE, int POST>
+struct GxySlotMax {
+  static constexpr int kPre = 2, kPost = 1;
+  float* slots;
+  float* out;
+  int rows, cols, reset;
+};
+template <int NT>
+__device__ __forceinline__ void gxy_prologue(float*) {}
+template <int NT>
+__device__ __forceinline__ void gxy_prologue(float* lds, const GxySlotMax& s) {
+  const int64_t wg = ((int64_t)blockIdx.z * gridDim.y + blockIdx.y) * gridDim.x + blockIdx.x;
+  if (wg >= s.rows) return;
+  slot_row_max<NT, 4>(s.slots + wg * s.cols, s.out + wg, s.cols, s.reset, lds, reinterpret_cast<int*>(lds) + NT / 64);
+  __syncthreads();
+}
+
+template <int PRE, int POST, class... X>
 __global__ void __launch_bounds__(kBlock)
 k_gauss_xy(const float* __restrict__ in, float* __restrict__ out, const float* __restrict__ aux, Dims d, int C, GaussW gw,
-           float scale, int TY, const float* __restrict__ in_hi, int planes_lo) {
+           float scale, int TY, const float* __restrict__ in_hi, int planes_lo, X... x) {
   extern __shared__ float gx_lds[];
+  gxy_prologue<kBlock>(gx_lds, x...);
   const int W = d.s2, Q = W >> 2, PA = W + 8;
   const int R = TY + 8;
   float* A = gx_lds;
@@ -1040,11 +1059,12 @@
   }
 }
 
-template <int PRE, int POST, int NT, int U>
+template <int PRE, int POST, int NT, int U, class... X>
 __global__ void __launch_bounds__(NT)
 k_gauss_xy_lanes(const float* __restrict__ in, float* __restrict__ out, const float* __restrict__ aux, Dims d, int C, GaussW gw,
-                 float scale, int TY, const float* __restrict__ in_hi, int planes_lo) {
+                 float scale, int TY, const float* __restrict__ in_hi, int planes_lo, X... x) {
   extern __shared__ float gx_lds[];
+  gxy_prologue<NT>(gx_lds, x...);
   const int W = d.s2, Q = W >> 2;
   const int R = TY + 8, NI = R * Q;
   float* B = gx_lds;
@@ -1263,6 +1283,88 @@
   }
 }
 
+constexpr int kTailMaxV = 1024;
+__global__ void __launch_bounds__(kBlock)
+k_band_reduce_gauss_pair(const float* __restrict__ in, float* __restrict__ out, int inner, BandAxis A, float yscale, GaussW gw,
+                         float gscale, int P) {
+  extern __shared__ __attribute__((aligned(16))) float tail_lds[];
+  __shared__ int lo_s[64];
+  const int V = A.g * inner, pitch = inner + 1;
+  float* slab = tail_lds;
+  float* Wd = slab + 2 * A.S * pitch;
+  float* ysum = Wd + kBrMaxW;
+  float* pp = ysum + 2 * V;
+  const int b = blockIdx.x;
+  const int q = inner >> 2, n1 = A.S * q, n4 = 2 * n1;
+  constexpr int U = 4;
+  float4 v[U];
+  auto fetch = [&](int idx) -> float4 {
+    const int e = min(idx, n4 - 1);
+    const int r = e / n1, e1 = e - r * n1;
+    const int sr = e1 / q, x4 = e1 - sr * q;
+    return *reinterpret_cast<const float4*>(in + ((int64_t)(b + r * P) * A.S + sr) * inner + 4 * x4);
+  };
+  auto put = [&](int idx, const float4& a) {
+    if (idx >= n4) return;
+    const int r = idx / n1, e1 = idx - r * n1;
+    const int sr = e1 / q, x4 = e1 - sr * q;
+    float* dst = slab + (r * A.S + sr) * pitch + 4 * x4;
+    dst[0] = a.x; dst[1] = a.y; dst[2] = a.z; dst[3] = a.w;
+  };
+#pragma unroll
+  for (int u = 0; u < U; ++u) v[u] = fetch(threadIdx.x + u * kBlock);
+  const int WB = stage_band(A, Wd, lo_s);
+#pragma unroll
+  for (int u = 0; u < U; ++u) put(threadIdx.x + u * kBlock, v[u]);
+  for (int i0 = threadIdx.x + U * kBlock; i0 < n4; i0 += U * kBlock) {
+#pragma unroll
+    for (int u = 0; u < U; ++u) v[u] = fetch(i0 + u * kBlock);
+#pragma unroll
+    for (int u = 0; u < U; ++u) put(i0 + u * kBlock, v[u]);
+  }
+  __syncthreads();
+  for (int t2 = threadIdx.x; t2 < 2 * V; t2 += kBlock) {
+    const int r = t2 / V, t = t2 - r * V;
+    const int k = t / inner, i = t - k * inner;
+    const float* sl = slab + r * A.S * pitch;
+    float acc = 0.f;
+    if (WB > 0) {
+      const int lo = lo_s[k];
+      const int len = min(WB, A.S - lo);
+      const float* w = Wd + k * WB;
+      const float* x = sl + lo * pitch + i;
+      for (int j = 0; j < len; ++j) acc = fmaf(x[j * pitch], w[j], acc);
+    } else {
+      const int lo = A.lo[k], hi = A.hi[k];
+      for (int sr = lo; sr < hi; ++sr) {
+        const int bb = k - A.start[sr];
+        if (bb >= 0 && bb < A.B) acc += sl[sr * pitch + i] * A.w[sr * A.B + bb];
+      }
+    }
+    const float gs = acc * yscale;
+    ysum[t2] = gs * gscale;
+  }
+  __syncthreads();
+  for (int pass = 0; pass < 2; ++pass) {
+    const float* src = pass == 0 ? ysum : pp;
+    float* dst = pass == 0 ? pp : ysum;
+    const int Sa = pass == 0 ? inner : A.g, st = pass == 0 ? 1 : inner;
+    for (int t2 = threadIdx.x; t2 < 2 * V; t2 += kBlock) {
+      const int i = t2 >= V ? t2 - V : t2;
+      const int ia = (i / st) % Sa;
+      float acc = 0.f;
+#pragma unroll
+      for (int k = -4; k <= 4; ++k) {
+        const int j = ia + k;
+        if (j >= 0 && j < Sa) acc += gw.w[k + 4] * src[t2 + k * st];
+      }
+      dst[t2] = acc;
+    }
+    __syncthreads();
+  }
+  for (int i = threadIdx.x; i < V; i += kBlock) out[(int64_t)b * V + i] = ysum[i] - ysum[V + i];
+}
+
 __global__ void __launch_bounds__(kBlock)
 k_axpy(const float* __restrict__ x, const float* __restrict__ y, float* __restrict__ out, float a, int64_t n4,
        int64_t n) {
@@ -1894,9 +1996,10 @@
 
 enum { kGxyAuto = 0, kGxyStaged = 1, kGxyLanes = 2 };
 
+template <class... X>
 static int gauss_xy_launch(const float* in, float* out, const float* aux, int64_t planes, int64_t C, int ndim, const int64_t* dims,
                            const float* weights9, int pre, int post, float scale, void* stream, const float* in_hi, int64_t planes_lo,
-                           int want, int ty, int nt) {
+                           int want, int ty, int nt, X... x) {
   ADVCHAIN_CHECK_ARG(in && out && in != out && weights9, "gauss_xy: null/aliased pointer");
   ADVCHAIN_CHECK_ARG(dims_ok(ndim, dims), "gauss_xy: bad dims");
   ADVCHAIN_CHECK_ARG(C >= 1 && C <= 3 && pre >= 0 && pre <= 2 && post >= 0 && post <= 2 && (post != 2 || aux), "gauss_xy: bad C/pre/post");
@@ -1920,15 +2023,20 @@
     const size_t lds = (size_t)(TY + 8) * d.s2 * sizeof(float);
     dim3 grid((unsigned)((d.s1 + TY - 1) / TY), (unsigned)d.s0, (unsigned)planes);
 #define GXL(PRE, POST, NT_, U_) do { \
-    auto kern = k_gauss_xy_lanes<PRE, POST, NT_, U_>; \
+    auto kern = k_gauss_xy_lanes<PRE, POST, NT_, U_, X...>; \
     if (lds > 65536) (void)hipFuncSetAttribute(reinterpret_cast<const void*>(kern), hipFuncAttributeMaxDynamicSharedMemorySize, (int)lds); \
-    hipLaunchKernelGGL(kern, grid, dim3(NT_), lds, st, in, out, aux, d, (int)C, gw, scale, TY, in_hi, (int)planes_lo); } while (0)
+    hipLaunchKernelGGL(kern, grid, dim3(NT_), lds, st, in, out, aux, d, (int)C, gw, scale, TY, in_hi, (int)planes_lo, x...); } while (0)
 #define GXL_TILE(PRE, POST) do { \
     if (ty == 16 && nt == 256) GXL(PRE, POST, 256, 6); \
     else if (ty == 16) GXL(PRE, POST, 512, 3); \
     else if (ty == 32 && nt == 256) GXL(PRE, POST, 256, 10); \
     else if (ty == 32) GXL(PRE, POST, 512, 5); \
     else GXL(PRE, POST, 1024, 5); } while (0)
+    if constexpr (sizeof...(X) != 0) {
+      using X0 = typename std::tuple_element<0, std::tuple<X...>>::type;
+      ADVCHAIN_CHECK_ARG(pre == X0::kPre && post == X0::kPost, "gauss_xy: hosted work with the wrong pre / post");
+      GXL_TILE(X0::kPre, X0::kPost);
+    } else
     switch (pre * 3 + post) {
       case 0: GXL_TILE(0, 0); break;
       case 1: GXL_TILE(0, 1); break;
@@ -1951,7 +2059,12 @@
   const size_t lds = (size_t)(TY + 8) * (2 * d.s2 + 8) * sizeof(float);
   if (lds > 65536) return ADVCHAIN_ERR_UNSUPPORTED;
   dim3 grid((unsigned)((d.s1 + TY - 1) / TY), (unsigned)d.s0, (unsigned)planes);
-#define GXY(PRE, POST) hipLaunchKernelGGL((k_gauss_xy<PRE, POST>), grid, dim3(kBlock), lds, st, in, out, aux, d, (int)C, gw, scale, TY, in_hi, (int)planes_lo)
+#define GXY(PRE, POST) hipLaunchKernelGGL((k_gauss_xy<PRE, POST, X...>), grid, dim3(kBlock), lds, st, in, out, aux, d, (int)C, gw, scale, TY, in_hi, (int)planes_lo, x...)
+  if constexpr (sizeof...(X) != 0) {
+    using X0 = typename std::tuple_element<0, std::tuple<X...>>::type;
+    ADVCHAIN_CHECK_ARG(pre == X0::kPre && post == X0::kPost, "gauss_xy: hosted work with the wrong pre / post");
+    GXY(X0::kPre, X0::kPost);
+  } else
   switch (pre * 3 + post) {
     case 0: GXY(0, 0); break;
     case 1: GXY(0, 1); break;
@@ -2001,6 +2114,38 @@
   while (TY > 8 && (size_t)(TY + 8) * (2 * d.s2 + 8) * 4 > 53248) TY >>= 1;
   *form = 1; *ty = gauss_xy_clamp_ty(TY, d); *nt = kBlock;
   return 0;
+}
+
+int advchain_gauss_xy_slots_plan(int ndim, const int64_t* dims, int64_t planes, int64_t rows, int64_t cols, int staged) {
+  int form = 0, ty = 0, nt = 0;
+  if (advchain_gauss_xy_plan(ndim, dims, planes, &form, &ty, &nt) != 0 || rows < 0 || rows >= 65536 || cols < 1 || cols >= (1ll << 31))
+    return -1;
+  if (form == 0) return ADVCHAIN_ERR_UNSUPPORTED;
+  const Dims d = make_dims(ndim, dims);
+  if (staged && form == 2) {
+    int TY = 32;
+    while (TY > 8 && (size_t)(TY + 8) * (2 * d.s2 + 8) * 4 > 53248) TY >>= 1;
+    ty = gauss_xy_clamp_ty(TY, d);
+  }
+  const int64_t wgs = (int64_t)((d.s1 + ty - 1) / ty) * d.s0 * planes;
+  return (rows >= 1 && rows <= wgs && (cols & 3) == 0) ? 1 : 0;
+}
+
+int advchain_slot_rows_max(float* slots, float* out, int64_t rows, int64_t cols, int reset, void* stream);
+int advchain_gauss_xy_slots(const float* in, float* out, int64_t planes, int64_t C, int ndim, const int64_t* dims,
+                            const float* weights9, float* slots, float* rows_out, int64_t rows, int64_t cols, int reset, int staged,
+                            void* stream) {
+  ADVCHAIN_CHECK_ARG(slots && rows_out, "gauss_xy_slots: null pointer");
+  const int plan = advchain_gauss_xy_slots_plan(ndim, dims, planes, rows, cols, staged);
+  ADVCHAIN_CHECK_ARG(plan != -1, "gauss_xy_slots: bad shape");
+  if (plan == ADVCHAIN_ERR_UNSUPPORTED) return plan;
+  const int want = staged ? kGxyStaged : kGxyAuto;
+  if (plan == 1 && (reinterpret_cast<uintptr_t>(slots) & 15) == 0)
+    return gauss_xy_launch(in, out, nullptr, planes, C, ndim, dims, weights9, 2, 1, 1.0f, stream, nullptr, planes, want, 0, 0,
+                           GxySlotMax{slots, rows_out, (int)rows, (int)cols, reset});
+  const int rc = gauss_xy_launch(in, out, nullptr, planes, C, ndim, dims, weights9, 2, 1, 1.0f, stream, nullptr, planes, want, 0, 0);
+  if (rc != ADVCHAIN_OK) return rc;
+  return advchain_slot_rows_max(slots, rows_out, rows, cols, reset, stream);
 }
 
 static int gauss_small_launch(const float* in, float* out, int64_t planes, int ndim, const int64_t* dims,
@@ -2035,6 +2180,32 @@
   return gauss_small_launch(in, out, planes, ndim, dims, weights9, 1, scale, adjoint ? 2 : 1, stream);
 }
 
+static size_t tail_lds_bytes(int64_t S1, int64_t g1, int64_t g2) {
+  return (size_t)(2 * S1 * (g2 + 1) + kBrMaxW + 4 * g1 * g2) * sizeof(float);
+}
+int advchain_band_reduce_gauss_pair_takes(const int64_t* S3, const int64_t* g3) {
+  if (!S3 || !g3 || S3[0] != 1 || g3[0] != 1 || S3[1] < 1 || g3[1] < 1 || g3[2] < 1) return 0;
+  if (g3[1] * g3[2] > kTailMaxV || (g3[2] & 3) != 0 || g3[1] > 64 || S3[1] > 4096) return 0;
+  return tail_lds_bytes(S3[1], g3[1], g3[2]) <= 65536 - 512 ? 1 : 0;
+}
+
+int advchain_band_reduce_gauss_pair(const float* t1, float* gvel, const int32_t* itab, const float* ftab, const int64_t* S,
+                                    const int64_t* g, const int64_t* B, int64_t P, const float* weights9, float scale,
+                                    void* stream) {
+  ADVCHAIN_CHECK_ARG(t1 && gvel && itab && ftab && weights9 && S && g && B, "band_reduce_gauss_pair: null pointer");
+  ADVCHAIN_CHECK_ARG(P >= 0 && 2 * P < 65536, "band_reduce_gauss_pair: bad plane count");
+  BandTables T;
+  ADVCHAIN_CHECK_ARG(unpack_tables(itab, ftab, S, g, B, T), "band_reduce_gauss_pair: bad band tables");
+  if (!advchain_band_reduce_gauss_pair_takes(S, g) || (reinterpret_cast<uintptr_t>(t1) & 15) != 0) return ADVCHAIN_ERR_UNSUPPORTED;
+  if (P == 0) return ADVCHAIN_OK;
+  GaussW gw;
+  for (int k = 0; k < 9; ++k) gw.w[k] = weights9[k];
+  hipLaunchKernelGGL(k_band_reduce_gauss_pair, dim3((unsigned)P), dim3(kBlock), tail_lds_bytes(S[1], g[1], g[2]), (hipStream_t)stream,
+                     t1, gvel, (int)g[2], T.a[1], 1.0f, gw, scale, (int)P);
+  ADVCHAIN_LAUNCH_CHECK();
+  return ADVCHAIN_OK;
+}
+
 int advchain_sign_axpy(const float* base, const float* x, float* out, float a, int64_t n, const float* gate, const float* old,
                        void* stream) {
   ADVCHAIN_CHECK_ARG(x && out && n >= 0 && (!gate || old), "sign_axpy: null pointer");
diff --git a/advchain_amd/csrc/loss.hip b/advchain_amd/csrc/loss.hip
--- a/advchain_amd/csrc/loss.hip
+++ b/advchain_amd/csrc/loss.hip
@@ -1,4 +1,5 @@
 #include <algorithm>
+#include <type_traits>
 #include "loss_common.h"
 
 namespace advchain {
@@ -870,6 +871,7 @@
     }
     if (KL) sums_put(sums, 3, acc[3], ord...);
   }
+  sums_done(sums, ord...);
 }
 
 template <int DIM, int K, bool KL, typename ST = float>
@@ -1434,6 +1436,12 @@
   return ADVCHAIN_OK;
 }
 
+static inline void ord_arm(const OrdCounts*) {}
+static inline void ord_arm(const OrdCounts*, SumsOrdered&) {}
+static inline void ord_arm(const OrdCounts* oc, SumsOrderedFinish& o) {
+  o.fin.n0 = oc->counts[0]; o.fin.n1 = oc->counts[1]; o.fin.n2 = oc->counts[2]; o.fin.n3 = oc->counts[3];
+}
+
 template <class... ORD>
 static int consistency_fused_fwd(const OrdCounts* oc, const float* pred, const float* ref, const float* mask, float* R, float* sums,
                                  int64_t N, int64_t K, int ndim, const int64_t* dims, int mask_channels, int ref_is_prob,
@@ -1458,7 +1466,10 @@
     if (edges) { oc->set(1, gf); oc->set(2, gf); }
     if (want_kl) oc->set(3, gf);
   }
-  if (zmarch) {
+  ord_arm(oc, ord...);
+  if constexpr ((std::is_same<ORD, SumsOrderedFinish>::value || ...)) {
+    if (zmarch) return ADVCHAIN_ERR_UNSUPPORTED;
+  } else if (zmarch) {
     const dim3 gz = gf, bz(kZ3Waves * 64);
     const size_t lds = z3_lds(d, K);
     hipStream_t stz = (hipStream_t)stream;
@@ -1487,16 +1498,7 @@
 __global__ void __launch_bounds__(kBlock)
 k_consistency_finish_ord(const float* __restrict__ partials, int stride, int n0, int n1, int n2, int n3, float c0, float c1, float c2,
                          float c3, float* __restrict__ sums, float* __restrict__ value) {
-  __shared__ float row[4];
-  const int r = threadIdx.x >> 6, j = threadIdx.x & 63;
-  const int cnt = r == 0 ? n0 : (r == 1 ? n1 : (r == 2 ? n2 : n3));
-  const float* p = partials + (int64_t)r * stride;
-  float v = 0.f;
-  for (int i = j; i < cnt; i += 64) v += p[i];
-  v = wave_sum(v);
-  if (j == 0) { row[r] = v; sums[r] = v; }
-  __syncthreads();
-  if (threadIdx.x == 0) value[0] = ((c0 * row[0] + c1 * row[1]) + c2 * row[2]) + c3 * row[3];
+  finish_ord_body<false>(partials, stride, OrdFinish{n0, n1, n2, n3, c0, c1, c2, c3, sums, value});
 }
 
 extern "C" {
@@ -1593,18 +1595,47 @@
   return (int64_t)g.x * g.y;
 }
 
+struct PendingFinish {
+  int state;
+  const float* partials;
+  uint32_t* arrive;
+  float coef[4];
+  float* sums;
+  float* value;
+};
+static thread_local PendingFinish g_pending_finish = {0, nullptr, nullptr, {0.f, 0.f, 0.f, 0.f}, nullptr, nullptr};
+
+int advchain_consistency_finish_ord_arm(const float* partials, uint32_t* arrive, const float* coef4_host, float* sums, float* value) {
+  g_pending_finish.state = 0;
+  ADVCHAIN_CHECK_ARG(partials && arrive && coef4_host && sums && value, "consistency_finish_ord_arm: null pointer");
+  g_pending_finish = PendingFinish{1, partials, arrive, {coef4_host[0], coef4_host[1], coef4_host[2], coef4_host[3]}, sums, value};
+  return ADVCHAIN_OK;
+}
+
 int advchain_consistency_fused_fwd_ord(const float* pred, const float* ref, const float* mask, float* R, float* partials,
                                        int64_t stride, int32_t* counts, int64_t N, int64_t K, int ndim, const int64_t* dims,
                                        int mask_channels, int ref_is_prob, int want_edges, int want_kl, void* stream) {
+  const PendingFinish pf = g_pending_finish;
+  g_pending_finish.state = 0;
   ADVCHAIN_CHECK_ARG(counts && stride >= 1 && stride < (1ll << 31), "consistency_fused_fwd_ord: bad partial buffer (stride / counts)");
   const OrdCounts oc{stride, counts};
+  if (pf.state == 1 && pf.partials == partials && ndim == 2 && N > 0) {
+    SumsOrderedFinish o{(int)stride, pf.arrive, OrdFinish{0, 0, 0, 0, pf.coef[0], pf.coef[1], pf.coef[2], pf.coef[3], pf.sums, pf.value}};
+    const int rc = consistency_fused_fwd<SumsOrderedFinish>(&oc, pred, ref, mask, R, partials, N, K, ndim, dims, mask_channels,
+                                                            ref_is_prob, want_edges, want_kl, stream, o);
+    if (rc == ADVCHAIN_OK) { g_pending_finish = pf; g_pending_finish.state = 2; }
+    return rc;
+  }
   return consistency_fused_fwd<SumsOrdered>(&oc, pred, ref, mask, R, partials, N, K, ndim, dims, mask_channels, ref_is_prob,
                                             want_edges, want_kl, stream, SumsOrdered{(int)stride});
 }
 
 int advchain_consistency_finish_ord(const float* partials, int64_t stride, const int32_t* counts4_host, const float* coef4_host,
                                     float* sums, float* value, void* stream) {
+  const PendingFinish pf = g_pending_finish;
+  g_pending_finish.state = 0;
   ADVCHAIN_CHECK_ARG(partials && counts4_host && coef4_host && sums && value, "consistency_finish_ord: null pointer");
+  if (pf.state == 2 && pf.partials == partials && pf.sums == sums && pf.value == value) return ADVCHAIN_OK;
   ADVCHAIN_CHECK_ARG(stride >= 1 && stride < (1ll << 31), "consistency_finish_ord: bad stride");
   for (int r = 0; r < 4; ++r)
     ADVCHAIN_CHECK_ARG(counts4_host[r] >= 0 && counts4_host[r] <= stride, "consistency_finish_ord: a count exceeds the stride");
@@ -1613,6 +1644,13 @@
                      sums, value);
   ADVCHAIN_LAUNCH_CHECK();
   return ADVCHAIN_OK;
+}
+
+int advchain_consistency_fused_fwd_ord_finish_takes(int64_t N, int64_t K, int ndim, const int64_t* dims, int has_mask,
+                                                    int mask_channels, int want_edges, int aligned16) {
+  const int64_t w = advchain_consistency_fused_fwd_partials(N, K, ndim, dims, has_mask, mask_channels, want_edges, aligned16);
+  if (w < 0) return (int)w;
+  return (ndim == 2 && N > 0) ? 1 : 0;
 }
 
 int advchain_consistency_fused_bwd(const float* pred, const float* ref, const float* R, const float* mask,
diff --git a/advchain_amd/csrc/loss_common.h b/advchain_amd/csrc/loss_common.h
--- a/advchain_amd/csrc/loss_common.h
+++ b/advchain_amd/csrc/loss_common.h
@@ -50,6 +50,56 @@
   bool fits(dim3 g) const { return (int64_t)g.x * g.y * g.z <= stride; }
   void set(int row, dim3 g) const { counts[row] = (int32_t)((int64_t)g.x * g.y * g.z); }
 };
+
+struct OrdFinish {
+  int n0, n1, n2, n3;
+  float c0, c1, c2, c3;
+  float* sums;
+  float* value;
+};
+template <bool COHERENT>
+__device__ __forceinline__ void finish_ord_body(const float* partials, int stride, const OrdFinish& f) {
+  __shared__ float row[4];
+  const int r = threadIdx.x >> 6, j = threadIdx.x & 63;
+  const int n0 = f.n0, n1 = f.n1, n2 = f.n2, n3 = f.n3;
+  const int cnt = r == 0 ? n0 : (r == 1 ? n1 : (r == 2 ? n2 : n3));
+  const float* p = partials + (int64_t)r * stride;
+  float v = 0.f;
+  for (int i = j; i < cnt; i += 64) v += COHERENT ? __hip_atomic_load(p + i, __ATOMIC_RELAXED, __HIP_MEMORY_SCOPE_AGENT) : p[i];
+  v = wave_sum(v);
+  if (j == 0) { row[r] = v; f.sums[r] = v; }
+  __syncthreads();
+  if (threadIdx.x == 0) f.value[0] = ((f.c0 * row[0] + f.c1 * row[1]) + f.c2 * row[2]) + f.c3 * row[3];
+}
+
+struct SumsOrderedFinish {
+  int stride;
+  unsigned int* arrive;
+  OrdFinish fin;
+};
+__device__ __forceinline__ void sums_put(float* __restrict__ sums, int row, float v, const SumsOrderedFinish& o) {
+  __hip_atomic_store(sums + (int64_t)row * o.stride + ((int64_t)blockIdx.z * gridDim.y + blockIdx.y) * gridDim.x + blockIdx.x, v,
+                     __ATOMIC_RELAXED, __HIP_MEMORY_SCOPE_AGENT);
+}
+__device__ __forceinline__ void sums_done(float*) {}
+__device__ __forceinline__ void sums_done(float*, const SumsOrdered&) {}
+__device__ __forceinline__ void sums_done(float* sums, const SumsOrderedFinish& o) {
+  __shared__ int is_last;
+  if (threadIdx.x == 0) {
+    asm volatile("s_waitcnt vmcnt(0)" ::: "memory");
+    const unsigned int total = gridDim.x * gridDim.y * gridDim.z;
+    const bool last = __hip_atomic_fetch_add(o.arrive, 1u, __ATOMIC_RELAXED, __HIP_MEMORY_SCOPE_AGENT) == total - 1u;
+    if (last) {
+      __builtin_amdgcn_fence(__ATOMIC_ACQUIRE, "agent");
+      asm volatile("s_waitcnt vmcnt(0)" ::: "memory");
+    }
+    is_last = last;
+  }
+  __syncthreads();
+  if (!is_last) return;
+  finish_ord_body<true>(sums, o.stride, o.fin);
+  if (threadIdx.x == 0) __hip_atomic_store(o.arrive, 0u, __ATOMIC_RELAXED, __HIP_MEMORY_SCOPE_AGENT);
+}
 
 
 __device__ __forceinline__ void online_step(float x, float& mx, float& s) {
diff --git a/advchain_amd/ops.py b/advchain_amd/ops.py
--- a/advchain_amd/ops.py
+++ b/advchain_amd/ops.py
@@ -173,6 +173,19 @@
 WINDOW_STAGED_CHANNELS = (1, 2, 4)
 BIAS_REDUCED = True
 GAUSS_XY_LANES = True
+SLOT_MAX_FOLDED = True
+LOSS_FINISH_FOLDED = True
+BWD_TAIL_FOLDED = True
+_FOLDS_SET = None
+
+
+def _sync_launch_folds():
+    global _FOLDS_SET
+    mask = (1 if SLOT_MAX_FOLDED else 0) | (2 if BWD_TAIL_FOLDED else 0)
+    if mask != _FOLDS_SET:
+        _lib.load().advchain_set_launch_folds(mask)
+        _FOLDS_SET = mask
+
 
 BWD_ROUTES = ("none", "general", "rows", "gather", "march", "window_float", "window_int64", "window_staged", "tiled")
 
@@ -314,6 +327,21 @@
     _lib.check(_lib.load().advchain_gauss_small_pair(_ptr(x), _ptr(out), planes, nd, _lib.dims_array(x.shape[2:]),
                                                      weights or _GAUSS9, float(scale), int(bool(adjoint)), _stream()),
                "gauss_small_pair")
+    return out
+
+
+def raw_band_reduce_gauss_pair(t1, tables, scale, weights=None):
+    w9 = weights or _GAUSS9
+    if tables.ndim != 2 or t1.dim() != 4 or t1.shape[0] % 2 or not t1.is_contiguous() or len(w9) != 9:
+        return None
+    g = list(tables.g)
+    out = torch.empty((t1.shape[0] // 2, t1.shape[1], g[1], g[2]), device=t1.device, dtype=torch.float32)
+    rc = _lib.load().advchain_band_reduce_gauss_pair(_ptr(t1), _ptr(out), _ptr(tables.itab), _ptr(tables.ftab),
+                                                     _lib.dims_array(tables.S), _lib.dims_array(g), _lib.dims_array(tables.B),
+                                                     (t1.shape[0] // 2) * t1.shape[1], w9, float(scale), _stream())
+    if rc == -2:
+        return None
+    _lib.check(rc, "band_reduce_gauss_pair")
     return out
 
 
@@ -464,6 +492,22 @@
     return cur
 
 
+def raw_gauss_slots(x, C, weights, slots, reset=True, out=None):
+    w9 = weights or _GAUSS9
+    if x.dim() != 4 or len(w9) != 9 or not x.is_contiguous():
+        return None
+    if out is None:
+        out = torch.empty(slots.shape[0], device=slots.device, dtype=torch.float32)
+    q = torch.empty_like(x)
+    rc = _lib.load().advchain_gauss_xy_slots(_ptr(x), _ptr(q), x.shape[0] * x.shape[1], C, 2, _lib.dims_array(x.shape[2:]), w9,
+                                             _ptr(slots), _ptr(out), slots.shape[0], slots.shape[1], int(bool(reset)),
+                                             int(not GAUSS_XY_LANES), _stream())
+    if rc == -2:
+        return None
+    _lib.check(rc, "gauss_xy_slots")
+    return q, out
+
+
 def raw_tp_interp(coef, tables, C, add_identity=False, scale=1.0, want_out=True, sumsq=None, disp_out=None, out=None):
     planes = coef.shape[0] * coef.shape[1]
     if want_out and out is None:
@@ -503,7 +547,11 @@
     return _tp_adjoint_passes(t1, tables, None, 1.0, (1, 0))
 
 
-def _tp_adjoint_passes(gfull, tables, gfull2, scale, axes):
+def raw_tp_adjoint_t1(gfull, tables, gfull2=None, scale=1.0):
+    return _tp_adjoint_passes(gfull, tables, gfull2, scale, (2,), reduced=())
+
+
+def _tp_adjoint_passes(gfull, tables, gfull2, scale, axes, reduced=None):
     lib = _lib.load()
     N, C = gfull.shape[:2]
     S, g, B = list(tables.S), list(tables.g), list(tables.B)
@@ -511,7 +559,7 @@
     cur, cur2 = gfull, gfull2
     shape = list(S)
     for ax in (2, 1, 0):
-        if ax not in axes:
+        if (ax not in axes) if reduced is None else (ax in reduced):
             shape[ax] = g[ax]
     first = 2 in axes
     for ax in axes:
@@ -1256,6 +1304,7 @@
                 q = torch.empty_like(phi0)
                 rows_max = None if disp is None else (plan.slot(site) if site is not None else
                                                       torch.empty(disp.shape[0], device=vel.device, dtype=torch.float32))
+                _sync_launch_folds()
                 rc = _lib.load().advchain_demons_compose_pair_fwd(
                     _ptr(vel), _ptr(s1), _ptr(phi0), _ptr(fields), _ptr(pos), _ptr(q), _ptr(disp), _ptr(rows_max), _ptr(tables.itab),
                     _ptr(tables.ftab), _lib.dims_array(tables.S), _lib.dims_array(tables.g), _lib.dims_array(tables.B),
@@ -1271,8 +1320,14 @@
                                                                _lib.dims_array(phi0.shape[2:]), n, _ptr(disp), harr,
                                                                None if (disp is None or not FUSE_2D) else _ptr(disp[n + 1]), _stream()),
                            "expo_chain_fwd")
-                q = pos if pos_only else raw_gauss(pos, d, pre=2, post=1, weights=w9)
-                rows_max = None if disp is None else raw_slot_rows_max(disp, reset=True, out=None if site is None else plan.slot(site))
+                both = None
+                if SLOT_MAX_FOLDED and disp is not None and not pos_only and d == 2:
+                    both = raw_gauss_slots(pos, d, w9, disp, reset=True, out=None if site is None else plan.slot(site))
+                if both is not None:
+                    q, rows_max = both
+                else:
+                    q = pos if pos_only else raw_gauss(pos, d, pre=2, post=1, weights=w9)
+                    rows_max = None if disp is None else raw_slot_rows_max(disp, reset=True, out=None if site is None else plan.slot(site))
         except BaseException:
             if disp is not None:
                 _forget_persistent(disp)
@@ -1332,6 +1387,7 @@
             gs1 = torch.empty((N2, d, gg[1], gg[2]), device=gpos.device, dtype=torch.float32)
             gvel = torch.empty((N2 // 2, d, gg[1], gg[2]), device=gpos.device, dtype=torch.float32)
             wd, wlo, WB = tables.dense_inner
+            _sync_launch_folds()
             rc = _lib.load().advchain_demons_compose_pair_bwd(
                 _ptr(gq[0]), _ptr(gq[1]), _ptr(pos), _ptr(phi0), _ptr(fields), _ptr(gpos), _ptr(g), _ptr(scratch), _ptr(ws), _ptr(t1),
                 _ptr(gs1), _ptr(gvel), (ctypes.c_int32 * n)(*[int(h) for h in halos]), _ptr(tables.itab), _ptr(tables.ftab), _ptr(wd),
@@ -1351,7 +1407,14 @@
             _lib.check(_lib.load().advchain_expo_chain_bwd(_ptr(gpos), _ptr(phi0), _ptr(fields), _ptr(g), _ptr(scratch), _ptr(ws),
                                                            (ctypes.c_int32 * n)(*[int(h) for h in halos]), gpos.shape[0], d,
                                                            _lib.dims_array(gpos.shape[2:]), n, _stream()), "expo_chain_bwd")
-        gs1 = raw_tp_adjoint(g, tables, gfull2=gpos, scale=inv)
+        if BWD_TAIL_FOLDED and ctx.pair and d == 2 and smooth_iter == 1:
+            t1 = raw_tp_adjoint_t1(g, tables, gfull2=gpos, scale=inv)
+            gvel = raw_band_reduce_gauss_pair(t1, tables, scale, w9)
+            if gvel is not None:
+                return gvel, None, None, None, None, None, None
+            gs1 = raw_tp_adjoint_from_t1(t1, tables)
+        else:
+            gs1 = raw_tp_adjoint(g, tables, gfull2=gpos, scale=inv)
         for _ in range(smooth_iter - 1):
             gs1 = raw_gauss(gs1, d, weights=w9)
         gvel = raw_gauss_small_pair(gs1, scale, adjoint=True, weights=w9) if ctx.pair else None
@@ -1513,13 +1576,23 @@
             P = D = None
             nf = _ordered_stride("fused_fwd", N, K, shape, int(mask is not None), mch, int(want_edges),
                                  _aligned16(pred, ref, mask, R)) if FUSED_LOSS else -2
-            if nf != -2:
-                part, stride, counts = _ordered_partials(nf, "consistency_fused_fwd_ord", pred.device)
-                rc = lib.advchain_consistency_fused_fwd_ord(_ptr(pred), _ptr(ref), _ptr(mask), _ptr(R), _ptr(part), stride,
-                                                            counts, *args)
-                fused = rc != -2
-                if fused:
-                    _lib.check(rc, "consistency_fused_fwd_ord")
+            arrive = None
+            try:
+                if nf != -2:
+                    part, stride, counts = _ordered_partials(nf, "consistency_fused_fwd_ord", pred.device)
+                    if LOSS_FINISH_FOLDED:
+                        arrive = _persistent_zeros("loss_arrive", (1,), pred.device)
+                        _lib.check(lib.advchain_consistency_finish_ord_arm(_ptr(part), _ptr(arrive), _lib.float_array(coef),
+                                                                           _ptr(sums), _ptr(value)), "consistency_finish_ord_arm")
+                    rc = lib.advchain_consistency_fused_fwd_ord(_ptr(pred), _ptr(ref), _ptr(mask), _ptr(R), _ptr(part), stride,
+                                                                counts, *args)
+                    fused = rc != -2
+                    if fused:
+                        _lib.check(rc, "consistency_fused_fwd_ord")
+            except BaseException:
+                if arrive is not None:
+                    _forget_persistent(arrive)
+                raise
             if not fused:
                 P = torch.empty_like(pred)
                 D = torch.empty_like(pred)
diff --git a/include/advchain_hip.h b/include/advchain_hip.h
--- a/include/advchain_hip.h
+++ b/include/advchain_hip.h
@@ -19,6 +19,11 @@
 
 void advchain_set_deterministic(int on);
 int advchain_get_deterministic(void);
+
+#define ADVCHAIN_FOLD_SLOT_MAX 1
+#define ADVCHAIN_FOLD_BWD_TAIL 2
+void advchain_set_launch_folds(int mask);
+int advchain_get_launch_folds(void);
 
 int advchain_grid_sample_fwd(const float* in, const float* grid, float* out, int64_t N, int64_t C, int ndim,
                              const int64_t* in_dims, const int64_t* out_dims, int interp, int padding,
@@ -163,11 +168,19 @@
                             const int64_t* dims, const float* weights9, int pre, int post, float scale, void* stream,
                             const float* in_hi, int64_t planes_lo, int ty, int nt);
 int advchain_gauss_xy_plan(int ndim, const int64_t* dims, int64_t planes, int* form, int* ty, int* nt);
+int advchain_gauss_xy_slots_plan(int ndim, const int64_t* dims, int64_t planes, int64_t rows, int64_t cols, int staged);
+int advchain_gauss_xy_slots(const float* in, float* out, int64_t planes, int64_t C, int ndim, const int64_t* dims,
+                            const float* weights9, float* slots, float* rows_out, int64_t rows, int64_t cols, int reset, int staged,
+                            void* stream);
 int advchain_gauss_small(const float* in, float* out, int64_t planes, int ndim, const int64_t* dims,
                          const float* weights9_host, int pre, float scale, void* stream);
 
 int advchain_gauss_small_pair(const float* in, float* out, int64_t planes, int ndim, const int64_t* dims,
                               const float* weights9_host, float scale, int adjoint, void* stream);
+int advchain_band_reduce_gauss_pair_takes(const int64_t* S, const int64_t* g);
+int advchain_band_reduce_gauss_pair(const float* t1, float* gvel, const int32_t* itab, const float* ftab, const int64_t* S,
+                                    const int64_t* g, const int64_t* B, int64_t P, const float* weights9_host, float scale,
+                                    void* stream);
 
 int advchain_axpy(const float* x, const float* y, float* out, float a, int64_t n, void* stream);
 int advchain_sign_axpy(const float* base, const float* x, float* out, float a, int64_t n, const float* gate, const float* old,
@@ -268,6 +281,9 @@
                                     const float* class_w , void* stream);
 int advchain_consistency_finish_ord(const float* partials, int64_t stride, const int32_t* counts4_host, const float* coef4_host,
                                     float* sums, float* value, void* stream);
+int advchain_consistency_finish_ord_arm(const float* partials, uint32_t* arrive, const float* coef4_host, float* sums, float* value);
+int advchain_consistency_fused_fwd_ord_finish_takes(int64_t N, int64_t K, int ndim, const int64_t* dims, int has_mask,
+                                                    int mask_channels, int want_edges, int aligned16);
 
 int advchain_consistency_fused_fwd_bf16(const void* pred, const void* ref, const float* mask, void* R, float* sums, int64_t N,
                                         int64_t K, int ndim, const int64_t* dims, void* stream);
```

Result: no change. 4460 (median of 4 runs) (+0.4%).
